# AgatheSenellart/MultiVae

Measured on AMD Instinct MI355X. Metric: train samples/sec (ELBO step) MoPoE MnistSvhn K=10, higher is better.
Workload: dtype f32 (error-corrected 2xfp16 / 3xbf16 products, fp32 accumulate); 1 GPU; MoPoE MnistSvhn (mnist MLP + svhn conv), K=10, per-device batch 512, latent_dim 20, Adam lr 1e-3, fwd+ELBO+bwd+optimizer; global_batch=512, K=10, parallelism=dp1, launch=hipGraph replay (fwd + bwd) + Adam

## Files before the change

include/mvk.h:

```cpp
#ifndef MVK_H
#define MVK_H

#include <stdint.h>

#ifdef __cplusplus
extern "C" {
#endif

#define MVK_OK 0
#define MVK_EINVAL (-1)
#define MVK_ELAUNCH (-2)

#define MVK_MAX_MODALITIES 8
#define MVK_MVAE_MAX_SUBSETS 32
#define MVK_IWAE_MAX_EXPERTS 32

#define MVK_DIST_NORMAL 0
#define MVK_DIST_LAPLACE 1
#define MVK_DIST_BERNOULLI 2
#define MVK_DIST_CATEGORICAL 3

#define MVK_ACT_NONE 0
#define MVK_ACT_RELU 1
#define MVK_ACT_SIGMOID 2
// ... 96 lines not shown
  int32_t fill;
} mvk_seed_desc;
int mvk_loss_backward_seed(const mvk_seed_desc* jobs, int n, const float* gscale, void* stream);


int mvk_mmvae_std_fwd(const float* lv, int rows, int L, int family, float* std, void* stream);
int mvk_mmvae_std_bwd(const float* lv, const float* std, const float* dstd, int rows, int L, int family,
                      float* dlv, void* stream);

int mvk_mmvae_latent_fwd(const float* const* mu, const float* const* std, const float* const* noise,
                         const uint8_t* const* masks, const float* prior_mean, const float* prior_std, int M,
                         int K, int B, int L, int family, float* const* z, float* const* lpz,
                         float* const* lqz, float* const* lq_all, int shared_dims, float* const* lqw, void* stream);

int mvk_mmvae_objective_fwd(const float* const* rows, const float* const* lpz, const float* const* lqz,
                            const uint8_t* const* masks, int M, int K, int B, int dreg, float* const* lw_out,
                            float* const* w, float* const* rowcoef, float* loss, const float* const* lqw, float beta,
                            void* stream);

int mvk_mmvae_latent_bwd(const float* const* mu, const float* const* std, const float* const* noise,
                         const float* const* z, const uint8_t* const* masks, const float* prior_mean,
                         const float* prior_std, const float* const* w, const float* const* lq_all,
                         const float* const* lqz, const float* const* dz_dec, int M, int K, int B, int L,
                         int family, int dreg, const float* gscale, float* const* dmu, float* const* dstd,
                         float* dprior_std, int shared_dims, float beta,
                         void* stream);

int mvk_mmvaeplus_cross_latent_fwd(const float* z, const float* prior_std, const float* noise, int64_t rows, int D,
                                   int Ls, int family, float* zc, void* stream);
int mvk_mmvaeplus_cross_latent_bwd(const float* dzc, const float* noise, int64_t rows, int D, int Ls, int family,
                                   float* dz, float* dprior_std, void* stream);


int mvk_iwae_sample(const float* loc, const float* sd, const float* noise, int K, int B, int L, int family, float* z,
                    void* stream);

int mvk_iwae_logw(const float* z, const float* const* rows, int n_rows, const float* const* loc,
                  const float* const* sd, int E, const float* prior_loc, const float* prior_sd, int K, int B, int L,
                  int family, float* lw, void* stream);

int mvk_iwae_reduce(const float* const* lw, int n, int K, int B, float* ll, void* stream);


int mvk_linear_fwd(const float* X, const float* W, const float* b, float* Y, int M, int N, int K, int act,
                   float* ws, int64_t ws_floats, void* stream);
int mvk_linear_bwd_data(const float* dY, const float* W, float* dX, int M, int N, int K, const float* y_out,
                        int y_act, const float* prev_out, int prev_act, int accumulate, float* colsum_acc,
                        float* ws, int64_t ws_floats, void* stream);
int mvk_linear_bwd_weight(const float* dY, const float* X, float* dW, float* db, int M, int N, int K,
                          const float* y_out, int y_act, float* ws, int64_t ws_floats, void* stream);
int64_t mvk_splitk_workspace_floats(int rows, int cols, int reduce_len);
int mvk_act_bwd_colsum(const float* dY, const float* Y, int act, int M, int N, float* dPre, float* db, float* ws,
                       int64_t ws_floats, void* stream);
int mvk_colsum_acc(const float* dY, const float* y_out, int y_act, float* db, int M, int N, float* ws, int64_t ws_floats,
                   void* stream);
int mvk_nchw_channel_sum_acc(const float* dY, const float* y_out, int y_act, float* db, int n, int c, int hw,
                             float* ws, int64_t ws_floats, void* stream);
int mvk_act_bwd(float* dY, const float* Y, int64_t n, int act, void* stream);
int mvk_act_bwd_scaled(const float* g, float a, const float* Y, int act, float* out, int64_t n, void* stream);

int mvk_gemm(const float* A, const float* B, float* C, int M, int N, int K, int ta, int tb, const float* bias,
             int bias_mod, int act, int accumulate, const float* a_act_src, int a_act, const float* c_act_src,
             int c_act, float* ws, int64_t ws_floats, void* stream);

#define MVK_FMT_IN_BF3 1
#define MVK_FMT_TILED 2
int mvk_f32_to_bf3(const float* x, int64_t n, void* planes, void* stream);
int mvk_bf3_to_f32(const void* planes, int64_t n, float* x, void* stream);

int mvk_pack_conv4s2_weight(const float* Wref, int Cv, int Cu, float* Wdown, int ld_down, int col_off,
                            float* Wup, void* stream);
#define MVK_PACK_MAX 16
typedef struct mvk_pack_desc {
  const float* Wref;
  float* Wdown;
  float* Wup;
  int Cv, Cu, ld_down, col_off, kind;
  void* Fdown;
  void* Fup;
  float* amax;
} mvk_pack_desc;
int64_t mvk_imgconv_frag_bytes(int Cu, int Cv);
int mvk_pack_weights(const mvk_pack_desc* jobs, int n, void* stream);
int mvk_conv4s2_down(const float* U, const float* Wdown, const float* bias, float* V, int n, int h, int w,
                     int Cu, int Cv, int act, int u_nchw, const float* u_act_src, int u_act,
                     const float* v_act_src, int v_act, float* colsum_acc, float* ws, int64_t ws_floats, int fmt,
                     const void* wfrag, void* stream);
int mvk_conv4s2_up(const float* V, const float* Wup, const float* bias, float* U, int n, int h, int w, int Cu,
                   int Cv, int act, int u_nchw, const float* u_act_src, int u_act, float* colsum_acc, float* ws,
                   int64_t ws_floats, int fmt, const void* wfrag, void* stream);
int mvk_gemm_smallk_amax(const float* A, const float* B, float* C, int M, int N, int K, int tb, const float* bias, int bias_mod,
                         int act, float* y_amax, void* stream);
int mvk_conv4s2_small_up_bwd_pre_y(const float* dpre, const float* rowscale, const float* V, int v_act, const float* Wref,
                                   float* dV, float* dWref, float* db, float* db_v, float* ws, int64_t ws_floats, int n, int h,
                                   int w, int Cu, int Cv, float* dv_amax, void* stream);
int mvk_conv4s2_scaled_ok(int n, int h, int w, int Cu, int Cv);
int mvk_conv4s2_wgrad_scaled_ok(int n, int h, int w, int Cu, int Cv);
int mvk_conv4s2_wgrad_s(const float* U, const float* V, float* dWref, int n, int h, int w, int Cu, int Cv, const float* u_amax,
                        const float* v_amax, float* ws, int64_t ws_floats, void* stream);
int mvk_conv4s2_down_s(const float* U, const float* Wdown, const float* bias, float* V, int n, int h, int w, int Cu, int Cv,
                       int act, const float* v_act_src, int v_act, float* colsum_acc, const float* x_amax,
                       const float* w_amax, float* y_amax, float* ws, int64_t ws_floats, const void* wfrag, void* stream);
int mvk_conv4s2_up_s(const float* V, const float* Wup, const float* bias, float* U, int n, int h, int w, int Cu, int Cv,
                     int act, const float* u_act_src, int u_act, float* colsum_acc, const float* x_amax, const float* w_amax,
                     float* y_amax, float* ws, int64_t ws_floats, const void* wfrag, void* stream);
int mvk_conv4s2_wgrad(const float* U, const float* V, float* dWref, int n, int h, int w, int Cu, int Cv,
                      int u_nchw, const float* u_act_src, int u_act, float* ws, int64_t ws_floats, void* stream);
int mvk_conv4s2_wgrad_pair(const float* U0, const float* V0, float* dW0, int h0, int w0, int Cu0, int Cv0, const float* U1,
                           const float* V1, float* dW1, int h1, int w1, int Cu1, int Cv1, int n, float* ws, int64_t ws_floats,
                           void* stream);

int mvk_conv3x3(const float* X, const float* Wp, const float* bias, float* Y, int n, int H, int W, int Cin, int Cout,
                int act, const float* y_act_src, int y_src_act, float* colsum_acc, float* ws, int64_t ws_floats,
                void* stream);
int mvk_conv3x3_res(const float* X, const float* Wp, const float* bias, float* Y, int n, int H, int W, int Cin,
                    int Cout, int act, const float* y_act_src, int y_src_act, const float* res, float res_alpha,
                    float* ws, int64_t ws_floats, void* stream);
int mvk_conv3x3_wgrad(const float* X, const float* dY, float* dWref, int n, int H, int W, int Cin, int Cout,
                      float* ws, int64_t ws_floats, void* stream);
int mvk_conv3x3_fused_ok(int n, int H, int W, int Cin, int Cout);
int mvk_conv3x3_f(const float* X, const float* Wp, const float* bias, float* Y, int n, int H, int W, int Cin, int Cout,
                  int act, const float* y_act_src, int y_src_act, const float* res, float res_alpha, float* colsum_acc,
                  int x_act, float pre_scale, float* ws, int64_t ws_floats, void* stream);
int mvk_conv3x3_wgrad_f(const float* X, const float* dY, float* dWref, float* db, int n, int H, int W, int Cin, int Cout,
                        int x_act, float dy_scale, float* ws, int64_t ws_floats, void* stream);
int mvk_amax(const float* x, int64_t n, float* out, void* stream);
int mvk_conv3x3_y(const float* X, const float* Wp, const float* bias, float* Y, int n, int H, int W, int Cin, int Cout, int act,
                  const float* y_act_src, int y_src_act, float* colsum_acc, float* y_amax, float* ws, int64_t ws_floats,
                  void* stream);
int mvk_conv3x3_scaled_ok(int n, int H, int W, int Cin, int Cout);
int mvk_conv3x3_s(const float* X, const float* Wp, const float* bias, float* Y, int n, int H, int W, int Cin, int Cout,
                  int act, const float* y_act_src, int y_src_act, const float* res, float res_alpha, float* colsum_acc,
                  int x_act, float pre_scale, const float* x_amax, const float* w_amax, float* y_amax, float* ws,
                  int64_t ws_floats, void* stream);
int mvk_conv3x3_s2(const float* X, const float* Wp, const float* bias, float* Y, float* y_pre, int n, int H, int W, int Cin, int Cout,
                   int act, const float* res, float res_alpha, const float* x_amax, const float* w_amax, float* y_amax, float* ws,
                   int64_t ws_floats, void* stream);
int mvk_conv3x3_s_part(const float* X, int x_channels, int x_off, const float* Wp, const float* bias, float* Y, int n, int H, int W,
                       int Cin, int Cout, int act, const float* y_act_src, int y_src_act, const float* res, int res_pre, int x_act,
                       float pre_scale, const float* x_amax, const float* w_amax, float* y_amax, void* stream);
int mvk_conv3x3_wgrad_scaled_ok(int n, int H, int W, int Cin, int Cout);
int mvk_conv3x3_wgrad_s(const float* X, const float* dY, float* dWref, float* db, int n, int H, int W, int Cin, int Cout,
                        int x_act, float dy_scale, const float* x_amax, const float* dy_amax, float* ws, int64_t ws_floats,
                        void* stream);
int mvk_avgpool3s2_fwd(const float* x, float* y, int n, int H, int W, int C, void* stream);
int mvk_avgpool3s2_bwd(const float* dy, float* dx, int n, int H, int W, int C, void* stream);
int mvk_upsample2_fwd(const float* x, float* y, int n, int H, int W, int C, void* stream);
int mvk_upsample2_bwd(const float* dy, float* dx, int n, int H, int W, int C, void* stream);
int mvk_axpby(const float* x, float a, const float* y, float b, int64_t n, int act, float* out, void* stream);
int mvk_probe_mfma_bf16(float* out, int iters, int random_operands, void* stream);
int mvk_probe_stream_copy(float* dst, const float* src, int64_t n, void* stream);
int mvk_transpose_act(const float* x, float* y, int batch, int rows, int cols, int act, const float* msrc, int dact,
                      void* stream);

int mvk_device_rng(float* out, int64_t n, uint64_t* state, int uniform, float lo, float hi, void* stream);
int mvk_conv4s2_up_nchw_small(const float* V, const float* Wref, const float* bias, float* U, int n, int h,
                              int w, int Cu, int Cv, int act, void* stream);

int mvk_conv4s2_small_down_fwd(const float* U, const float* Wdown, const float* bias, float* V, int n, int h, int w,
                               int Cu, int Cv, int act, void* stream);
int mvk_conv4s2_small_down_fwd_wref(const float* U, const float* Wref, const float* bias, float* V, int n, int h, int w,
                                    int Cu, int Cv, int act, void* stream);
int mvk_conv4s2_small_up_supported(int h, int w, int Cu, int Cv);
int mvk_conv4s2_small_up_fwd(const float* V, const float* Wref, const float* bias, float* U, int n, int h, int w,
                             int Cu, int Cv, int act, void* stream);
int mvk_conv4s2_small_up_bwd(const float* dU, const float* Uout, int u_act, const float* V, int v_act,
                             const float* Wref, float* dV, float* dWref, float* db, float* db_v, float* ws,
                             int64_t ws_floats, int n, int h, int w, int Cu, int Cv, void* stream);
int mvk_conv4s2_small_up_nll_supported(int h, int w, int Cu, int Cv);
int mvk_conv4s2_small_up_fwd_nll(const float* V, const float* Wref, const float* bias, const float* X, int xrows, float scale,
                                 float* dpre, float* rows, int n, int h, int w, int Cu, int Cv, int act, void* stream);
int mvk_conv4s2_small_up_bwd_pre(const float* dpre, const float* rowscale, const float* V, int v_act, const float* Wref,
                                 float* dV, float* dWref, float* db, float* db_v, float* ws, int64_t ws_floats, int n, int h,
                                 int w, int Cu, int Cv, void* stream);
int mvk_conv4s2_small_up_fwd_nll_w(const float* V, const float* Wref, const float* bias, const float* X, int xrows, float scale,
                                   float grad_weight, float* dpre, float* rows, int n, int h, int w, int Cu, int Cv, int act,
                                   void* stream);
int mvk_conv4s2_small_up_fwd_s(const float* V, const float* Wref, const float* bias, float* U, int n, int h, int w, int Cu, int Cv,
                               int act, const float* v_amax, void* stream);
int mvk_conv4s2_small_up_fwd_nll_s(const float* V, const float* Wref, const float* bias, const float* X, int xrows, float scale,
                                   float grad_weight, float* dpre, float* rows, int n, int h, int w, int Cu, int Cv, int act,
                                   const float* v_amax, void* stream);
int mvk_conv4s2_small_up_fwd_nll_sy(const float* V, const float* Wref, const float* bias, const float* X, int xrows, float scale,
                                    float grad_weight, float* dpre, float* rows, int n, int h, int w, int Cu, int Cv, int act,
                                    const float* v_amax, float* dpre_amax, void* stream);
int mvk_conv4s2_small_up_bwd_pre_s(const float* dpre, const float* rowscale, const float* V, int v_act, const float* Wref,
                                   float* dV, float* dWref, float* db, float* db_v, float* ws, int64_t ws_floats, int n, int h,
                                   int w, int Cu, int Cv, const float* dpre_amax, const float* v_amax, float* dv_amax,
// ... 178 lines not shown
```

multivae_amd/_lib.py:

```python
import ctypes as C
import os

import torch

_HERE = os.path.dirname(os.path.abspath(__file__))


_ALWAYS_READ = {"MVK_TUNE", "MVK_LIB_PATH", "MVK_DEFER_MB", "MVK_SYNC_DEBUG", "MVK_TRAINER_ALLOW_CPU", "MVK_CPU_THREADS",
                "MVK_BENCH_SAME_GPU", "MVK_FORCE_DIST", "MVK_DIST_BACKEND", "MVK_ADAM_ZERO", "MVK_RCCL", "MVK_BENCH_CHILD", "MVK_OVERLAP", "MVK_GRAPH_ADAM"}


def _warn_ignored_switches():
    if os.environ.get("MVK_TUNE") == "1":
        return
    ignored = sorted(k for k in os.environ if k.startswith("MVK_") and k not in _ALWAYS_READ)
    if ignored:
        import warnings

        warnings.warn(f"{', '.join(ignored)} set without MVK_TUNE=1: experiment switches are ignored unless MVK_TUNE=1 "
                      "(this process runs the shipped configuration)", RuntimeWarning, stacklevel=3)


_warn_ignored_switches()


def tune(name, default):
    return os.environ.get(name, default) if os.environ.get("MVK_TUNE") == "1" else default


LIB_PATH = os.environ.get("MVK_LIB_PATH") or os.path.join(_HERE, "libmvk.so")

MVK_OK = 0
DIST = {"normal": 0, "laplace": 1, "bernoulli": 2, "categorical": 3}
ACT = {None: 0, "none": 0, "relu": 1, "sigmoid": 2, "leaky_relu_0.2": 3}
FAMILY = {"normal": 0, "laplace_with_softmax": 1, "normal_with_softplus": 2}
MAX_MODALITIES = 8

_p = C.c_void_p
_i = C.c_int
_f = C.c_float
_d = C.c_double
_i64 = C.c_int64


class ReconDesc(C.Structure):
    _fields_ = [("recon", _p), ("x", _p), ("mask", _p), ("rows", _p), ("drecon", _p), ("rowcoef", _p),
                ("D", _i64), ("dist", C.c_int32), ("scale", _f), ("rescale", _f), ("coef", _f),
                ("n_classes", C.c_int32)]


class PackDesc(C.Structure):
    _fields_ = [("Wref", _p), ("Wdown", _p), ("Wup", _p), ("Cv", C.c_int32), ("Cu", C.c_int32),
                ("ld_down", C.c_int32), ("col_off", C.c_int32), ("kind", C.c_int32), ("Fdown", _p), ("Fup", _p),
                ("amax", _p)]


class CopyDesc(C.Structure):
    _fields_ = [("dst", _p), ("src", _p), ("bytes", _i64)]


class SeedDesc(C.Structure):
    _fields_ = [("buf", _p), ("n", _i64), ("coef", _f), ("fill", C.c_int32)]


class TermDesc(C.Structure):
    _fields_ = [("v", _p), ("mask", _p), ("n", _i64), ("period", _i64), ("coef", _f), ("lossw", _f), ("gfill", _p)]


PROTOTYPES = {
    "mvk_version": [],
    "mvk_mopoe_posterior_fwd": [_p, _p, _i, _p, _i, _p, _p, _p, _i, _i, _i, _p, _p, _p, _p, _p, _p, _p],
    "mvk_mopoe_posterior_bwd": [_p, _p, _i, _p, _i, _p, _p, _p, _p, _i, _i, _i, _p, _p, _p, _p],
    "mvk_mvtcae_posterior_fwd": [_p, _p, _p, _i, _p, _i, _i, _i, _p, _p, _p, _p, _p, _p],
    "mvk_mvtcae_posterior_bwd": [_p, _p, _p, _i, _p, _p, _i, _i, _i, _p, _p, _p, _p, _p],
    "mvk_jmvae_posterior_fwd": [_p, _p, _p, _p, _i, _p, _i, _i, _i, _p, _p, _p, _p],
    "mvk_jmvae_posterior_bwd": [_p, _p, _p, _p, _i, _p, _p, _i, _i, _i, _p, _p, _p, _p, _p, _p, _p],
    "mvk_recon_nll_fwd": [C.POINTER(ReconDesc), _i, _i, _i, _p],
    "mvk_recon_nll_bwd": [C.POINTER(ReconDesc), _i, _i, _i, _p],
    "mvk_reduce_terms": [C.POINTER(TermDesc), _i, _f, _p, _p, _p],
    "mvk_reduce_terms_ws": [C.POINTER(TermDesc), _i, _f, _p, _p, _p, _i64, _p],
    "mvk_scale_by_device_scalar": [_p, _i64, _p, _p],
    "mvk_linear_fwd": [_p, _p, _p, _p, _i, _i, _i, _i, _p, _i64, _p],
    "mvk_linear_bwd_data": [_p, _p, _p, _i, _i, _i, _p, _i, _p, _i, _i, _p, _p, _i64, _p],
    "mvk_linear_bwd_weight": [_p, _p, _p, _p, _i, _i, _i, _p, _i, _p, _i64, _p],
    "mvk_act_bwd_colsum": [_p, _p, _i, _i, _i, _p, _p, _p, _i64, _p],
    "mvk_colsum_acc": [_p, _p, _i, _p, _i, _i, _p, _i64, _p],
    "mvk_nchw_channel_sum_acc": [_p, _p, _i, _p, _i, _i, _i, _p, _i64, _p],
    "mvk_act_bwd": [_p, _p, _i64, _i, _p],
    "mvk_act_bwd_scaled": [_p, _f, _p, _i, _p, _i64, _p],
    "mvk_gemm": [_p, _p, _p, _i, _i, _i, _i, _i, _p, _i, _i, _i, _p, _i, _p, _i, _p, _i64, _p],
    "mvk_pack_conv4s2_weight": [_p, _i, _i, _p, _i, _i, _p, _p],
    "mvk_conv4s2_down": [_p, _p, _p, _p, _i, _i, _i, _i, _i, _i, _i, _p, _i, _p, _i, _p, _p, _i64, _i, _p, _p],
    "mvk_conv4s2_up": [_p, _p, _p, _p, _i, _i, _i, _i, _i, _i, _i, _p, _i, _p, _p, _i64, _i, _p, _p],
    "mvk_pack_weights": [C.POINTER(PackDesc), _i, _p],
    "mvk_loss_backward_seed": [C.POINTER(SeedDesc), _i, _p, _p],
    "mvk_f32_to_bf3": [_p, _i64, _p, _p],
    "mvk_bf3_to_f32": [_p, _i64, _p, _p],
    "mvk_conv4s2_small_up_fwd_nll": [_p, _p, _p, _p, _i, _f, _p, _p, _i, _i, _i, _i, _i, _i, _p],
    "mvk_conv4s2_small_up_fwd_nll_w": [_p, _p, _p, _p, _i, _f, _f, _p, _p, _i, _i, _i, _i, _i, _i, _p],
    "mvk_conv4s2_small_up_fwd_nll_s": [_p, _p, _p, _p, _i, _f, _f, _p, _p, _i, _i, _i, _i, _i, _i, _p, _p],
    "mvk_conv4s2_small_up_fwd_s": [_p, _p, _p, _p, _i, _i, _i, _i, _i, _i, _p, _p],
    "mvk_conv4s2_small_up_fwd_nll_sy": [_p, _p, _p, _p, _i, _f, _f, _p, _p, _i, _i, _i, _i, _i, _i, _p, _p, _p],
    "mvk_conv4s2_small_up_bwd_pre_s": [_p, _p, _p, _i, _p, _p, _p, _p, _p, _p, _i64, _i, _i, _i, _i, _i, _p, _p, _p, _p],
    "mvk_conv4s2_small_up_bwd_pre": [_p, _p, _p, _i, _p, _p, _p, _p, _p, _p, _i64, _i, _i, _i, _i, _i, _p],
    "mvk_conv3x3": [_p, _p, _p, _p, _i, _i, _i, _i, _i, _i, _p, _i, _p, _p, _i64, _p],
    "mvk_conv3x3_y": [_p, _p, _p, _p, _i, _i, _i, _i, _i, _i, _p, _i, _p, _p, _p, _i64, _p],
    "mvk_conv3x3_res": [_p, _p, _p, _p, _i, _i, _i, _i, _i, _i, _p, _i, _p, _f, _p, _i64, _p],
    "mvk_conv3x3_wgrad": [_p, _p, _p, _i, _i, _i, _i, _i, _p, _i64, _p],
    "mvk_conv3x3_f": [_p, _p, _p, _p, _i, _i, _i, _i, _i, _i, _p, _i, _p, _f, _p, _i, _f, _p, _i64, _p],
    "mvk_conv3x3_wgrad_f": [_p, _p, _p, _p, _i, _i, _i, _i, _i, _i, _f, _p, _i64, _p],
    "mvk_conv3x3_s": [_p, _p, _p, _p, _i, _i, _i, _i, _i, _i, _p, _i, _p, _f, _p, _i, _f, _p, _p, _p, _p, _i64, _p],
    "mvk_conv3x3_s2": [_p, _p, _p, _p, _p, _i, _i, _i, _i, _i, _i, _p, _f, _p, _p, _p, _p, _i64, _p],
    "mvk_conv3x3_s_part": [_p, _i, _i, _p, _p, _p, _i, _i, _i, _i, _i, _i, _p, _i, _p, _i, _i, _f, _p, _p, _p, _p],
    "mvk_amax": [_p, _i64, _p, _p],
    "mvk_conv4s2_wgrad_s": [_p, _p, _p, _i, _i, _i, _i, _i, _p, _p, _p, _i64, _p],
    "mvk_gemm_smallk_amax": [_p, _p, _p, _i, _i, _i, _i, _p, _i, _i, _p, _p],
    "mvk_conv4s2_small_up_bwd_pre_y": [_p, _p, _p, _i, _p, _p, _p, _p, _p, _p, _i64, _i, _i, _i, _i, _i, _p, _p],
    "mvk_conv4s2_down_s": [_p, _p, _p, _p, _i, _i, _i, _i, _i, _i, _p, _i, _p, _p, _p, _p, _p, _i64, _p, _p],
    "mvk_conv4s2_up_s": [_p, _p, _p, _p, _i, _i, _i, _i, _i, _i, _p, _i, _p, _p, _p, _p, _p, _i64, _p, _p],
    "mvk_conv3x3_wgrad_s": [_p, _p, _p, _p, _i, _i, _i, _i, _i, _i, _f, _p, _p, _p, _i64, _p],
    "mvk_avgpool3s2_fwd": [_p, _p, _i, _i, _i, _i, _p],
    "mvk_avgpool3s2_bwd": [_p, _p, _i, _i, _i, _i, _p],
    "mvk_upsample2_fwd": [_p, _p, _i, _i, _i, _i, _p],
    "mvk_upsample2_bwd": [_p, _p, _i, _i, _i, _i, _p],
    "mvk_axpby": [_p, _f, _p, _f, _i64, _i, _p, _p],
    "mvk_transpose_act": [_p, _p, _i, _i, _i, _i, _p, _i, _p],
    "mvk_probe_mfma_bf16": [_p, _i, _i, _p],
    "mvk_probe_stream_copy": [_p, _p, _i64, _p],
    "mvk_device_rng": [_p, _i64, _p, _i, _f, _f, _p],
    "mvk_conv4s2_wgrad": [_p, _p, _p, _i, _i, _i, _i, _i, _i, _p, _i, _p, _i64, _p],
    "mvk_conv4s2_wgrad_pair": [_p, _p, _p, _i, _i, _i, _i, _p, _p, _p, _i, _i, _i, _i, _i, _p, _i64, _p],
    "mvk_conv4s2_up_nchw_small": [_p, _p, _p, _p, _i, _i, _i, _i, _i, _i, _p],
    "mvk_conv4s2_small_up_fwd": [_p, _p, _p, _p, _i, _i, _i, _i, _i, _i, _p],
    "mvk_conv4s2_small_down_fwd": [_p, _p, _p, _p, _i, _i, _i, _i, _i, _i, _p],
    "mvk_conv4s2_small_down_fwd_wref": [_p, _p, _p, _p, _i, _i, _i, _i, _i, _i, _p],
    "mvk_conv4s2_small_up_bwd": [_p, _p, _i, _p, _i, _p, _p, _p, _p, _p, _p, _i64, _i, _i, _i, _i, _i, _p],
    "mvk_pack_unflatten_weight": [_p, _i, _i, _p, _p],
    "mvk_unflatten_wgrad": [_p, _p, _p, _i, _i, _i, _p, _i64, _p],
    "mvk_flatten_wgrad": [_p, _p, _p, _i, _i, _i, _p, _i64, _p],
    "mvk_nchw_to_nhwc": [_p, _p, _i, _i, _i, _i, _p],
    "mvk_nhwc_to_nchw": [_p, _p, _i, _i, _i, _i, _p],
    "mvk_adam_step": [_p, _p, _p, _p, _i64, _d, _d, _d, _d, _d, _i, _d, _p],
    "mvk_heads_fwd": [_p, _p, _p, _p, _p, _p, _p, _i, _i, _i, _i64, _i64, _p],
    "mvk_heads_bwd": [_p, _i, _p, _p, _p, _p, _i64, _i64, _i, _p, _p, _p, _p, _p, _p, _i, _i, _i, _p, _i64, _p],
    "mvk_defer_begin": [_p, _i64, _p, _i64],
    "mvk_defer_flush": [_p],
    "mvk_defer_end": [_p],
    "mvk_adam_step_amsgrad": [_p, _p, _p, _p, _p, _i64, _d, _d, _d, _d, _d, _i, _d, _p],
    "mvk_adam_step_fused": [_p, _p, _p, _p, _p, _i64, _d, _d, _d, _d, _d, _i, _d, _i, _p],
    "mvk_copy_batch": [C.POINTER(CopyDesc), _i, _p],
    "mvk_adam_prepare": [_p, _p, _p],
    "mvk_adam_step_pub": [_p, _p, _p, _p, _p, _i64, _d, _d, _d, _d, _d, _i, _d, _i, _p, _p],
    "mvk_adam_identity": [_p, _p],
    "mvk_adam_step_dev": [_p, _p, _p, _p, _p, _i64, _p, _i, _p],
    "mvk_mmvae_std_fwd": [_p, _i, _i, _i, _p, _p],
    "mvk_mmvae_std_bwd": [_p, _p, _p, _i, _i, _i, _p, _p],
    "mvk_mmvae_latent_fwd": [_p, _p, _p, _p, _p, _p, _i, _i, _i, _i, _i, _p, _p, _p, _p, _i, _p, _p],
    "mvk_mmvae_objective_fwd": [_p, _p, _p, _p, _i, _i, _i, _i, _p, _p, _p, _p, _p, _f, _p],
    "mvk_mmvae_latent_bwd": [_p, _p, _p, _p, _p, _p, _p, _p, _p, _p, _p, _i, _i, _i, _i, _i, _i, _p, _p, _p, _p, _i, _f, _p],
    "mvk_mmvaeplus_cross_latent_fwd": [_p, _p, _p, _i64, _i, _i, _i, _p, _p],
    "mvk_mmvaeplus_cross_latent_bwd": [_p, _p, _i64, _i, _i, _i, _p, _p, _p],
    "mvk_mvae_posterior_fwd": [_p, _p, _p, _i, _p, _i, _p, _i, _i, _p, _p, _p, _p, _p],
    "mvk_mvae_posterior_bwd": [_p, _p, _p, _i, _p, _i, _p, _p, _i, _i, _p, _p, _p, _p],
    "mvk_gauss_sample_kl_fwd": [_p, _p, _p, _i, _i, _i, _p, _p, _p],
    "mvk_gauss_sample_kl_bwd": [_p, _p, _p, _p, _p, _i, _i, _i, _p, _p, _p],
    "mvk_cond_latent_fwd": [_p, _p, _p, _p, _p, _p, _p, _i, _i, _i, _i, _p, _p, _p],
    "mvk_cond_latent_bwd": [_p, _p, _p, _p, _p, _p, _p, _i, _i, _i, _i, _p, _p, _p, _p, _p],
    "mvk_iwae_sample": [_p, _p, _p, _i, _i, _i, _i, _p, _p],
    "mvk_iwae_logw": [_p, _p, _i, _p, _p, _i, _p, _p, _i, _i, _i, _i, _p, _p],
    "mvk_iwae_reduce": [_p, _i, _i, _i, _p, _p],
    "mvk_poe_fwd": [_p, _p, _i, _i64, _f, _i, _p, _p, _p],
    "mvk_poe_bwd": [_p, _p, _i, _i64, _f, _i, _p, _p, _p, _p, _p],
    "mvk_kl_gauss_fwd": [_p, _i64, _p, _i64, _p, _i64, _p, _i64, _i64, _i, _p, _p],
    "mvk_kl_gauss_bwd": [_p, _i64, _p, _i64, _p, _i64, _p, _i64, _i64, _i, _p, _p, _p, _p, _p, _p],
    "mvk_logprob_fwd": [_p, _p, _i64, _i64, _i, _f, _i, _f, _p, _p],
    "mvk_logprob_bwd": [_p, _p, _i64, _i64, _i, _f, _i, _f, _p, _p, _p],
    "mvk_comm_unique_id": [_p],
    "mvk_comm_init": [C.POINTER(C.c_void_p), _i, _i, _p],
    "mvk_comm_destroy": [_p],
    "mvk_allreduce_avg": [_p, _i64, _i, _p, _p],
    "mvk_comm_size": [_p, C.POINTER(C.c_int), C.POINTER(C.c_int)],
    "mvk_allreduce_avg_ranges": [_p, C.POINTER(C.c_int64), C.POINTER(C.c_int64), _i, _i64, _p, _p],
    "mvk_event_create": [C.POINTER(C.c_void_p)],
    "mvk_event_destroy": [_p],
    "mvk_event_record": [_p, _i, _p],
    "mvk_stream_wait_event": [_p, _p],
    "mvk_dense16_pack": [_p, _i, _i, _p, _p, _p, _p, _p, _p, _p],
    "mvk_dense16_first": [_p, _p, _p, _p, _p, _p, _p, _i, _i, _i, _i, _p],
    "mvk_dense16_fwd_nll": [_p, _p, _p, _p, _p, _p, _p, _p, _i, _p, _f, _f, _p, _p, _p, _p, _p, _i, _i, _i, _p],
    "mvk_dense16_bwd_data": [_p, _p, _p, _p, _p, _p, _p, _p, _p, _p, _i64, _i, _i, _i, _p],
    "mvk_dense16_wgrad": [_p, _p, _p, _p, _p, _p, _p, _i, _p, _p, _p, _i64, _i, _i, _i, _p],
    "mvk_dense16_unsplit": [_p, _p, _p, _p, _f, _i, _i, _i, _p, _p],
    "mvk_nexus_aggregate_fwd": [_p, _p, _p, _p, _f, _i, _i, _i, _p, _p, _p],
    "mvk_nexus_aggregate_bwd": [_p, _p, _i, _i, _i, _p, _p],
    "mvk_nexus_top_nll_fwd": [_p, _p, _p, _p, _p, _p, _i, _i, _p, _p, _p, _p, _p],
    "mvk_nexus_top_nll_bwd": [_p, _p, _p, _p, _p, _p, _i, _i, _p, _p, _p, _p, _p, _p],
    "mvk_gmm_scratch_bytes": [_i, _i, C.POINTER(C.c_int64)],
    "mvk_gmm_estep": [_p, _i64, _i, _i, _p, _p, _p, _p, _i, _p, _p, _p, _p, _p, _p, _p],
    "mvk_gmm_mstep": [_p, _p, _i64, _i, _i, _d, _i, _p, _p, _p, _p, _p, _p, _p, _p],
    "mvk_gmm_em_step": [_p, _i64, _i, _i, _d, _d, _p, _p, _p, _p, _p, _p, _p, _p, _p, _p],
    "mvk_gmm_sample": [_p, _p, _p, _p, _i64, _i, _i, _p, _p],
    "mvk_ssim_tile": [],
# ... 50 lines not shown
    lib.mvk_conv3x3_fused_ok.restype = C.c_int
    lib.mvk_conv3x3_scaled_ok.argtypes = [_i, _i, _i, _i, _i]
    lib.mvk_conv3x3_scaled_ok.restype = C.c_int
    lib.mvk_conv3x3_wgrad_scaled_ok.argtypes = [_i, _i, _i, _i, _i]
    lib.mvk_conv3x3_wgrad_scaled_ok.restype = C.c_int
    lib.mvk_conv4s2_scaled_ok.argtypes = [_i, _i, _i, _i, _i]
    lib.mvk_conv4s2_scaled_ok.restype = C.c_int
    lib.mvk_conv4s2_wgrad_scaled_ok.argtypes = [_i, _i, _i, _i, _i]
    lib.mvk_conv4s2_wgrad_scaled_ok.restype = C.c_int
    lib.mvk_defer_wanted.argtypes = []
    lib.mvk_defer_wanted.restype = C.c_int64
    lib.mvk_defer_pending.argtypes = []
    lib.mvk_defer_pending.restype = C.c_int
    lib.mvk_prof_enable.argtypes = [_p, _i, _p, _p]
    lib.mvk_prof_enable.restype = C.c_int
    lib.mvk_prof_calibrate.argtypes = [_p, _i, _p]
    lib.mvk_prof_calibrate.restype = C.c_int
    lib.mvk_prof_count.argtypes = []
    lib.mvk_prof_count.restype = C.c_int
    lib.mvk_prof_clock_khz.argtypes = []
    lib.mvk_prof_clock_khz.restype = C.c_int
    lib.mvk_imgconv_frag_bytes.argtypes = [_i, _i]
    lib.mvk_imgconv_frag_bytes.restype = C.c_int64
    lib.mvk_comm_id_bytes.argtypes = []
    lib.mvk_comm_id_bytes.restype = C.c_int
    lib.mvk_comm_available.argtypes = []
    lib.mvk_comm_available.restype = C.c_int
    lib.mvk_dense16_ok.argtypes = [_i, _i, _i]
    lib.mvk_dense16_ok.restype = C.c_int
    lib.mvk_dense16_fwd_nll_rows.argtypes = [_i]
    lib.mvk_dense16_fwd_nll_rows.restype = C.c_int
    lib.mvk_dense16_colsum_rows.argtypes = [_i]
    lib.mvk_dense16_colsum_rows.restype = C.c_int
    lib.mvk_splitk_workspace_floats.argtypes = [_i, _i, _i]
    lib.mvk_splitk_workspace_floats.restype = C.c_int64
    _lib = lib
    return lib


def stream_ptr():
    return C.c_void_p(torch.cuda.current_stream().cuda_stream)


def ptr(t):
    if t is None:
        return None
    return C.c_void_p(t.data_ptr())


def ptr_array(tensors):
    arr = (C.c_void_p * len(tensors))()
    for i, t in enumerate(tensors):
        arr[i] = None if t is None else t.data_ptr()
    return arr


def check(rc, what):
    if rc != MVK_OK:
        raise MvkError(f"{what} failed with code {rc}")


_SYNC_DEBUG = os.environ.get("MVK_SYNC_DEBUG", "")


GEMM_FLOPS = {
    "mvk_linear_fwd": lambda a: 2.0 * a[4] * a[5] * a[6],
    "mvk_linear_bwd_data": lambda a: 2.0 * a[3] * a[4] * a[5],
    "mvk_linear_bwd_weight": lambda a: 2.0 * a[4] * a[5] * a[6],
    "mvk_gemm": lambda a: 2.0 * a[3] * a[4] * a[5],
    "mvk_conv4s2_down": lambda a: 2.0 * a[4] * a[5] * a[6] * 16 * a[7] * a[8],
    "mvk_conv4s2_up": lambda a: 2.0 * a[4] * a[5] * a[6] * 16 * a[7] * a[8],
    "mvk_conv4s2_wgrad": lambda a: 2.0 * a[3] * a[4] * a[5] * 16 * a[6] * a[7],
    "mvk_conv4s2_wgrad_pair": lambda a: 2.0 * a[14] * 16 * (a[3] * a[4] * a[5] * a[6] + a[10] * a[11] * a[12] * a[13]),
    "mvk_conv3x3": lambda a: 2.0 * a[4] * a[5] * a[6] * 9 * a[7] * a[8],
    "mvk_conv3x3_y": lambda a: 2.0 * a[4] * a[5] * a[6] * 9 * a[7] * a[8],
    "mvk_conv3x3_res": lambda a: 2.0 * a[4] * a[5] * a[6] * 9 * a[7] * a[8],
    "mvk_conv3x3_wgrad": lambda a: 2.0 * a[3] * a[4] * a[5] * 9 * a[6] * a[7],
    "mvk_conv3x3_f": lambda a: 2.0 * a[4] * a[5] * a[6] * 9 * a[7] * a[8],
    "mvk_conv3x3_wgrad_f": lambda a: 2.0 * a[4] * a[5] * a[6] * 9 * a[7] * a[8],
    "mvk_conv3x3_s": lambda a: 2.0 * a[4] * a[5] * a[6] * 9 * a[7] * a[8],
    "mvk_conv4s2_down_s": lambda a: 2.0 * a[4] * a[5] * a[6] * 16 * a[7] * a[8],
    "mvk_conv4s2_wgrad_s": lambda a: 2.0 * a[3] * a[4] * a[5] * 16 * a[6] * a[7],
    "mvk_conv4s2_up_s": lambda a: 2.0 * a[4] * a[5] * a[6] * 16 * a[7] * a[8],
    "mvk_conv3x3_wgrad_s": lambda a: 2.0 * a[4] * a[5] * a[6] * 9 * a[7] * a[8],
    "mvk_conv3x3_s2": lambda a: 2.0 * a[5] * a[6] * a[7] * 9 * a[8] * a[9],
    "mvk_conv3x3_s_part": lambda a: 2.0 * a[6] * a[7] * a[8] * 9 * a[9] * a[10],
    "mvk_conv4s2_up_nchw_small": lambda a: 2.0 * a[4] * a[5] * a[6] * 16 * a[7] * a[8],
    "mvk_conv4s2_small_up_fwd": lambda a: 2.0 * a[4] * a[5] * a[6] * 16 * a[7] * a[8],
    "mvk_conv4s2_small_down_fwd": lambda a: 2.0 * a[4] * a[5] * a[6] * 16 * a[7] * a[8],
    "mvk_conv4s2_small_down_fwd_wref": lambda a: 2.0 * a[4] * a[5] * a[6] * 16 * a[7] * a[8],
    "mvk_conv4s2_small_up_bwd": lambda a: 2.0 * 2.0 * a[12] * a[13] * a[14] * 16 * a[15] * a[16],
    "mvk_conv4s2_small_up_fwd_nll": lambda a: 2.0 * a[8] * a[9] * a[10] * 16 * a[11] * a[12],
    "mvk_conv4s2_small_up_fwd_nll_w": lambda a: 2.0 * a[9] * a[10] * a[11] * 16 * a[12] * a[13],
    "mvk_conv4s2_small_up_fwd_nll_s": lambda a: 2.0 * a[9] * a[10] * a[11] * 16 * a[12] * a[13],
    "mvk_conv4s2_small_up_bwd_pre": lambda a: 2.0 * 2.0 * a[11] * a[12] * a[13] * 16 * a[14] * a[15],
    "mvk_conv4s2_small_up_bwd_pre_y": lambda a: 2.0 * 2.0 * a[11] * a[12] * a[13] * 16 * a[14] * a[15],
    "mvk_conv4s2_small_up_fwd_nll_sy": lambda a: 2.0 * a[9] * a[10] * a[11] * 16 * a[12] * a[13],
    "mvk_conv4s2_small_up_bwd_pre_s": lambda a: 2.0 * 2.0 * a[11] * a[12] * a[13] * 16 * a[14] * a[15],
    "mvk_gemm_smallk_amax": lambda a: 2.0 * a[3] * a[4] * a[5],
    "mvk_unflatten_wgrad": lambda a: 2.0 * a[3] * a[4] * 16 * a[5],
    "mvk_flatten_wgrad": lambda a: 2.0 * a[3] * 16 * a[4] * a[5],
    "mvk_heads_fwd": lambda a: 2.0 * (2 if a[4] and a[4].value else 1) * a[7] * a[8] * a[9],
    "mvk_heads_bwd": lambda a: 4.0 * a[15] * a[16] * a[17] * (2 if a[3] else 1),
    "mvk_dense16_first": lambda a: 2.0 * a[7] * a[8] * a[9],
    "mvk_dense16_fwd_nll": lambda a: 2.0 * a[17] * a[18] * a[19],
    "mvk_dense16_bwd_data": lambda a: 2.0 * a[11] * a[12] * a[13],
    "mvk_dense16_wgrad": lambda a: 2.0 * a[12] * a[13] * a[14],
}
COUNT_FLOPS = None


_HIP = None


def new_stream(device):
    global _HIP
    if _HIP is None:
        cand = os.path.join(os.path.dirname(torch.__file__), "lib", "libamdhip64.so")
        _HIP = C.CDLL(cand if os.path.exists(cand) else "libamdhip64.so")
        _HIP.hipStreamCreateWithFlags.argtypes = [C.POINTER(C.c_void_p), C.c_uint]
        _HIP.hipStreamCreateWithFlags.restype = C.c_int
    h = C.c_void_p()
    with torch.cuda.device(device):
        rc = _HIP.hipStreamCreateWithFlags(C.byref(h), 1)
    if rc != 0 or not h.value:
        raise MvkError(f"hipStreamCreateWithFlags failed ({rc})")
    return torch.cuda.ExternalStream(h.value, device=device)


def call(name, *args):
    lib = load()
    check(getattr(lib, name)(*args), name)
    if COUNT_FLOPS is not None and name in GEMM_FLOPS:
        COUNT_FLOPS[0] += GEMM_FLOPS[name](args)
    if _SYNC_DEBUG and (_SYNC_DEBUG == "1" or name in _SYNC_DEBUG.split(",")):
        torch.cuda.synchronize()


def require_gpu_tensor(t, name="tensor"):
    if not t.is_cuda:
        raise MvkError(f"{name} must live on the GPU: multivae_amd has no CPU compute path")
    if t.dtype != torch.float32:
        raise MvkError(f"{name} must be float32, got {t.dtype}")
```

multivae_amd/csrc/igemm.hip:

```cpp
#include "igemm_bf.hpp"
#include <mutex>
#include <vector>

namespace mvk {
namespace {
struct DeferState {
  std::mutex mu;
  bool active = false;
  float* arena = nullptr;
  long long cap = 0, used = 0;
  long long wanted = 0;
  const char* g0 = nullptr;
  const char* g1 = nullptr;
  std::vector<DeferItem> items;
  std::vector<hipStream_t> streams;
  std::vector<hipEvent_t> events;
};
DeferState g_defer;

void defer_note_stream(hipStream_t s) {
  for (hipStream_t t : g_defer.streams)
    if (t == s) return;
  g_defer.streams.push_back(s);
}
// ... 569 lines not shown
  const int M = taps * Cu;
  if (deferred) return defer_push(e, M, Cv, nz, (long long)M * Cv);
  hipLaunchKernelGGL(splitk_reduce_kernel, dim3((M * Cv + 31) / 32), dim3(256), 0, s, e, M, Cv, nz);
  MVK_CHECK_LAUNCH();
  return MVK_OK;
}

__global__ void act_bwd_plain_kernel(float* __restrict__ dY, const float* __restrict__ Y, long long n, int act) {
  const long long stride = (long long)gridDim.x * blockDim.x;
  for (long long i = (long long)blockIdx.x * blockDim.x + threadIdx.x; i < n; i += stride)
    dY[i] *= mvk_act_grad_from_out(Y[i], act);
}

__global__ __launch_bounds__(256) void act_bwd_colsum_kernel(const float* __restrict__ dY, const float* __restrict__ Y,
                                                             int act, int M, int N, int rows_per_block,
                                                             float* __restrict__ dPre, float* __restrict__ part) {
  const int nq = N >> 2;
  const int r0 = blockIdx.x * rows_per_block;
  int r1 = r0 + rows_per_block;
  if (r1 > M) r1 = M;
  for (int q = threadIdx.x; q < nq; q += 256) {
    float4 acc = make_float4(0.f, 0.f, 0.f, 0.f);
#pragma unroll 4
    for (int r = r0; r < r1; ++r) {
      const long long o = (long long)r * N + 4 * q;
      float4 v = *reinterpret_cast<const float4*>(dY + o);
      const float4 y = *reinterpret_cast<const float4*>(Y + o);
      v.x *= mvk_act_grad_from_out(y.x, act);
      v.y *= mvk_act_grad_from_out(y.y, act);
      v.z *= mvk_act_grad_from_out(y.z, act);
      v.w *= mvk_act_grad_from_out(y.w, act);
      *reinterpret_cast<float4*>(dPre + o) = v;
      acc.x += v.x;
      acc.y += v.y;
      acc.z += v.z;
      acc.w += v.w;
    }
    *reinterpret_cast<float4*>(part + (long long)blockIdx.x * N + 4 * q) = acc;
  }
}

static int launch_with_colsum(GemmDesc& d, int zdim, float* db, float* ws, int64_t ws_floats, const float* out,
                              long long out_rows, hipStream_t s) {
  if (!db) return launch_igemm(d, zdim, s);
  const long long max_rows = (long long)((d.M + 63) / 64) * zdim;
  float* dpart = epilogue_vec_ok(d.e, d.N) ? defer_scratch(db, max_rows * d.N, s) : nullptr;
  float* cws = dpart ? dpart : ws;
  const bool fuse = cws && mvk_aligned16(cws) && epilogue_vec_ok(d.e, d.N) && (dpart || max_rows * d.N <= ws_floats);
  LaunchInfo info{};
  d.e.colsum_part = fuse ? cws : nullptr;
  int rc = launch_igemm(d, zdim, s, &info);
  d.e.colsum_part = nullptr;
  if (rc != MVK_OK) return rc;
  if (fuse && info.bm > 0) {
    const int rows = ((d.M + info.bm - 1) / info.bm) * zdim;
    return dpart ? defer_push_plain(db, dpart, d.N, rows, d.N, s) : colsum_finish(cws, rows, d.N, db, s);
  }
  return colsum(out, nullptr, 0, (int)out_rows, d.N, db, ws, ws_floats, s);
}

}

using namespace mvk;

namespace mvk {
int conv3_smallcin(const float* X, const float* Wp, const float* bias, float* Y, int n, int H, int W, int Cin, int Cout, int act,
                   const float* mask_src, int mask_act, hipStream_t s, float* y_amax = nullptr);
int conv3_smallcout(const float* X, const float* Wp, const float* bias, float* Y, int n, int H, int W, int Cin, int Cout, int act,
                    const float* mask_src, int mask_act, hipStream_t s);
int conv3_small_wgrad(const float* X, const float* dY, float* slab, long long slab_floats, int n, int H, int W, int Cin, int Cout,
                      int* nz, hipStream_t s);
int conv3_small_wgrad_slabs(const float* X, const float* dY, int n, int H, int W, int Cin, int Cout);
int heads_launch(const float* X, const float* W0, const float* b0, float* Y0, const float* W1, const float* b1, float* Y1,
                 int M, int N, int K, long long w_sk, long long w_sn, int act, hipStream_t s, float* ws = nullptr,
                 long long ws_floats = 0);
int heads_bwd_launch(const float* X, int x_act, const float* dY0, const float* dY1, const float* W0, const float* W1,
                     long long w_sk, long long w_sn, int flat_c, float* dX, float* wslab0, float* wslab1, float* bslab0,
                     float* bslab1, float* pslab, int M, int N, int K, int* nz, hipStream_t s);
int smallk_fwd(const float* X, const float* W, long long w_sk, long long w_sn, const float* bias, int bias_mod, int act,
               float* Y, int M, int N, int K, hipStream_t s, const float* mask_src = nullptr, int mask_act = 0,
               int accumulate = 0, float* y_amax = nullptr);
int imgconv_up(const float* V, const float* Wup, const void* wfrag, const float* bias, float* U, int n, int h, int w, int Cu,
               int Cv, int act, const float* u_act_src, int u_act, float* colsum_part, int* part_rows, const float* x_amax,
               const float* w_amax, float* y_amax, hipStream_t s);
int imgconv_down(const float* U, const float* Wdown, const void* wfrag, const float* bias, float* V, int n, int h, int w,
                 int Cu, int Cv, int act, const float* v_act_src, int v_act, float* colsum_part, int* part_rows,
                 const float* x_amax, const float* w_amax, float* y_amax, hipStream_t s);
int imgconv_wgrad(const float* U, const float* V, float* slab, long long slab_floats, int n, int h, int w, int Cu, int Cv,
                  int* nz, const float* u_amax, const float* v_amax, hipStream_t s);
int c3rs_conv(const float* X, const float* Wp, const float* bias, float* Y, int n, int H, int W, int Cin, int Cout, int act,
              const float* act_src, int src_act, const float* res, float res_alpha, float* colsum_part, int* part_rows,
              int x_act, float pre_scale, const float* x_amax, const float* w_amax, float* y_amax, hipStream_t s,
              float* y_pre = nullptr, int x_channels = 0, int w_channels = 0, int res_pre = 0);
bool c3rs_shape_ok(int n, int H, int W, int Cin, int Cout, int np);
bool c3rs_wgrad_ok(int n, int H, int W, int Cin, int Cout);
int c3rs_wgrad(const float* X, const float* dY, float* slab, long long slab_floats, float* dbpart, int x_act, float dy_scale,
               int n, int H, int W, int Cin, int Cout, int* nz, const float* x_amax, const float* y_amax, hipStream_t s);
int convref_reduce(const float* slab, int nz, int Cu, int Cv, int taps, float* dWref, hipStream_t s, bool deferred);
static bool c3rs_wgrad_covers(int n, int H, int W, int Cin, int Cout);
static bool c3rs_covers(int n, int H, int W, int Cin, int Cout, int np = 3) {
  static int min_tiles = -1;
  if (min_tiles < 0) {
    const char* e = mvk_tune("MVK_C3RS");
    min_tiles = e ? atoi(e) : 200;
    if (min_tiles == 0) min_tiles = 1 << 30;
  }
  if (g_dbg_flags & 0x400) return false;
  if (!c3rs_shape_ok(n, H, W, Cin, Cout, np)) return false;
  const long long tiles = ((long long)n * (H + 1) * (W + 1) + 31) / 32;
  return (g_dbg_flags & 0x800) ? true : tiles >= min_tiles;
}
static bool c3rs_wgrad_covers(int n, int H, int W, int Cin, int Cout) {
  if ((g_dbg_flags & 0x400) || !c3rs_wgrad_ok(n, H, W, Cin, Cout)) return false;
  if (g_dbg_flags & 0x800) return true;
  return c3rs_covers(n, H, W, 64, 64);
}
static int imgconv_min_images() {
  static int v = -1;
  if (v < 0) {
    const char* e = mvk_tune("MVK_IMGCONV");
    v = e ? atoi(e) : 256;
    if (v == 0) v = 1 << 30;
  }
  if (g_dbg_flags & 0x100) return 1 << 30;
  if (g_dbg_flags & 0x200) return 1;
  return v;
}
static bool imgconv_act_ok(int a) { return a == MVK_ACT_NONE || a == MVK_ACT_RELU; }
}

extern "C" {

static int launch_auto(GemmDesc& d, float* ws, int64_t ws_floats, hipStream_t s) {
  long long tiles = (long long)((d.M + 127) / 128) * ((d.N + 63) / 64);
  if (d.e.atomic || (ws && tiles < 128 && d.K >= 256)) return launch_splitk(d, ws, ws_floats, 512, s);
  return launch_igemm(d, 1, s);
}

int mvk_linear_fwd(const float* X, const float* W, const float* b, float* Y, int M, int N, int K, int act,
                   float* ws, int64_t ws_floats, void* stream) {
  if (M == 0) return MVK_OK;
  if (!X || !W || !Y || M < 0 || N <= 0 || K <= 0) return MVK_EINVAL;
  if (K <= 32) {
    const int rc = smallk_fwd(X, W, 1, K, b, N, act, Y, M, N, K, mvk_stream(stream));
    if (rc != 1) return rc;
  }
  static const int fewrows = mvk_tune("MVK_FEWROWS") ? atoi(mvk_tune("MVK_FEWROWS")) : 1024;
  if (M <= fewrows && K >= 64 && (long long)N * K <= (1 << 21)) {
    const int rc = heads_launch(X, W, b, Y, nullptr, nullptr, nullptr, M, N, K, 1, K, act, mvk_stream(stream), ws, ws_floats);
    if (rc != 1) return rc;
  }
  GemmDesc d{};
  plain_a(d.a, X, K, 1, M, K);
  plain_b(d.b, W, 1, K, K, N);
  rowmajor_epi(d.e, Y, N);
  d.e.bias = b;
  d.e.bias_mod = N;
  d.e.act = act;
  d.M = M;
  d.N = N;
  d.K = K;
  return launch_auto(d, ws, ws_floats, mvk_stream(stream));
}

int mvk_linear_bwd_data(const float* dY, const float* W, float* dX, int M, int N, int K, const float* y_out,
                        int y_act, const float* prev_out, int prev_act, int accumulate, float* colsum_acc, float* ws,
                        int64_t ws_floats, void* stream) {
  if (M == 0) return MVK_OK;
  if (!dY || !W || !dX || M < 0 || N <= 0 || K <= 0 || (colsum_acc && accumulate)) return MVK_EINVAL;
  GemmDesc d{};
// ... 49 lines not shown
  if (!fused) {
    if (dPre != dY && hipMemcpyAsync(dPre, dY, sizeof(float) * (size_t)M * N, hipMemcpyDeviceToDevice, s) != hipSuccess)
      return MVK_ELAUNCH;
    const long long n = (long long)M * N;
    hipLaunchKernelGGL(act_bwd_plain_kernel, dim3((unsigned)((n + 255) / 256 > 65535 ? 65535 : (n + 255) / 256)), dim3(256),
                       0, s, dPre, Y, n, act);
    MVK_CHECK_LAUNCH();
    return db ? colsum(dPre, nullptr, 0, M, N, db, ws, ws_floats, s) : MVK_OK;
  }
  float* dpart = db ? defer_scratch(db, (long long)blocks * N, s) : nullptr;
  hipLaunchKernelGGL(act_bwd_colsum_kernel, dim3(blocks), dim3(256), 0, s, dY, Y, act, M, N, rpb, dPre, dpart ? dpart : ws);
  MVK_CHECK_LAUNCH();
  if (dpart) return defer_push_plain(db, dpart, N, blocks, N, s);
  return db ? colsum_finish(ws, blocks, N, db, s) : MVK_OK;
}

int mvk_colsum_acc(const float* dY, const float* y_out, int y_act, float* db, int M, int N, float* ws, int64_t ws_floats,
                   void* stream) {
  if (!dY || !db) return MVK_EINVAL;
  return colsum(dY, y_out, y_act, M, N, db, ws, ws_floats, mvk_stream(stream));
}

int mvk_nchw_channel_sum_acc(const float* dY, const float* y_out, int y_act, float* db, int n, int c, int hw,
                             float* ws, int64_t ws_floats, void* stream) {
  if (!dY || !db || n < 0 || c <= 0 || hw <= 0) return MVK_EINVAL;
  if (n == 0) return MVK_OK;
  int ipb = 16;
  const int gy = (n + ipb - 1) / ipb;
  float* dpart = defer_scratch(db, (long long)gy * c, mvk_stream(stream));
  float* part = dpart ? dpart : ((ws && (long long)gy * c <= ws_floats) ? ws : nullptr);
  hipLaunchKernelGGL(nchw_channel_sum_kernel, dim3(c, gy), dim3(256), 0, mvk_stream(stream), dY, y_out, y_act, n, c, hw,
                     ipb, db, part);
  MVK_CHECK_LAUNCH();
  if (dpart) return defer_push_plain(db, dpart, c, gy, c, mvk_stream(stream));
  return part ? colsum_finish_any(part, gy, c, db, mvk_stream(stream)) : MVK_OK;
}

int mvk_gemm(const float* A, const float* B, float* C, int M, int N, int K, int ta, int tb, const float* bias,
             int bias_mod, int act, int accumulate, const float* a_act_src, int a_act, const float* c_act_src,
             int c_act, float* ws, int64_t ws_floats, void* stream) {
  if (!A || !B || !C || M < 0 || N <= 0 || K <= 0) return MVK_EINVAL;
  if (K <= 32 && !ta && !a_act_src && M > 0 && !accumulate && !c_act_src) {
    const int rc = smallk_fwd(A, B, tb ? 1 : N, tb ? K : 1, bias, bias_mod, act, C, M, N, K, mvk_stream(stream), c_act_src,
                              c_act, accumulate);
    if (rc != 1) return rc;
  }
  GemmDesc d{};
  if (ta)
    plain_a(d.a, A, 1, M, M, K);
  else
    plain_a(d.a, A, K, 1, M, K);
  d.a.act_src = a_act_src;
  d.a.act = a_act;
  if (tb)
    plain_b(d.b, B, 1, K, K, N);
  else
    plain_b(d.b, B, N, 1, K, N);
  rowmajor_epi(d.e, C, N);
  d.e.bias = bias;
  d.e.bias_mod = bias_mod > 0 ? bias_mod : 1;
  d.e.act = act;
  d.e.act_src = c_act_src;
  d.e.src_act = c_act;
  d.e.atomic = accumulate;
  d.M = M;
  d.N = N;
  d.K = K;
  return launch_auto(d, ws, ws_floats, mvk_stream(stream));
}

int mvk_gemm_smallk_amax(const float* A, const float* B, float* C, int M, int N, int K, int tb, const float* bias, int bias_mod,
                         int act, float* y_amax, void* stream) {
  if (!A || !B || !C || !y_amax || M < 0 || N <= 0 || K <= 0 || K > 32) return MVK_EINVAL;
  if (M == 0) return MVK_OK;
  const int rc = smallk_fwd(A, B, tb ? 1 : N, tb ? K : 1, bias, bias_mod, act, C, M, N, K, mvk_stream(stream), nullptr, 0, 0, y_amax);
  return rc == 1 ? MVK_EINVAL : rc;
}

static bool imgconv_pair(int h, int w, int Cu, int Cv) { return h == w && ((h == 8 && Cu == 32 && Cv == 64) || (h == 4 && Cu == 64 && Cv == 128)); }

static int conv4s2_down_impl(const float* U, const float* Wdown, const float* bias, float* V, int n, int h, int w, int Cu,
                             int Cv, int act, int u_nchw, const float* u_act_src, int u_act, const float* v_act_src,
                             int v_act, float* colsum_acc, float* ws, int64_t ws_floats, int fmt, const void* wfrag,
                             const float* x_amax, const float* w_amax, float* y_amax, void* stream) {
  if (n == 0) return MVK_OK;
  if (!U || !Wdown || !V || n < 0 || h <= 0 || w <= 0 || Cu <= 0 || Cv <= 0 || (!x_amax != !w_amax)) return MVK_EINVAL;
  const bool wants_rs = x_amax || y_amax;
  if ((fmt & ~MVK_FMT_IN_BF3) || ((fmt & MVK_FMT_IN_BF3) && (u_nchw || u_act_src))) return MVK_EINVAL;
  if (u_nchw && !u_act_src && !v_act_src && !colsum_acc) {
    if (mvk_conv4s2_small_up_supported(h, w, Cu, Cv))
      return mvk_conv4s2_small_down_fwd(U, Wdown, bias, V, n, h, w, Cu, Cv, act, stream);
    if (smallcin_supported(Cu, Cv)) return smallcin_fwd(U, Wdown, bias, V, n, h, w, Cu, Cv, act, mvk_stream(stream));
  }
  if (!u_nchw && !u_act_src && fmt == 0 && n >= imgconv_min_images() && imgconv_act_ok(act) &&
      imgconv_act_ok(v_act) && (!colsum_acc || (ws && ws_floats >= 256 * (int64_t)Cv)) && mvk_aligned16(U)) {
    int rows = 0;
    float* dpart = colsum_acc ? defer_scratch(colsum_acc, 256 * (long long)Cv, mvk_stream(stream)) : nullptr;
    float* cpart = dpart ? dpart : ws;
    const int rc = imgconv_down(U, Wdown, wfrag, bias, V, n, h, w, Cu, Cv, act, v_act_src, v_act, colsum_acc ? cpart : nullptr,
                                &rows, x_amax, w_amax, y_amax, mvk_stream(stream));
    if (rc == MVK_OK && dpart) return defer_push_plain(colsum_acc, dpart, Cv, rows, Cv, mvk_stream(stream));
    if (rc == MVK_OK && colsum_acc) return colsum_finish(ws, rows, Cv, colsum_acc, mvk_stream(stream));
    if (rc != 1) return rc;
  }
  if (wants_rs) return MVK_EINVAL;
  GemmDesc d{};
  d.a = AOperand{};
  d.a.p = U;
  d.a.kind = u_nchw ? A_DOWN_NCHW : A_DOWN;
  d.a.trans = 0;
  d.a.C = Cu;
  d.a.H = 2 * h;
  d.a.W = 2 * w;
  d.a.OH = h;
  d.a.OW = w;
  d.a.contig_k = u_nchw ? 0 : 1;
  d.a.vec4 = (!u_nchw) && (Cu % 4 == 0) && mvk_aligned16(U) && (!u_act_src || mvk_aligned16(u_act_src));
  d.a.act_src = u_act_src;
  d.a.act = u_act;
  d.a.bf3 = (fmt & MVK_FMT_IN_BF3) ? 1 : 0;
  d.a.plane_bytes = (long long)n * 4 * h * w * Cu * 2;
  plain_b(d.b, Wdown, Cv, 1, 16 * Cu, Cv);
  rowmajor_epi(d.e, V, Cv);
  d.e.bias = bias;
  d.e.bias_mod = Cv;
  d.e.act = act;
  d.e.act_src = v_act_src;
  d.e.src_act = v_act;
  d.M = n * h * w;
  d.N = Cv;
  d.K = 16 * Cu;
  return launch_with_colsum(d, 1, colsum_acc, ws, ws_floats, V, (long long)n * h * w, mvk_stream(stream));
}

int mvk_conv4s2_down(const float* U, const float* Wdown, const float* bias, float* V, int n, int h, int w, int Cu,
                     int Cv, int act, int u_nchw, const float* u_act_src, int u_act, const float* v_act_src,
                     int v_act, float* colsum_acc, float* ws, int64_t ws_floats, int fmt, const void* wfrag, void* stream) {
  return conv4s2_down_impl(U, Wdown, bias, V, n, h, w, Cu, Cv, act, u_nchw, u_act_src, u_act, v_act_src, v_act, colsum_acc, ws,
                           ws_floats, fmt, wfrag, nullptr, nullptr, nullptr, stream);
}

int mvk_conv4s2_scaled_ok(int n, int h, int w, int Cu, int Cv) {
  return n >= imgconv_min_images() && imgconv_pair(h, w, Cu, Cv) && (h != 4 || n % 2 == 0) ? 1 : 0;
}

int mvk_conv4s2_down_s(const float* U, const float* Wdown, const float* bias, float* V, int n, int h, int w, int Cu, int Cv,
                       int act, const float* v_act_src, int v_act, float* colsum_acc, const float* x_amax, const float* w_amax,
                       float* y_amax, float* ws, int64_t ws_floats, const void* wfrag, void* stream) {
  if (n == 0) return MVK_OK;
  if (!mvk_conv4s2_scaled_ok(n, h, w, Cu, Cv) || (!x_amax && !y_amax)) return MVK_EINVAL;
  return conv4s2_down_impl(U, Wdown, bias, V, n, h, w, Cu, Cv, act, 0, nullptr, MVK_ACT_NONE, v_act_src, v_act, colsum_acc, ws,
                           ws_floats, 0, wfrag, x_amax, w_amax, y_amax, stream);
}

static int conv4s2_up_impl(const float* V, const float* Wup, const float* bias, float* U, int n, int h, int w, int Cu,
                           int Cv, int act, int u_nchw, const float* u_act_src, int u_act, float* colsum_acc, float* ws,
                           int64_t ws_floats, int fmt, const void* wfrag, const float* x_amax, const float* w_amax,
                           float* y_amax, void* stream) {
  if (n == 0) return MVK_OK;
  if (!V || !Wup || !U || n < 0 || h <= 0 || w <= 0 || Cu <= 0 || Cv <= 0 || (colsum_acc && u_nchw) || (!x_amax != !w_amax))
    return MVK_EINVAL;
  const bool wants_rs = x_amax || y_amax;
  if (fmt & ~(MVK_FMT_IN_BF3 | MVK_FMT_TILED)) return MVK_EINVAL;
  if (!u_nchw && fmt == 0 && n >= imgconv_min_images() && imgconv_act_ok(act) && imgconv_act_ok(u_act) &&
      (!colsum_acc || (ws && ws_floats >= 256 * (int64_t)Cu)) && mvk_aligned16(V)) {
    int rows = 0;
    float* dpart = colsum_acc ? defer_scratch(colsum_acc, 256 * (long long)Cu, mvk_stream(stream)) : nullptr;
    float* cpart = dpart ? dpart : ws;
    const int rc = imgconv_up(V, Wup, wfrag, bias, U, n, h, w, Cu, Cv, act, u_act_src, u_act, colsum_acc ? cpart : nullptr,
                              &rows, x_amax, w_amax, y_amax, mvk_stream(stream));
    if (rc == MVK_OK && dpart) return defer_push_plain(colsum_acc, dpart, Cu, rows, Cu, mvk_stream(stream));
    if (rc == MVK_OK && colsum_acc) return colsum_finish(ws, rows, Cu, colsum_acc, mvk_stream(stream));
    if (rc != 1) return rc;
  }
  if (wants_rs) return MVK_EINVAL;
  GemmDesc d{};
  d.a = AOperand{};
  d.a.p = V;
  d.a.kind = A_UP;
  d.a.trans = 0;
  d.a.C = Cv;
  d.a.H = h;
  d.a.W = w;
  d.a.OH = h;
  d.a.OW = w;
  d.a.contig_k = 1;
  d.a.vec4 = (Cv % 4 == 0) && mvk_aligned16(V);
  d.a.bf3 = (fmt & MVK_FMT_IN_BF3) ? 1 : 0;
  d.a.plane_bytes = (long long)n * h * w * Cv * 2;
  plain_b(d.b, Wup, Cu, 1, 4 * Cv, Cu);
  d.b.z_stride = (long long)4 * Cv * Cu;
  d.e = Epilogue{};
  d.e.out = U;
  d.e.kind = u_nchw ? E_UP_NCHW : E_UP;
  d.e.ld = Cu;
  d.e.bias = bias;
  d.e.bias_mod = Cu;
  d.e.act = act;
  d.e.act_src = u_act_src;
  d.e.src_act = u_act;
  d.e.Cu = Cu;
  d.e.OH = h;
  d.e.OW = w;
  d.M = n * h * w;
  d.N = Cu;
  d.K = 4 * Cv;
  d.zmode = Z_PARITY;
  return launch_with_colsum(d, 4, colsum_acc, ws, ws_floats, U, (long long)n * 4 * h * w, mvk_stream(stream));
}

int mvk_conv4s2_up(const float* V, const float* Wup, const float* bias, float* U, int n, int h, int w, int Cu,
                   int Cv, int act, int u_nchw, const float* u_act_src, int u_act, float* colsum_acc, float* ws,
                   int64_t ws_floats, int fmt, const void* wfrag, void* stream) {
  return conv4s2_up_impl(V, Wup, bias, U, n, h, w, Cu, Cv, act, u_nchw, u_act_src, u_act, colsum_acc, ws, ws_floats, fmt, wfrag,
                         nullptr, nullptr, nullptr, stream);
}

int mvk_conv4s2_up_s(const float* V, const float* Wup, const float* bias, float* U, int n, int h, int w, int Cu, int Cv, int act,
                     const float* u_act_src, int u_act, float* colsum_acc, const float* x_amax, const float* w_amax,
                     float* y_amax, float* ws, int64_t ws_floats, const void* wfrag, void* stream) {
  if (n == 0) return MVK_OK;
  if (!mvk_conv4s2_scaled_ok(n, h, w, Cu, Cv) || (!x_amax && !y_amax)) return MVK_EINVAL;
  return conv4s2_up_impl(V, Wup, bias, U, n, h, w, Cu, Cv, act, 0, u_act_src, u_act, colsum_acc, ws, ws_floats, 0, wfrag, x_amax,
                         w_amax, y_amax, stream);
}

static int conv3x3_any(const float* X, const float* Wp, const float* bias, float* Y, int n, int H, int W, int Cin, int Cout,
                       int act, const float* y_act_src, int y_src_act, float* colsum_acc, const float* res, float res_alpha,
                       float* ws, int64_t ws_floats, void* stream, int x_act = MVK_ACT_NONE, float pre_scale = 1.f,
                       const float* x_amax = nullptr, const float* w_amax = nullptr, float* y_amax = nullptr,
                       float* y_pre = nullptr) {
  const bool img_y = y_amax && !x_amax && !w_amax && Cin <= 4 && !res && x_act == MVK_ACT_NONE && pre_scale == 1.f;
  const bool fused = !img_y && (x_act != MVK_ACT_NONE || pre_scale != 1.f || x_amax || w_amax || y_amax || y_pre);
  if (y_pre && !(res && x_amax && w_amax && !y_act_src && !colsum_acc)) return MVK_EINVAL;
  const int np = x_amax && w_amax ? 2 : 3;
  if (!X || !Wp || !Y || n < 0 || H <= 0 || W <= 0 || Cin <= 0 || Cout <= 0 || (!x_amax != !w_amax)) return MVK_EINVAL;
  if (fused && !(n > 0 && ws && ws_floats >= 256ll * Cout && !(res && colsum_acc) && mvk_aligned16(X) &&
                 (!colsum_acc || y_act_src) && c3rs_covers(n, H, W, Cin, Cout, np)))
    return MVK_EINVAL;
  if (n > 0 && Cin <= 4 && !res) {
    const int rc = conv3_smallcin(X, Wp, bias, Y, n, H, W, Cin, Cout, act, y_act_src, y_src_act, mvk_stream(stream), y_amax);
    if (rc == MVK_OK && colsum_acc)
      return colsum(Y, nullptr, 0, n * H * W, Cout, colsum_acc, ws, ws_floats, mvk_stream(stream));
    if (rc != 1) return rc;
  }
  if (img_y) return MVK_EINVAL;
  if (n > 0 && Cout <= 4 && !res) {
    const int rc = conv3_smallcout(X, Wp, bias, Y, n, H, W, Cin, Cout, act, y_act_src, y_src_act, mvk_stream(stream));
    if (rc == MVK_OK && colsum_acc)
      return colsum(Y, nullptr, 0, n * H * W, Cout, colsum_acc, ws, ws_floats, mvk_stream(stream));
    if (rc != 1) return rc;
  }
  if (n > 0 && ws && ws_floats >= 256ll * Cout && !(res && colsum_acc) && mvk_aligned16(X) && act != MVK_ACT_SIGMOID &&
      !(y_act_src && y_src_act == MVK_ACT_SIGMOID) && (!colsum_acc || y_act_src) && c3rs_covers(n, H, W, Cin, Cout, np)) {
    int rows = 0;
    float* dpart = colsum_acc ? defer_scratch(colsum_acc, 256ll * Cout, mvk_stream(stream)) : nullptr;
    const int rc = c3rs_conv(X, Wp, bias, Y, n, H, W, Cin, Cout, act, y_act_src, y_src_act, res, res_alpha,
                             colsum_acc ? (dpart ? dpart : ws) : nullptr, &rows, x_act, pre_scale, x_amax, w_amax, y_amax,
                             mvk_stream(stream), y_pre);
    if (rc == MVK_OK && dpart) return defer_push_plain(colsum_acc, dpart, Cout, rows, Cout, mvk_stream(stream));
    if (rc == MVK_OK && colsum_acc) return colsum_finish(ws, rows, Cout, colsum_acc, mvk_stream(stream));
    if (rc != 1) return rc;
    if (dpart) return MVK_EINVAL;
  }
  if (fused) return MVK_EINVAL;
  GemmDesc d{};
  d.a = AOperand{};
  d.a.p = X;
  d.a.kind = A_DOWN;
  d.a.tw = 3;
  d.a.mul = 1;
  d.a.trans = 0;
  d.a.C = Cin;
  d.a.H = H;
  d.a.W = W;
  d.a.OH = H;
  d.a.OW = W;
  d.a.contig_k = 1;
  d.a.vec4 = (Cin % 4 == 0) && mvk_aligned16(X);
  plain_b(d.b, Wp, Cout, 1, 9 * Cin, Cout);
  rowmajor_epi(d.e, Y, Cout);
  d.e.bias = bias;
  d.e.bias_mod = Cout;
  d.e.act = act;
  d.e.act_src = y_act_src;
  d.e.src_act = y_src_act;
  d.e.res = res;
  d.e.res_alpha = res_alpha;
  d.M = n * H * W;
  d.N = Cout;
  d.K = 9 * Cin;
  if (res && colsum_acc && !epilogue_vec_ok(d.e, d.N)) return MVK_EINVAL;
  return launch_with_colsum(d, 1, colsum_acc, ws, ws_floats, Y, (long long)n * H * W, mvk_stream(stream));
}

int mvk_conv3x3(const float* X, const float* Wp, const float* bias, float* Y, int n, int H, int W, int Cin, int Cout,
                int act, const float* y_act_src, int y_src_act, float* colsum_acc, float* ws, int64_t ws_floats,
                void* stream) {
  return conv3x3_any(X, Wp, bias, Y, n, H, W, Cin, Cout, act, y_act_src, y_src_act, colsum_acc, nullptr, 0.f, ws, ws_floats,
                     stream);
}

int mvk_conv3x3_res(const float* X, const float* Wp, const float* bias, float* Y, int n, int H, int W, int Cin, int Cout,
                    int act, const float* y_act_src, int y_src_act, const float* res, float res_alpha, float* ws,
                    int64_t ws_floats, void* stream) {
  if (!res) return MVK_EINVAL;
  return conv3x3_any(X, Wp, bias, Y, n, H, W, Cin, Cout, act, y_act_src, y_src_act, nullptr, res, res_alpha, ws, ws_floats,
                     stream);
}
// ... 363 lines not shown
```

multivae_amd/csrc/imgconv.hip:

```cpp
#include <cstdlib>
#include <type_traits>

#include "bf3.hpp"


namespace mvk {

constexpr int ic_sched(int hs) { return hs == 8 ? 5 : 4; }
constexpr int IC_SCHED2 = 2;

#ifdef MVK_ICPROF
__device__ unsigned long long* g_ic_dbg = nullptr;
#define IC_CLK() __builtin_readcyclecounter()
#endif

enum { IC_UP = 0, IC_DOWN = 1 };

struct ImgConvArgs {
  const float* A;
  const float* Wp;
  const void* wfrag;
  const float* bias;
  float* out;
  const float* act_src;
  float* colsum_part;
  int n;
  int act, src_act;
  mvk_prof_slot* prof;
  const float* x_amax;
  const float* w_amax;
  float* y_amax;
};

template <int KIND, int HS, int CIN, int COUT, int NP = 3>
struct ICfg {
  static constexpr int PIX = HS * HS;
  static constexpr int APIX = KIND == IC_UP ? PIX : 4 * PIX;
  static constexpr int AW = KIND == IC_UP ? HS : 2 * HS;
  static constexpr int CHUNKS = CIN / 16;
  static constexpr int NTAPS = 16 / CHUNKS;
  static constexpr int TAPS_ALL = KIND == IC_UP ? 4 : 16;
  static constexpr int KSPLIT = TAPS_ALL / NTAPS;
  static constexpr int NCT = COUT / 32;
  static constexpr int ROLES = (KIND == IC_UP ? 4 : 1) * NCT * KSPLIT;
  static constexpr int WG_TYPES = ROLES / 4;
  static constexpr int SU = PIX >= 32 ? 1 : 32 / PIX;
  static constexpr int TPU = PIX >= 32 ? PIX / 32 : 1;
  static constexpr int AROWS = SU * APIX;
  static constexpr int S = CIN * 2 + 16;
  static constexpr bool XPERM = KIND == IC_DOWN && HS == 8;
  static constexpr int LPAD = KIND == IC_DOWN ? 64 : 0;
  static constexpr int IPAD = (KIND == IC_DOWN && HS == 4) ? 16 : 0;
  static constexpr int LINEB = AW * S + LPAD;
  static constexpr int IMGB = AW * LINEB + IPAD;
  static constexpr int ZOFF = SU * IMGB;
  static constexpr int PLANE = SU * IMGB + S;
  __host__ __device__ static constexpr int pix_off(int img, int y, int x) {
    return img * IMGB + y * LINEB + (XPERM ? (x & 1) * (AW / 2) + (x >> 1) : x) * S;
  }
  static constexpr int BUF = NP * PLANE;
  static constexpr int NF4 = AROWS * CIN / 4 / 256;
  static constexpr int OWN = 16 / KSPLIT;
  static constexpr int XWAVE = (KSPLIT - 1) * OWN * 64 * 4;
  static constexpr int XBUF = KSPLIT > 1 ? 4 * XWAVE : 0;
  static constexpr int LDS_BYTES = 2 * BUF + 2 * XBUF + 4 * 32 * 4;
  static_assert(CIN % 16 == 0 && 16 % CHUNKS == 0 && TAPS_ALL % NTAPS == 0, "k split");
  static_assert(ROLES % 4 == 0 && COUT % 32 == 0, "roles");
  static_assert((AROWS * CIN / 4) % 256 == 0, "stage unit must split evenly over 256 threads");
  static_assert(LDS_BYTES <= 160 * 1024, "LDS");
};

__device__ __forceinline__ bf16x8 ic_pack8(const unsigned (&d)[4]) {
  u32x4 v = {d[0], d[1], d[2], d[3]};
  return __builtin_bit_cast(bf16x8, v);
}

template <int KIND, int HS, int CIN, int COUT, bool HAS_SRC, bool PIPE, int NP = 3>
__global__ __launch_bounds__(256) __attribute__((amdgpu_waves_per_eu(1, 1))) void imgconv_kernel(const ImgConvArgs g) {
  using T = ICfg<KIND, HS, CIN, COUT, NP>;
  static_assert(NP == 3 || PIPE, "the scaled-fp16 form exists for the two-tile-latency loop only");
  using frag = std::conditional_t<NP == 3, bf16x8, f16x8>;
  const float sx = NP == 2 ? f16_scale_of(*g.x_amax) : 1.f, sw = NP == 2 ? f16_scale_of(*g.w_amax) : 1.f;
  const float inv_s = NP == 2 ? f16_inv_scale(sx) * f16_inv_scale(sw) : 1.f;
  extern __shared__ __attribute__((aligned(16))) char lds[];
  mvk_prof_begin(g.prof);
#ifdef MVK_ICPROF
  const unsigned long long ic_t0 = IC_CLK();
  unsigned long long ic_bar = 0, ic_k = 0, ic_pre = 0, ic_post = 0, ic_tend = 0;
#endif
  const int tid = threadIdx.x, lane = tid & 63, wave = tid >> 6;
  const int col = lane & 31, kg = lane >> 5;
  int wgtype = blockIdx.x % T::WG_TYPES;
  int worker = blockIdx.x / T::WG_TYPES;
  const int workers = gridDim.x / T::WG_TYPES;
  if (T::WG_TYPES > 1 && gridDim.x % (8 * T::WG_TYPES) == 0) {
    const int xcd = blockIdx.x & 7, slot = blockIdx.x >> 3;
    wgtype = slot % T::WG_TYPES;
    worker = xcd * (gridDim.x / (8 * T::WG_TYPES)) + slot / T::WG_TYPES;
  }

  int cls = 0, ct = 0, ks = 0;
  if (KIND == IC_UP) {
    const int role = wgtype * 4 + wave;
    cls = role / (T::KSPLIT * T::NCT);
    ks = (role / T::NCT) % T::KSPLIT;
    ct = role % T::NCT;
  } else if (T::WG_TYPES == 1) {
    ks = wave / T::NCT;
    ct = wave % T::NCT;
  } else {
    ct = wgtype;
    ks = wave;
  }
  const int py = cls >> 1, px = cls & 1;
  const int ncol = ct * 32 + col;

  frag Bw[T::NTAPS][T::CHUNKS][NP];
  if (NP == 3 && g.wfrag) {
    const bf16x8* f = reinterpret_cast<const bf16x8*>(g.wfrag) + (long long)(wgtype * 4 + wave) * 16 * 3 * 64 + lane;
#pragma unroll
    for (int q = 0; q < T::NTAPS; ++q)
#pragma unroll
      for (int c = 0; c < T::CHUNKS; ++c)
#pragma unroll
        for (int pc = 0; pc < 3; ++pc) Bw[q][c][pc < NP ? pc : 0] = __builtin_bit_cast(frag, f[((q * T::CHUNKS + c) * 3 + pc) * 64]);
  } else
#pragma unroll
  for (int q = 0; q < T::NTAPS; ++q) {
    const int tap = ks * T::NTAPS + q;
    const long long rowbase = KIND == IC_UP ? (long long)(cls * 4 + tap) * CIN : (long long)tap * CIN;
#pragma unroll
    for (int c = 0; c < T::CHUNKS; ++c) {
      float v[8];
#pragma unroll
      for (int e = 0; e < 8; ++e) v[e] = g.Wp[(rowbase + c * 16 + kg * 8 + e) * COUT + ncol];
      unsigned p[3][4];
#pragma unroll
      for (int e = 0; e < 4; ++e) {
        if constexpr (NP == 3) bf3_split(v[2 * e], v[2 * e + 1], p[0][e], p[1][e], p[2][e]);
        else f16_split(v[2 * e] * sw, v[2 * e + 1] * sw, p[0][e], p[1][e]);
      }
#pragma unroll
      for (int pc = 0; pc < NP; ++pc) Bw[q][c][pc] = __builtin_bit_cast(frag, u32x4{p[pc][0], p[pc][1], p[pc][2], p[pc][3]});
    }
  }

#pragma unroll
  for (int q = 0; q < T::NTAPS; ++q)
#pragma unroll
    for (int c = 0; c < T::CHUNKS; ++c)
#pragma unroll
      for (int pc = 0; pc < NP; ++pc) {
        frag t = Bw[q][c][pc];
        asm volatile("" : "=a"(Bw[q][c][pc]) : "0"(t));
      }

  char* const xbase = lds + 2 * T::BUF;
  float* const csred = reinterpret_cast<float*>(lds + 2 * T::BUF + 2 * T::XBUF);
  for (int i = tid; i < 2 * NP * (T::S / 4); i += 256) {
    const int pl = i / (T::S / 4), w = i % (T::S / 4);
    *reinterpret_cast<unsigned*>(lds + (pl / NP) * T::BUF + (pl % NP) * T::PLANE + T::ZOFF + w * 4) = 0u;
  }
  int aoff[T::TPU][T::NTAPS];
#pragma unroll
  for (int tt = 0; tt < T::TPU; ++tt) {
    const int gr = tt * 32 + col;
    const int img = gr / T::PIX, p = gr % T::PIX, i = p / HS, j = p % HS;
#pragma unroll
    for (int q = 0; q < T::NTAPS; ++q) {
      const int tap = ks * T::NTAPS + q;
      int y, x;
      if (KIND == IC_UP) {
        y = i + py - (tap >> 1);
        x = j + px - (tap & 1);
      } else {
        y = 2 * i - 1 + (tap >> 2);
        x = 2 * j - 1 + (tap & 3);
      }
      const bool ok = y >= 0 && y < T::AW && x >= 0 && x < T::AW;
      aoff[tt][q] = (ok ? T::pix_off(img, y, x) : T::ZOFF) + kg * 16;
    }
  }
  int soff[T::NF4];
#pragma unroll
  for (int u = 0; u < T::NF4; ++u) {
    const int f = tid + u * 256;
    const int r = f / (CIN / 4), img = r / T::APIX, p = r % T::APIX;
    soff[u] = T::pix_off(img, p / T::AW, p % T::AW) + (f % (CIN / 4)) * 8;
  }
  auto out_off = [&](int tt, int r, int kgv) -> int {
    const int R = (r & 3) + 8 * (r >> 2) + 4 * kgv;
    const int gr = tt * 32 + R;
    const int img = gr / T::PIX, p = gr % T::PIX, i = p / HS, j = p % HS;
    if (KIND == IC_UP) return ((img * 2 * HS + 2 * i) * 2 * HS + 2 * j) * COUT;
    return (img * T::PIX + p) * COUT;
  };
  const int obase = out_off(0, ks * T::OWN, kg) + (KIND == IC_UP ? (py * 2 * HS + px) * COUT : 0) + ncol;
  constexpr long long OUT_UNIT = (long long)T::SU * (KIND == IC_UP ? 4 * T::PIX : T::PIX) * COUT;
  constexpr long long IN_UNIT = (long long)T::AROWS * CIN;

  const float bias = g.bias ? g.bias[ncol] : 0.f;
  const float act_lo = g.act == MVK_ACT_RELU ? 0.f : -__builtin_inff();
  const float src_lo = g.src_act == MVK_ACT_RELU ? 0.f : -__builtin_inff();
  float csum = 0.f, amax_l = 0.f;

  const long long units = g.n / T::SU;
  const long long u0 = __builtin_amdgcn_readfirstlane((int)(units * worker / workers));
  const long long u1 = __builtin_amdgcn_readfirstlane((int)(units * (worker + 1) / workers));

  f32x4 raw[T::NF4];
  auto unit_src = [&](long long u) {
    const long long uc = u < u1 ? u : u1 - 1;
    return reinterpret_cast<const f32x4*>(g.A + uc * IN_UNIT) + tid;
  };
  auto write_f4 = [&](char* buf, int k) {
    if constexpr (NP == 3) {
      unsigned a0, a1, a2, b0, b1, b2;
      bf3_split(raw[k][0], raw[k][1], a0, a1, a2);
      bf3_split(raw[k][2], raw[k][3], b0, b1, b2);
      *reinterpret_cast<u32x2*>(buf + soff[k]) = u32x2{a0, b0};
      *reinterpret_cast<u32x2*>(buf + T::PLANE + soff[k]) = u32x2{a1, b1};
      *reinterpret_cast<u32x2*>(buf + 2 * T::PLANE + soff[k]) = u32x2{a2, b2};
    } else {
      unsigned a0, a1, b0, b1;
      f16_split_su(raw[k][0], raw[k][1], sx, a0, a1);
      f16_split_su(raw[k][2], raw[k][3], sx, b0, b1);
      *reinterpret_cast<u32x2*>(buf + soff[k]) = u32x2{a0, b0};
      *reinterpret_cast<u32x2*>(buf + T::PLANE + soff[k]) = u32x2{a1, b1};
    }
  };

  if (u0 < u1) {
    const f32x4* s0 = unit_src(u0);
#pragma unroll
    for (int k = 0; k < T::NF4; ++k) raw[k] = s0[k * 256];
#pragma unroll
    for (int k = 0; k < T::NF4; ++k) write_f4(lds, k);
    const f32x4* s1 = unit_src(u0 + 1);
// ... 367 lines not shown
        ic_tend = IC_CLK();
        ic_bar += ic_tend - ic_b0;
#else
        if (tt == T::TPU - 1) __syncthreads();
#endif
        read_pair(a_cur, next_buf, ntt, 0);
      }
#pragma unroll
      for (int o = 0; o < T::OWN; ++o) msk_prev[o] = msk_cur[o];
      first = false;
#ifdef MVK_ICPROF
      ic_post += IC_CLK() - ic_tend;
#endif
    }
  }
  if (u0 < u1) {
    float* const outp_last = g.out + (u1 - 1) * OUT_UNIT;
#pragma unroll
    for (int o = 0; o < T::OWN; ++o) epilogue_row(outp_last, T::TPU - 1, o, 1.f);
  }

  }
  if (g.y_amax) {
    amax_publish(amax_l, g.y_amax, csred);
    __syncthreads();
  }
  if (g.colsum_part) {
    csum += __shfl_xor(csum, 32, 64);
    if (kg == 0) csred[wave * 32 + col] = csum;
    __syncthreads();
    if (KIND == IC_DOWN && T::WG_TYPES > 1) {
      if (tid < 32) {
        float s = 0.f;
        for (int w = 0; w < 4; ++w) s += csred[w * 32 + tid];
        g.colsum_part[(long long)worker * COUT + wgtype * 32 + tid] = s;
      }
    } else if (tid < COUT) {
      const int c_t = tid / 32, c_l = tid % 32;
      float s = 0.f;
      for (int w = 0; w < 4; ++w) {
        const int wct = KIND == IC_UP ? (wgtype * 4 + w) % T::NCT : w % T::NCT;
        if (wct == c_t) s += csred[w * 32 + c_l];
      }
      g.colsum_part[(long long)(worker * T::WG_TYPES + wgtype) * COUT + tid] = s;
    }
  }
#ifdef MVK_ICPROF
  if (g_ic_dbg && lane == 0) {
    unsigned long long* o = g_ic_dbg + (blockIdx.x * 4 + wave) * 4;
    o[0] = IC_CLK() - ic_t0;
    o[1] = ic_bar;
    o[2] = ic_k;
    o[3] = (ic_pre << 32) | (ic_post & 0xffffffffull);
  }
#endif
  mvk_prof_end(g.prof);
}

template <int KIND, int HS, int CIN, int COUT>
static int imgconv_launch_f16(const ImgConvArgs& a, int* part_rows, hipStream_t s) {
  using T = ICfg<KIND, HS, CIN, COUT, 2>;
  static bool attr_done = false;
  auto kern = a.act_src ? imgconv_kernel<KIND, HS, CIN, COUT, true, true, 2> : imgconv_kernel<KIND, HS, CIN, COUT, false, true, 2>;
  if (!attr_done) {
    const void* all[2] = {reinterpret_cast<const void*>(imgconv_kernel<KIND, HS, CIN, COUT, true, true, 2>),
                          reinterpret_cast<const void*>(imgconv_kernel<KIND, HS, CIN, COUT, false, true, 2>)};
    for (const void* f : all)
      if (hipFuncSetAttribute(f, hipFuncAttributeMaxDynamicSharedMemorySize, T::LDS_BYTES) != hipSuccess) return MVK_ELAUNCH;
    attr_done = true;
  }
  const int grid = 256;
  if (part_rows) *part_rows = (KIND == IC_DOWN && T::WG_TYPES > 1) ? grid / T::WG_TYPES : grid;
  ImgConvArgs ap = a;
  ap.prof = prof_next(KIND == IC_UP ? 2 : 3, 2.0 * a.n * HS * HS * 16.0 * CIN * COUT);
  hipLaunchKernelGGL(kern, dim3(grid), dim3(256), T::LDS_BYTES, s, ap);
  MVK_CHECK_LAUNCH();
  prof_fold(ap.prof, s);
  return MVK_OK;
}

template <int KIND, int HS, int CIN, int COUT>
static int imgconv_launch(const ImgConvArgs& a, int* part_rows, hipStream_t s) {
  using T = ICfg<KIND, HS, CIN, COUT>;
  if (a.x_amax && a.w_amax) return imgconv_launch_f16<KIND, HS, CIN, COUT>(a, part_rows, s);
  static bool attr_done = false;
  static const bool pipe = !(mvk_tune("MVK_IMGCONV_PIPE") && atoi(mvk_tune("MVK_IMGCONV_PIPE")) == 0);
  auto kern = a.act_src ? (pipe ? imgconv_kernel<KIND, HS, CIN, COUT, true, true> : imgconv_kernel<KIND, HS, CIN, COUT, true, false>)
                        : (pipe ? imgconv_kernel<KIND, HS, CIN, COUT, false, true> : imgconv_kernel<KIND, HS, CIN, COUT, false, false>);
  if (!attr_done) {
    const void* all[4] = {reinterpret_cast<const void*>(imgconv_kernel<KIND, HS, CIN, COUT, true, true>),
                          reinterpret_cast<const void*>(imgconv_kernel<KIND, HS, CIN, COUT, true, false>),
                          reinterpret_cast<const void*>(imgconv_kernel<KIND, HS, CIN, COUT, false, true>),
                          reinterpret_cast<const void*>(imgconv_kernel<KIND, HS, CIN, COUT, false, false>)};
    for (const void* f : all)
      if (hipFuncSetAttribute(f, hipFuncAttributeMaxDynamicSharedMemorySize, T::LDS_BYTES) != hipSuccess) return MVK_ELAUNCH;
    attr_done = true;
  }
  const int grid = 256;
  if (part_rows) *part_rows = (KIND == IC_DOWN && T::WG_TYPES > 1) ? grid / T::WG_TYPES : grid;
  ImgConvArgs ap = a;
  ap.prof = prof_next(KIND == IC_UP ? 2 : 3, 2.0 * a.n * HS * HS * 16.0 * CIN * COUT);
  hipLaunchKernelGGL(kern, dim3(grid), dim3(256), T::LDS_BYTES, s, ap);
  MVK_CHECK_LAUNCH();
  prof_fold(ap.prof, s);
  return MVK_OK;
}

template <int HS, int CU, int CV, int NP = 3>
struct WCfg {
  static constexpr int PIX = HS * HS, AW = 2 * HS;
  static constexpr bool SPLIT_KH = (CU * CV > 32 * 64);
  static constexpr int WG_TYPES = SPLIT_KH ? 4 : 1;
  static constexpr int NKW = SPLIT_KH ? 1 : 4;
  static constexpr int MT = SPLIT_KH ? CU / 32 : 4;
  static constexpr int NT = CV / 32;
  static constexpr int SU = PIX >= 32 ? 1 : 2;
  static constexpr int KS = SU * PIX / 16;
  static constexpr int UROWS_IMG = SPLIT_KH ? HS * AW : 4 * PIX;
  static constexpr int UROWS = SU * UROWS_IMG, VROWS = SU * PIX;
  static constexpr int PAD = SPLIT_KH ? 32 : 0;
  static constexpr int SUB = CU * 2 + PAD, SVB = CV * 2 + PAD;
  static constexpr int PLANE_U = (UROWS + 1) * SUB, PLANE_V = VROWS * SVB;
  static constexpr int OFF_V = NP * PLANE_U;
  static constexpr int BUF = NP * PLANE_U + 3 * PLANE_V;
  static constexpr int NFU = UROWS * CU / 4 / 256, NFV = VROWS * CV / 4 / 256;
  static constexpr int NF = NFU + NFV;
  static constexpr int LDS_BYTES = 2 * BUF;
  static_assert(MT * NT == 8, "8 accumulator tiles per wave");
  static_assert(SPLIT_KH || CU == 32, "the 4 taps of a kernel row are the 4 row tiles");
  static_assert(UROWS * CU / 4 % 256 == 0 && VROWS * CV / 4 % 256 == 0 && NF % KS == 0, "staging split");
  static_assert(LDS_BYTES <= 160 * 1024, "LDS");
};

typedef __bf16 bf16x4 __attribute__((ext_vector_type(4)));

typedef _Float16 ic_f16x4 __attribute__((ext_vector_type(4)));
template <typename F>
__device__ __forceinline__ F ic_tr_pair(const char* p0, const char* p1) {
  if constexpr (std::is_same<F, bf16x8>::value) {
    typedef __attribute__((address_space(3))) bf16x4* lp;
    const bf16x4 lo = __builtin_amdgcn_ds_read_tr16_b64_v4bf16((lp)(p0));
    const bf16x4 hi = __builtin_amdgcn_ds_read_tr16_b64_v4bf16((lp)(p1));
    return __builtin_shufflevector(lo, hi, 0, 1, 2, 3, 4, 5, 6, 7);
  } else {
    typedef __fp16 h4 __attribute__((__vector_size__(4 * sizeof(__fp16))));
    typedef __attribute__((address_space(3))) h4* lp;
    const ic_f16x4 lo = __builtin_bit_cast(ic_f16x4, __builtin_amdgcn_ds_read_tr16_b64_v4f16((lp)(p0)));
    const ic_f16x4 hi = __builtin_bit_cast(ic_f16x4, __builtin_amdgcn_ds_read_tr16_b64_v4f16((lp)(p1)));
    return __builtin_shufflevector(lo, hi, 0, 1, 2, 3, 4, 5, 6, 7);
  }
}

struct ImgWgradArgs {
  const float* U;
  const float* V;
  float* slab;
  int n;
  mvk_prof_slot* prof;
  const float* u_amax;
  const float* v_amax;
};

template <int HS, int CU, int CV, int NP = 3>
__global__ __launch_bounds__(256) __attribute__((amdgpu_waves_per_eu(1, 1))) void imgwgrad_kernel(const ImgWgradArgs g) {
  using T = WCfg<HS, CU, CV, NP>;
  using frag = std::conditional_t<NP == 3, bf16x8, f16x8>;
  constexpr int NPU = NP, NPV = 3;
// ... 164 lines not shown
      }
      {
        constexpr int IW_SCHED = 4;
#pragma unroll
        for (int m = 0; m < 2 * NP * T::MT * T::NT; ++m) {
          __builtin_amdgcn_sched_group_barrier(0x008, 1, 0);
          __builtin_amdgcn_sched_group_barrier(0x496, IW_SCHED * (NP == 3 ? 1 : 2), 0);
        }
      }
      if (s + 1 < T::KS) {
#pragma unroll
        for (int pc = 0; pc < 3; ++pc) {
          if (pc < NPU) {
#pragma unroll
            for (int a = 0; a < T::MT; ++a) Af[a][pc] = An[a][pc];
          }
#pragma unroll
          for (int b = 0; b < T::NT; ++b) Bf[b][pc] = Bn[b][pc];
        }
      }
    }
    __syncthreads();
    read_frags(Af, Bf, nbuf, 0);
  }

  float* const slab = g.slab + (long long)worker * 16 * CU * CV;
  const int col = lane & 31, kg = lane >> 5;
  const float oa = NP == 2 ? f16_inv_scale(su) : 1.f, ob = NP == 2 ? f16_inv_scale(sv) * (1.f / 2048.f) : 1.f;
#pragma unroll
  for (int a = 0; a < T::MT; ++a) {
    const int kw = T::SPLIT_KH ? wave : a, cut = T::SPLIT_KH ? a : 0;
    const int tap = kh * 4 + kw;
#pragma unroll
    for (int b = 0; b < T::NT; ++b)
#pragma unroll
      for (int r = 0; r < 16; ++r) {
        const int cu = cut * 32 + (r & 3) + 8 * (r >> 2) + 4 * kg;
        slab[(long long)(tap * CU + cu) * CV + b * 32 + col] = NP == 2 ? acc[a][b][r] * oa * ob : acc[a][b][r];
      }
  }
  mvk_prof_end(g.prof);
}

template <int HS, int CU, int CV, int NP>
static int imgwgrad_launch_np(const ImgWgradArgs& a, int* nz, hipStream_t s);
template <int HS, int CU, int CV>
static int imgwgrad_launch(const ImgWgradArgs& a, int* nz, hipStream_t s) {
  return a.u_amax && a.v_amax ? imgwgrad_launch_np<HS, CU, CV, 2>(a, nz, s) : imgwgrad_launch_np<HS, CU, CV, 3>(a, nz, s);
}
template <int HS, int CU, int CV, int NP>
static int imgwgrad_launch_np(const ImgWgradArgs& a, int* nz, hipStream_t s) {
  using T = WCfg<HS, CU, CV, NP>;
  static bool attr_done = false;
  auto kern = imgwgrad_kernel<HS, CU, CV, NP>;
  if (!attr_done) {
    if (hipFuncSetAttribute(reinterpret_cast<const void*>(kern), hipFuncAttributeMaxDynamicSharedMemorySize,
                            T::LDS_BYTES) != hipSuccess)
      return MVK_ELAUNCH;
    attr_done = true;
  }
  static const int grid_env = mvk_tune("MVK_IMGWGRAD_GRID") ? atoi(mvk_tune("MVK_IMGWGRAD_GRID")) : 256;
  const int grid = (grid_env >= T::WG_TYPES && grid_env <= 256) ? grid_env / T::WG_TYPES * T::WG_TYPES : 256;
  *nz = grid / T::WG_TYPES;
  ImgWgradArgs ap = a;
  ap.prof = prof_next(4, 2.0 * a.n * HS * HS * 16.0 * CU * CV);
  hipLaunchKernelGGL(kern, dim3(grid), dim3(256), T::LDS_BYTES, s, ap);
  MVK_CHECK_LAUNCH();
  prof_fold(ap.prof, s);
  return MVK_OK;
}

int imgconv_wgrad(const float* U, const float* V, float* slab, long long slab_floats, int n, int h, int w, int Cu, int Cv,
                  int* nz, const float* u_amax, const float* v_amax, hipStream_t s) {
  if (h != w) return 1;
  ImgWgradArgs a{U, V, slab, n, nullptr, u_amax, v_amax};
  if (h == 8 && Cu == 32 && Cv == 64 && slab_floats >= 256ll * 16 * Cu * Cv) return imgwgrad_launch<8, 32, 64>(a, nz, s);
  if (h == 4 && Cu == 64 && Cv == 128 && n % 2 == 0 && slab_floats >= 64ll * 16 * Cu * Cv)
    return imgwgrad_launch<4, 64, 128>(a, nz, s);
  return 1;
}

int imgconv_up(const float* V, const float* Wup, const void* wfrag, const float* bias, float* U, int n, int h, int w, int Cu,
               int Cv, int act, const float* u_act_src, int u_act, float* colsum_part, int* part_rows, const float* x_amax,
               const float* w_amax, float* y_amax, hipStream_t s) {
  if (h != w) return 1;
  ImgConvArgs a{V, Wup, wfrag, bias, U, u_act_src, colsum_part, n, act, u_act, nullptr, x_amax, w_amax, y_amax};
  if (h == 8 && Cv == 64 && Cu == 32) return imgconv_launch<IC_UP, 8, 64, 32>(a, part_rows, s);
  if (h == 4 && Cv == 128 && Cu == 64 && n % 2 == 0) return imgconv_launch<IC_UP, 4, 128, 64>(a, part_rows, s);
  return 1;
}

int imgconv_down(const float* U, const float* Wdown, const void* wfrag, const float* bias, float* V, int n, int h, int w,
                 int Cu, int Cv, int act, const float* v_act_src, int v_act, float* colsum_part, int* part_rows,
                 const float* x_amax, const float* w_amax, float* y_amax, hipStream_t s) {
  if (h != w) return 1;
  ImgConvArgs a{U, Wdown, wfrag, bias, V, v_act_src, colsum_part, n, act, v_act, nullptr, x_amax, w_amax, y_amax};
  if (h == 8 && Cu == 32 && Cv == 64) return imgconv_launch<IC_DOWN, 8, 32, 64>(a, part_rows, s);
  if (h == 4 && Cu == 64 && Cv == 128 && n % 2 == 0) return imgconv_launch<IC_DOWN, 4, 64, 128>(a, part_rows, s);
  return 1;
}

}

#ifdef MVK_ICPROF
extern "C" int mvk_imgconv_debug_buffer(unsigned long long* p) {
  return hipMemcpyToSymbol(HIP_SYMBOL(mvk::g_ic_dbg), &p, sizeof(p)) == hipSuccess ? 0 : -2;
}
#endif
```

multivae_amd/csrc/misc.hip:

```cpp
#include "bf3.hpp"

namespace {

__global__ void pack_conv4s2_kernel(const float* __restrict__ Wref, int Cv, int Cu, float* __restrict__ Wdown,
                                    int ldd, int coff, float* __restrict__ Wup) {
  int idx = blockIdx.x * blockDim.x + threadIdx.x;
  int total = Cv * Cu * 16;
  if (idx >= total) return;
  int tap = idx & 15;
  int cu = (idx >> 4) % Cu;
  int cv = (idx >> 4) / Cu;
  float v = Wref[idx];
  int kh = tap >> 2, kw = tap & 3;
  if (Wdown) Wdown[(long long)(tap * Cu + cu) * ldd + coff + cv] = v;
  if (Wup) {
    int ph = 1 - (kh & 1), a = kh >> 1;
    int pw = 1 - (kw & 1), b = kw >> 1;
    Wup[((long long)(ph * 2 + pw) * 4 * Cv + (a * 2 + b) * Cv + cv) * Cu + cu] = v;
  }
}

struct PackJobs {
  mvk_pack_desc j[MVK_PACK_MAX];
};
__device__ __forceinline__ void pack_amax(const mvk_pack_desc& d, int total, float* red) {
  constexpr int NB = 32;
  if (!d.amax || blockIdx.x >= NB) return;
  float m[8] = {0.f, 0.f, 0.f, 0.f, 0.f, 0.f, 0.f, 0.f};
  const int stride = NB * 256;
  for (int i = blockIdx.x * 256 + threadIdx.x; i < total; i += 8 * stride) {
#pragma unroll
    for (int j = 0; j < 8; ++j) {
      const int k = i + j * stride;
      m[j] = fmaxf(m[j], k < total ? fabsf(d.Wref[k]) : 0.f);
    }
  }
  const float mm = fmaxf(fmaxf(fmaxf(m[0], m[1]), fmaxf(m[2], m[3])), fmaxf(fmaxf(m[4], m[5]), fmaxf(m[6], m[7])));
  mvk::amax_publish(mm, d.amax, red);
}

__global__ __launch_bounds__(256) void pack_multi_kernel(const PackJobs jobs) {
  __shared__ float amax_red[4];
  const mvk_pack_desc& d = jobs.j[blockIdx.y];
  if (d.kind == 2) {
    const int total9 = d.Cv * d.Cu * 9;
    for (int idx = blockIdx.x * 256 + threadIdx.x; idx < total9; idx += gridDim.x * 256) {
      const int tap = idx % 9;
      const int cu = (idx / 9) % d.Cu;
      const int cv = (idx / 9) / d.Cu;
      const float v = d.Wref[idx];
      if (d.Wdown) d.Wdown[(long long)(tap * d.Cu + cu) * d.ld_down + d.col_off + cv] = v;
      if (d.Wup) d.Wup[(long long)((8 - tap) * d.Cv + cv) * d.Cu + cu] = v;
    }
    pack_amax(d, total9, amax_red);
    return;
  }
  const int total = d.Cv * d.Cu * 16;
  if (d.kind == 0 && d.Cu % 8 == 0 && d.Cv % 8 == 0 && d.ld_down % 4 == 0 && d.col_off % 4 == 0 &&
      mvk_dev_aligned16(d.Wref) && (!d.Wdown || mvk_dev_aligned16(d.Wdown)) && (!d.Wup || mvk_dev_aligned16(d.Wup))) {
    __shared__ __attribute__((aligned(16))) float T[8][8][16];
    const int tcu = d.Cu / 8, ntiles = (d.Cv / 8) * tcu, t = threadIdx.x;
    typedef float pf4 __attribute__((ext_vector_type(4)));
    typedef unsigned pu4 __attribute__((ext_vector_type(4)));
    float wmax = 0.f;
    for (int tile = blockIdx.x; tile < ntiles; tile += gridDim.x) {
      const int cv0 = (tile / tcu) * 8, cu0 = (tile % tcu) * 8;
      __syncthreads();
#pragma unroll
      for (int r = 0; r < 4; ++r) {
        const int e = t + 256 * r, cvl = e >> 7, rem = e & 127;
        const float v = d.Wref[((long long)(cv0 + cvl) * d.Cu + cu0) * 16 + rem];
        (&T[0][0][0])[e] = v;
        wmax = fmaxf(wmax, fabsf(v));
      }
      __syncthreads();
      const int pair = t >> 1, half = t & 1, tap = pair >> 3, l8 = pair & 7;
      const int kh = tap >> 2, kw = tap & 3, ph = 1 - (kh & 1), a = kh >> 1, pw = 1 - (kw & 1), b = kw >> 1;
      if (d.Wdown) {
        const pf4 v = {T[4 * half][l8][tap], T[4 * half + 1][l8][tap], T[4 * half + 2][l8][tap], T[4 * half + 3][l8][tap]};
        *reinterpret_cast<pf4*>(d.Wdown + (long long)(tap * d.Cu + cu0 + l8) * d.ld_down + d.col_off + cv0 + 4 * half) = v;
      }
      if (d.Wup) {
        const pf4 v = {T[l8][4 * half][tap], T[l8][4 * half + 1][tap], T[l8][4 * half + 2][tap], T[l8][4 * half + 3][tap]};
        *reinterpret_cast<pf4*>(d.Wup + ((long long)(ph * 2 + pw) * 4 * d.Cv + (a * 2 + b) * d.Cv + cv0 + l8) * d.Cu + cu0 + 4 * half) = v;
      }
      if (t < 128 && d.Fdown) {
        const int tp = t >> 3, cvl = t & 7, cv = cv0 + cvl;
        const int chunks = d.Cu / 16, ntaps = 16 / chunks, ksplit = 16 / ntaps, nct = d.Cv / 32;
        const int ks = tp / ntaps, q = tp % ntaps, ct = cv / 32;
        const int role = nct * ksplit <= 4 ? ks * nct + ct : ct * 4 + ks;
        const int kk = q * chunks + cu0 / 16, lane = ((cu0 % 16) / 8) * 32 + cv % 32;
        pu4 pc[3];
#pragma unroll
        for (int j = 0; j < 4; ++j) {
          unsigned p0, p1, p2;
          mvk::bf3_split(T[cvl][2 * j][tp], T[cvl][2 * j + 1][tp], p0, p1, p2);
          pc[0][j] = p0;
          pc[1][j] = p1;
          pc[2][j] = p2;
        }
        pu4* f = static_cast<pu4*>(d.Fdown);
#pragma unroll
        for (int p = 0; p < 3; ++p) f[(((long long)role * 16 + kk) * 3 + p) * 64 + lane] = pc[p];
      }
      if (t >= 128 && d.Fup) {
        const int i = t - 128, tp = i >> 3, cul = i & 7, cu = cu0 + cul;
        const int kh2 = tp >> 2, kw2 = tp & 3, ph2 = 1 - (kh2 & 1), a2 = kh2 >> 1, pw2 = 1 - (kw2 & 1), b2 = kw2 >> 1;
        const int chunks = d.Cv / 16, ntaps = 16 / chunks, ksplit = 4 / ntaps, nct = d.Cu / 32;
        const int t4 = a2 * 2 + b2, ks = t4 / ntaps, q = t4 % ntaps, ct = cu / 32;
        const int role = (ph2 * 2 + pw2) * (ksplit * nct) + ks * nct + ct;
        const int kk = q * chunks + cv0 / 16, lane = ((cv0 % 16) / 8) * 32 + cu % 32;
        pu4 pc[3];
#pragma unroll
        for (int j = 0; j < 4; ++j) {
          unsigned p0, p1, p2;
          mvk::bf3_split(T[2 * j][cul][tp], T[2 * j + 1][cul][tp], p0, p1, p2);
          pc[0][j] = p0;
          pc[1][j] = p1;
          pc[2][j] = p2;
        }
        pu4* f = static_cast<pu4*>(d.Fup);
#pragma unroll
        for (int p = 0; p < 3; ++p) f[(((long long)role * 16 + kk) * 3 + p) * 64 + lane] = pc[p];
      }
    }
    if (d.amax && blockIdx.x < ntiles) mvk::amax_publish(wmax, d.amax, amax_red);
    return;
  }
  for (int idx = blockIdx.x * 256 + threadIdx.x; idx < total; idx += gridDim.x * 256) {
    const int tap = idx & 15;
    const int cu = (idx >> 4) % d.Cu;
    const int cv = (idx >> 4) / d.Cu;
    const float v = d.Wref[idx];
    if (d.kind == 1) {
      d.Wup[(long long)cv * 16 * d.Cu + tap * d.Cu + cu] = v;
      continue;
    }
    const int kh = tap >> 2, kw = tap & 3;
    if (d.Wdown) d.Wdown[(long long)(tap * d.Cu + cu) * d.ld_down + d.col_off + cv] = v;
    const int ph = 1 - (kh & 1), a = kh >> 1;
    const int pw = 1 - (kw & 1), b = kw >> 1;
    if (d.Wup) d.Wup[((long long)(ph * 2 + pw) * 4 * d.Cv + (a * 2 + b) * d.Cv + cv) * d.Cu + cu] = v;
    if (d.Fdown || d.Fup) {
      unsigned p0, p1, p2;
      mvk::bf3_split(v, 0.f, p0, p1, p2);
      const unsigned short pc[3] = {(unsigned short)p0, (unsigned short)p1, (unsigned short)p2};
      if (d.Fdown) {
        const int chunks = d.Cu / 16, ntaps = 16 / chunks, ksplit = 16 / ntaps, nct = d.Cv / 32;
        const int ks = tap / ntaps, q = tap % ntaps, ct = cv / 32;
        const int role = nct * ksplit <= 4 ? ks * nct + ct : ct * 4 + ks;
        const int kk = q * chunks + cu / 16, lane = ((cu % 16) / 8) * 32 + cv % 32;
        unsigned short* f = static_cast<unsigned short*>(d.Fdown);
#pragma unroll
        for (int p = 0; p < 3; ++p) f[((((long long)role * 16 + kk) * 3 + p) * 64 + lane) * 8 + cu % 8] = pc[p];
      }
      if (d.Fup) {
        const int chunks = d.Cv / 16, ntaps = 16 / chunks, ksplit = 4 / ntaps, nct = d.Cu / 32;
        const int t4 = a * 2 + b, ks = t4 / ntaps, q = t4 % ntaps, ct = cu / 32;
        const int role = (ph * 2 + pw) * (ksplit * nct) + ks * nct + ct;
        const int kk = q * chunks + cv / 16, lane = ((cv % 16) / 8) * 32 + cu % 32;
        unsigned short* f = static_cast<unsigned short*>(d.Fup);
#pragma unroll
        for (int p = 0; p < 3; ++p) f[((((long long)role * 16 + kk) * 3 + p) * 64 + lane) * 8 + cv % 8] = pc[p];
      }
    }
  }
  pack_amax(d, total, amax_red);
}

__global__ void pack_unflatten_kernel(const float* __restrict__ Wref, int Cin, int Cout, float* __restrict__ Wp) {
  int idx = blockIdx.x * blockDim.x + threadIdx.x;
  int total = Cin * Cout * 16;
  if (idx >= total) return;
  int tap = idx & 15;
  int co = (idx >> 4) % Cout;
  int ci = (idx >> 4) / Cout;
  Wp[(long long)ci * 16 * Cout + tap * Cout + co] = Wref[idx];
}

__global__ void nchw_to_nhwc_kernel(const float* __restrict__ src, float* __restrict__ dst, long long total, int c,
                                    int hw) {
  long long idx = (long long)blockIdx.x * blockDim.x + threadIdx.x;
  if (idx >= total) return;
  int ch = idx % c;
  long long t = idx / c;
  int p = t % hw;
  long long n = t / hw;
  dst[idx] = src[(n * c + ch) * hw + p];
}
__global__ void nhwc_to_nchw_kernel(const float* __restrict__ src, float* __restrict__ dst, long long total, int c,
                                    int hw) {
  long long idx = (long long)blockIdx.x * blockDim.x + threadIdx.x;
  if (idx >= total) return;
  int p = idx % hw;
  long long t = idx / hw;
  int ch = t % c;
  long long n = t / c;
  dst[idx] = src[(n * hw + p) * c + ch];
}

__global__ void act_bwd_kernel(float* __restrict__ dY, const float* __restrict__ Y, long long n, int act) {
  long long i = (long long)blockIdx.x * blockDim.x + threadIdx.x;
  long long stride = (long long)gridDim.x * blockDim.x;
  for (; i < n; i += stride) dY[i] *= mvk_act_grad_from_out(Y[i], act);
}

// ... 304 lines not shown
__global__ __launch_bounds__(64) void prof_fold_kernel(mvk_prof_slot* s) {
  const unsigned long long now = (unsigned long long)wall_clock64();
  const int l = threadIdx.x & (MVK_PROF_ENTRIES - 1);
  unsigned long long t0 = s->w[8 + 8 * l], t1 = s->w[8 + 8 * MVK_PROF_ENTRIES + 8 * l];
#pragma unroll
  for (int off = MVK_PROF_ENTRIES / 2; off > 0; off >>= 1) {
    const unsigned long long a = __shfl_xor(t0, off, 64), b = __shfl_xor(t1, off, 64);
    t0 = a < t0 ? a : t0;
    t1 = b > t1 ? b : t1;
  }
  if (threadIdx.x == 0 && t1 > t0) {
    s->w[0] += t1 - t0;
    s->w[1] += 1;
    s->w[2] += now - t0;
  }
  if (threadIdx.x < MVK_PROF_ENTRIES) {
    s->w[8 + 8 * l] = ~0ull;
    s->w[8 + 8 * MVK_PROF_ENTRIES + 8 * l] = 0ull;
  }
}
__global__ __launch_bounds__(64) void prof_stamp_kernel(unsigned long long* out) {
  const unsigned long long t = (unsigned long long)wall_clock64();
  if (threadIdx.x == 0) {
    out[0] = t;
    out[1] = (unsigned long long)wall_clock64();
  }
}
namespace mvk {
mvk_prof_slot* prof_next(int kind, double work) {
  if (!g_prof_slots || g_prof_used >= g_prof_n) return nullptr;
  const int i = g_prof_used++;
  if (g_prof_kinds) g_prof_kinds[i] = kind;
  if (g_prof_work) g_prof_work[i] = work;
  return g_prof_slots + i;
}
void prof_fold(mvk_prof_slot* slot, hipStream_t s) {
  if (slot) hipLaunchKernelGGL(prof_fold_kernel, dim3(1), dim3(64), 0, s, slot);
}
}

extern "C" {

int mvk_version(void) { return 100; }

int mvk_prof_enable(void* device_slots, int nslots, int32_t* host_kinds, double* host_work) {
  g_prof_slots = static_cast<mvk_prof_slot*>(device_slots);
  g_prof_n = device_slots ? nslots : 0;
  g_prof_used = 0;
  g_prof_kinds = host_kinds;
  g_prof_work = host_work;
  return MVK_OK;
}
int mvk_prof_count(void) { return g_prof_used; }
int mvk_prof_calibrate(void* device_ticks, int n, void* stream) {
  if (!device_ticks || n < 2) return MVK_EINVAL;
  unsigned long long* out = static_cast<unsigned long long*>(device_ticks);
  for (int i = 0; i < n; ++i) hipLaunchKernelGGL(prof_stamp_kernel, dim3(1), dim3(64), 0, mvk_stream(stream), out + 2 * i);
  MVK_CHECK_LAUNCH();
  return MVK_OK;
}
int mvk_prof_clock_khz(void) {
  int dev = 0, khz = 0;
  if (hipGetDevice(&dev) != hipSuccess) return 0;
  if (hipDeviceGetAttribute(&khz, hipDeviceAttributeWallClockRate, dev) != hipSuccess) return 0;
  return khz;
}

int mvk_pack_conv4s2_weight(const float* Wref, int Cv, int Cu, float* Wdown, int ld_down, int col_off,
                            float* Wup, void* stream) {
  if (!Wref || Cv <= 0 || Cu <= 0 || (!Wdown && !Wup)) return MVK_EINVAL;
  int total = Cv * Cu * 16;
  hipLaunchKernelGGL(pack_conv4s2_kernel, dim3((total + 255) / 256), dim3(256), 0, mvk_stream(stream), Wref, Cv, Cu,
                     Wdown, ld_down > 0 ? ld_down : Cv, col_off, Wup);
  MVK_CHECK_LAUNCH();
  return MVK_OK;
}

int64_t mvk_imgconv_frag_bytes(int Cu, int Cv) {
  if ((Cu == 32 && Cv == 64) || (Cu == 64 && Cv == 128)) return (int64_t)16 * Cu * Cv * 3 * 2;
  return 0;
}

int mvk_pack_weights(const mvk_pack_desc* jobs, int n, void* stream) {
  if (!jobs || n <= 0 || n > MVK_PACK_MAX) return MVK_EINVAL;
  PackJobs pj{};
  int maxtot = 0;
  for (int i = 0; i < n; ++i) {
    const mvk_pack_desc& d = jobs[i];
    if (!d.Wref || d.Cv <= 0 || d.Cu <= 0 || d.kind < 0 || d.kind > 2 || (!d.Wdown && !d.Wup && !d.Fdown && !d.Fup) ||
        (d.kind == 1 && !d.Wup))
      return MVK_EINVAL;
    if ((d.Fdown || d.Fup) && (d.kind != 0 || mvk_imgconv_frag_bytes(d.Cu, d.Cv) == 0)) return MVK_EINVAL;
    pj.j[i] = d;
    if (pj.j[i].ld_down <= 0) pj.j[i].ld_down = d.Cv;
    const int tot = d.Cv * d.Cu * 16;
    if (tot > maxtot) maxtot = tot;
  }
  int gx = (maxtot + 255) / 256;
  if (gx > 256) gx = 256;
  hipLaunchKernelGGL(pack_multi_kernel, dim3(gx, n), dim3(256), 0, mvk_stream(stream), pj);
  MVK_CHECK_LAUNCH();
  return MVK_OK;
}

int mvk_pack_unflatten_weight(const float* Wref, int Cin, int Cout, float* Wp, void* stream) {
  if (!Wref || !Wp || Cin <= 0 || Cout <= 0) return MVK_EINVAL;
  int total = Cin * Cout * 16;
  hipLaunchKernelGGL(pack_unflatten_kernel, dim3((total + 255) / 256), dim3(256), 0, mvk_stream(stream), Wref, Cin,
                     Cout, Wp);
  MVK_CHECK_LAUNCH();
  return MVK_OK;
}

int mvk_nchw_to_nhwc(const float* src, float* dst, int n, int c, int h, int w, void* stream) {
  if (!src || !dst) return MVK_EINVAL;
  long long total = (long long)n * c * h * w;
  if (total == 0) return MVK_OK;
  hipLaunchKernelGGL(nchw_to_nhwc_kernel, dim3((unsigned)((total + 255) / 256)), dim3(256), 0, mvk_stream(stream), src,
                     dst, total, c, h * w);
  MVK_CHECK_LAUNCH();
  return MVK_OK;
}

int mvk_nhwc_to_nchw(const float* src, float* dst, int n, int c, int h, int w, void* stream) {
  if (!src || !dst) return MVK_EINVAL;
  long long total = (long long)n * c * h * w;
  if (total == 0) return MVK_OK;
  hipLaunchKernelGGL(nhwc_to_nchw_kernel, dim3((unsigned)((total + 255) / 256)), dim3(256), 0, mvk_stream(stream), src,
                     dst, total, c, h * w);
  MVK_CHECK_LAUNCH();
  return MVK_OK;
}

int mvk_act_bwd(float* dY, const float* Y, int64_t n, int act, void* stream) {
  if (!dY || !Y) return MVK_EINVAL;
  if (n == 0) return MVK_OK;
  if (n % 4 == 0 && mvk_aligned16(dY) && mvk_aligned16(Y))
    hipLaunchKernelGGL(act_bwd4_kernel, dim3((unsigned)((n / 4 + 255) / 256)), dim3(256), 0, mvk_stream(stream),
                       reinterpret_cast<float4*>(dY), reinterpret_cast<const float4*>(Y), (long long)(n / 4), act);
  else
    hipLaunchKernelGGL(act_bwd_kernel, dim3(grid_for(n, 256)), dim3(256), 0, mvk_stream(stream), dY, Y, (long long)n, act);
  MVK_CHECK_LAUNCH();
  return MVK_OK;
}

int mvk_act_bwd_scaled(const float* g, float a, const float* Y, int act, float* out, int64_t n, void* stream) {
  if (!g || !Y || !out || n < 0) return MVK_EINVAL;
  if (n == 0) return MVK_OK;
  hipLaunchKernelGGL(act_bwd_scaled_kernel, dim3((unsigned)((n / 4 + 256) / 256)), dim3(256), 0, mvk_stream(stream), g, a, Y,
                     (long long)n, act, out);
  MVK_CHECK_LAUNCH();
  return MVK_OK;
}

int mvk_scale_by_device_scalar(float* buf, int64_t n, const float* gscale, void* stream) {
  if (!buf || !gscale) return MVK_EINVAL;
  if (n == 0) return MVK_OK;
  hipLaunchKernelGGL(scale_kernel, dim3(grid_for(n, 256)), dim3(256), 0, mvk_stream(stream), buf, (long long)n, gscale);
  MVK_CHECK_LAUNCH();
  return MVK_OK;
}

int mvk_loss_backward_seed(const mvk_seed_desc* jobs, int n, const float* gscale, void* stream) {
  if (!jobs || !gscale || n <= 0 || n > MVK_SEED_MAX) return MVK_EINVAL;
  SeedJobs sj{};
  long long maxn = 0;
  for (int i = 0; i < n; ++i) {
    if (!jobs[i].buf || jobs[i].n < 0) return MVK_EINVAL;
    sj.j[i] = jobs[i];
    if (jobs[i].n > maxn) maxn = jobs[i].n;
  }
  if (maxn == 0) return MVK_OK;
  long long gx = (maxn + 255) / 256;
  if (gx > 4096) gx = 4096;
  hipLaunchKernelGGL(loss_seed_kernel, dim3((unsigned)gx, n), dim3(256), 0, mvk_stream(stream), sj, gscale);
// ... 724 lines not shown
```

multivae_amd/kernels.py:

```python
import ctypes as C
import math

import torch
from torch.autograd import Function
from torch.autograd.function import once_differentiable

from . import _lib, schedule
from ._lib import ACT, DIST, FAMILY, PackDesc, ReconDesc, SeedDesc, TermDesc, call, ptr, ptr_array, stream_ptr

RELU, SIGMOID, NONE = ACT["relu"], ACT["sigmoid"], ACT["none"]

PROFILE = {}
DIRECT_GRAD = True
deferred_reductions = schedule.deferred_reductions
_ws = schedule._ws

_RNG = {}
_UNIT_SEEDS = {}
_CONST_GRADS = {}


def _c(t):
    _lib.require_gpu_tensor(t)
    return t if t.is_contiguous() else t.contiguous()
# ... 70 lines not shown
def linear_bwd_weight(dy, x2, w, b, y_out=None, y_act=NONE):
    M, N = dy.shape
    K = x2.shape[1]
    dw, rw = _grad_target(w)
    db, rb = _grad_target(b) if b is not None else (None, None)
    ws = _ws(dy)
    call("mvk_linear_bwd_weight", ptr(dy), ptr(x2), ptr(dw), ptr(db), M, N, K, ptr(y_out), y_act, ptr(ws),
         ws.numel(), stream_ptr())
    return rw, rb


def gemm(a, b, M, N, K, ta=False, tb=False, bias=None, bias_mod=0, act=NONE, out=None, accumulate=False,
         a_act_src=None, a_act=NONE, c_act_src=None, c_act=NONE):
    c = out if out is not None else _new((M, N), a)
    ws = _ws(a)
    call("mvk_gemm", ptr(a), ptr(b), ptr(c), M, N, K, int(ta), int(tb), ptr(bias), bias_mod, act,
         1 if accumulate else 0, ptr(a_act_src), a_act, ptr(c_act_src), c_act, ptr(ws), ws.numel(), stream_ptr())
    return c


def heads_fwd(h2, w_mu, b_mu, w_lv, b_lv, N, w_sk, w_sn):
    M, K = h2.shape
    if N > 32 or K % 4 != 0:
        return None
    mu, lv = _new((M, N), h2), _new((M, N), h2)
    call("mvk_heads_fwd", ptr(h2), ptr(w_mu), ptr(b_mu), ptr(mu), ptr(w_lv), ptr(b_lv), ptr(lv), M, N, K, w_sk, w_sn,
         stream_ptr())
    return mu, lv


HEADS_BWD = _lib.tune("MVK_HEADS_BWD", "1") != "0"
_HEADS_BWD_MLP_MODE = _lib.tune("MVK_HEADS_BWD_MLP", "auto")


def heads_bwd_mlp(device):
    if _HEADS_BWD_MLP_MODE in ("0", "1"):
        return _HEADS_BWD_MLP_MODE == "1"
    return not schedule.has_big_late_leaves(device)


def heads_bwd(x, x_act, dys, ws_, bs, w_sk, w_sn, flat_c=0, want_dx=True, prev_bias=None, dw_params=None):
    M, K = x.shape
    N = dys[0].shape[1]
    if not HEADS_BWD or N > 32 or K % 16 != 0 or len(dys) > 2 or M < 1 or (M + 127) // 128 > 64:
        return None
    dw_params = ws_ if dw_params is None else dw_params
    tw, rw = zip(*[_grad_target(p) for p in dw_params])
    tb, rb = zip(*[_grad_target(b) if b is not None else (None, None) for b in bs])
    tp, rp = _grad_target(prev_bias) if prev_bias is not None else (None, None)
    dx = _new((M, K), x) if want_dx else None
    two = len(dys) == 2
    ws = _ws(x)
    rgs = (M + 127) // 128
    if (len(dys) * (N * K + N) + K) * rgs + 64 > ws.numel():
        return None
    call("mvk_heads_bwd", ptr(x), x_act, ptr(dys[0]), ptr(dys[1]) if two else None, ptr(ws_[0]), ptr(ws_[1]) if two else None,
         w_sk, w_sn, flat_c, ptr(dx), ptr(tw[0]), ptr(tw[1]) if two else None, ptr(tb[0]), ptr(tb[1]) if two else None,
         ptr(tp), M, N, K, ptr(ws), ws.numel(), stream_ptr())
    return dx, list(rw), list(rb), rp


def colsum(dy2, b, y_out=None, y_act=NONE):
    M, N = dy2.shape
    db, rb = _grad_target(b)
    ws = _ws(dy2)
    call("mvk_colsum_acc", ptr(dy2), ptr(y_out), y_act, ptr(db), M, N, ptr(ws), ws.numel(), stream_ptr())
    return rb


def pack_conv(wref, want_down=True, want_up=True):
    (wd, wu), = pack_weights([(wref, want_down, want_up)])
    return wd, wu


def _frag(like, Cu, Cv):
    nb = _lib.load().mvk_imgconv_frag_bytes(Cu, Cv)
    return torch.empty(nb, dtype=torch.uint8, device=like.device) if nb else None


def wfrag(w):
    return getattr(w, "mvk_frag", None)


PACK_MAX = 16
_PACK_SCOPE = None


class pack_scope:

    def __init__(self, model):
        self.model, self.own = model, False

    def __enter__(self):
        global _PACK_SCOPE
        if _PACK_SCOPE is None:
            _PACK_SCOPE = {"model": self.model, "cache": {}, "done": False}
            self.own = True
            dev = next((p.device for p in self.model.parameters()), None)
            if (C3_F16 or IMG_F16) and dev is not None and dev.type == "cuda":
                _PACK_SCOPE["amax"], _PACK_SCOPE["amax_pos"] = torch.zeros(512, dtype=torch.float32, device=dev), 0
        return self

    def __exit__(self, *exc):
        global _PACK_SCOPE
        if self.own:
            _PACK_SCOPE = None
        return False


def _job_key(job):
    return (job[0].data_ptr(), tuple(job[0].shape)) + tuple(job[1:])


def pack_weights(jobs):
    sc = _PACK_SCOPE
    keys = [_job_key(j) for j in jobs]
    rot = schedule.rotation(jobs[0][0].device)
    if rot is not None and rot.cache:
        hit = [k in rot.cache for k in keys]
        if any(hit):
            rot.wait()
            if all(hit):
                return [rot.cache[k] for k in keys]
            rest = iter(pack_weights([j for j, h in zip(jobs, hit) if not h]))
            return [rot.cache[k] if h else next(rest) for k, h in zip(keys, hit)]
    if sc is None:
        return _pack_launch(jobs)
    cache = sc["cache"]
    if all(k in cache for k in keys):
        return [cache[k] for k in keys]
    todo, tkeys = list(jobs), list(keys)
    if not sc["done"]:
        sc["done"] = True
        for mod in sc["model"].modules():
            announce = getattr(mod, "pack_jobs", None)
            if announce is None:
                continue
            for j in announce():
                k = _job_key(j)
                if rot is not None and k in rot.cache:
                    continue
                if k not in tkeys and k not in cache and j[0].device == jobs[0][0].device and len(todo) < PACK_MAX:
                    todo.append(j)
                    tkeys.append(k)
    outs = []
    for i0 in range(0, len(todo), PACK_MAX):
        outs += _pack_launch(todo[i0:i0 + PACK_MAX])
    for k, o in zip(tkeys, outs):
        cache[k] = o
    return outs[:len(jobs)]


def _pack_launch(jobs, am=None):
    descs = (PackDesc * len(jobs))()
    outs = []
    if am is None and ((C3_F16 and any(job[1] == "c3" for job in jobs))
                       or (IMG_F16 and any(job[1] not in ("c3", "unflatten") for job in jobs))):
        am = _amax_slots(jobs[0][0], len(jobs), create=True)
    for i, job in enumerate(jobs):
        wref = job[0]
        Cv, Cu = wref.shape[0], wref.shape[1]
        d = descs[i]
        d.Wref, d.Cv, d.Cu, d.ld_down, d.col_off = wref.data_ptr(), Cv, Cu, Cv, 0
        if job[1] == "unflatten":
            wp = _new((Cv, 16 * Cu), wref)
            d.kind, d.Wdown, d.Wup = 1, None, wp.data_ptr()
            outs.append(wp)
        elif job[1] == "c3":
            wf = _new((9 * Cu, Cv), wref) if job[2] else None
            wb = _new((9 * Cv, Cu), wref) if job[3] else None
            d.kind = 2
            d.Wdown = wf.data_ptr() if wf is not None else None
            d.Wup = wb.data_ptr() if wb is not None else None
            if am is not None:
                d.amax = am[i:i + 1].data_ptr()
                for t in (wf, wb):
                    if t is not None:
                        t.mvk_amax = am[i:i + 1]
            outs.append((wf, wb))
        else:
            wd = _new((16 * Cu, Cv), wref) if job[1] else None
            wu = _new((4, 4 * Cv, Cu), wref) if job[2] else None
            d.kind = 0
            d.Wdown = wd.data_ptr() if wd is not None else None
            d.Wup = wu.data_ptr() if wu is not None else None
            if wd is not None:
                wd.mvk_frag = _frag(wref, Cu, Cv)
                d.Fdown = wd.mvk_frag.data_ptr() if wd.mvk_frag is not None else None
            if wu is not None:
                wu.mvk_frag = _frag(wref, Cu, Cv)
                d.Fup = wu.mvk_frag.data_ptr() if wu.mvk_frag is not None else None
            if am is not None:
                d.amax = am[i:i + 1].data_ptr()
                for t in (wd, wu):
                    if t is not None:
                        t.mvk_amax = am[i:i + 1]
            outs.append((wd, wu))
    call("mvk_pack_weights", descs, len(jobs), stream_ptr())
    return outs


def conv4s2_scaled_ok(n, h, w, Cu, Cv):
    return bool(_lib.load().mvk_conv4s2_scaled_ok(n, h, w, Cu, Cv))


def conv_down(U, wdown, bias, n, h, w, Cu, Cv, act=NONE, u_nchw=False, u_act_src=None, u_act=NONE,
              v_act_src=None, v_act=NONE, out_bias=None, in_bf3=False, frag=None, amax=None, out=None):
    V = out if out is not None else torch.empty((n, h, w, Cv), dtype=torch.float32, device=U.device)
    ws = _ws(V)
    tb, rb = _bias_target(out_bias)
    if amax is not None:
        if u_nchw or u_act_src is not None or in_bf3:
            raise _lib.MvkError("conv_down: the amax form takes NHWC fp32 input without a fused input activation")
        call("mvk_conv4s2_down_s", ptr(U), ptr(wdown), ptr(bias), ptr(V), n, h, w, Cu, Cv, act, ptr(v_act_src), v_act, ptr(tb),
             ptr(amax[0]), ptr(amax[1]), ptr(amax[2]), ptr(ws), ws.numel(), ptr(frag if frag is not None else wfrag(wdown)),
             stream_ptr())
        return V if out_bias is None else (V, rb)
    call("mvk_conv4s2_down", ptr(U), ptr(wdown), ptr(bias), ptr(V), n, h, w, Cu, Cv, act, int(u_nchw),
         ptr(u_act_src), u_act, ptr(v_act_src), v_act, ptr(tb), ptr(ws), ws.numel(), FMT_IN_BF3 if in_bf3 else 0,
         ptr(frag if frag is not None else wfrag(wdown)), stream_ptr())
    return V if out_bias is None else (V, rb)


def conv_up(V, wup, bias, n, h, w, Cu, Cv, act=NONE, u_nchw=False, u_act_src=None, u_act=NONE, out_bias=None,
            in_bf3=False, frag=None, amax=None, out=None):
    U = out if out is not None else torch.empty((n, Cu, 2 * h, 2 * w) if u_nchw else (n, 2 * h, 2 * w, Cu), dtype=torch.float32,
                                                device=V.device)
    ws = _ws(U)
    tb, rb = _bias_target(out_bias)
    if amax is not None:
        if u_nchw or in_bf3:
            raise _lib.MvkError("conv_up: the amax form writes NHWC and reads fp32")
        call("mvk_conv4s2_up_s", ptr(V), ptr(wup), ptr(bias), ptr(U), n, h, w, Cu, Cv, act, ptr(u_act_src), u_act, ptr(tb),
             ptr(amax[0]), ptr(amax[1]), ptr(amax[2]), ptr(ws), ws.numel(), ptr(frag if frag is not None else wfrag(wup)),
             stream_ptr())
        return U if out_bias is None else (U, rb)
    call("mvk_conv4s2_up", ptr(V), ptr(wup), ptr(bias), ptr(U), n, h, w, Cu, Cv, act, int(u_nchw),
         ptr(u_act_src), u_act, ptr(tb), ptr(ws), ws.numel(), FMT_IN_BF3 if in_bf3 else 0,
         ptr(frag if frag is not None else wfrag(wup)), stream_ptr())
    return U if out_bias is None else (U, rb)


LEAKY = ACT["leaky_relu_0.2"]


C3_Y_AMAX = _lib.tune("MVK_C3_Y_AMAX", "1") != "0"


def conv3x3(X, wpack, bias, n, H, W, Cin, Cout, act=NONE, y_act_src=None, y_src_act=NONE, out_bias=None, res=None,
            res_alpha=1.0, y_amax=None):
    Y = _new((n, H, W, Cout), X)
    ws = _ws(X)
    if res is not None:
        if out_bias is not None:
            raise _lib.MvkError("conv3x3: a residual and a fused bias gradient are exclusive")
        call("mvk_conv3x3_res", ptr(X), ptr(wpack), ptr(bias), ptr(Y), n, H, W, Cin, Cout, act, ptr(y_act_src), y_src_act,
             ptr(res), float(res_alpha), ptr(ws), ws.numel(), stream_ptr())
        return Y
    tb, rb = _bias_target(out_bias)
    if y_amax is not None:
        call("mvk_conv3x3_y", ptr(X), ptr(wpack), ptr(bias), ptr(Y), n, H, W, Cin, Cout, act, ptr(y_act_src), y_src_act,
             ptr(tb), ptr(y_amax), ptr(ws), ws.numel(), stream_ptr())
        return Y if out_bias is None else (Y, rb)
    call("mvk_conv3x3", ptr(X), ptr(wpack), ptr(bias), ptr(Y), n, H, W, Cin, Cout, act, ptr(y_act_src), y_src_act,
         ptr(tb), ptr(ws), ws.numel(), stream_ptr())
    return Y if out_bias is None else (Y, rb)


def conv3x3_wgrad(X, dY, wparam, n, H, W, Cin, Cout):
    dw, rw = _grad_target(wparam)
    ws = _ws(X)
    call("mvk_conv3x3_wgrad", ptr(X), ptr(dY), ptr(dw), n, H, W, Cin, Cout, ptr(ws), ws.numel(), stream_ptr())
    return rw


def conv3x3_fused_ok(n, H, W, Cin, Cout):
    return bool(_lib.load().mvk_conv3x3_fused_ok(n, H, W, Cin, Cout))


def conv3x3_f(X, wpack, bias, n, H, W, Cin, Cout, act=NONE, y_act_src=None, y_src_act=NONE, res=None, res_alpha=1.0,
              out_bias=None, x_act=NONE, pre_scale=1.0):
    Y = _new((n, H, W, Cout), X)
    ws = _ws(X)
    tb, rb = _bias_target(out_bias)
    call("mvk_conv3x3_f", ptr(X), ptr(wpack), ptr(bias), ptr(Y), n, H, W, Cin, Cout, act, ptr(y_act_src), y_src_act, ptr(res),
         float(res_alpha), ptr(tb), x_act, float(pre_scale), ptr(ws), ws.numel(), stream_ptr())
    return Y if out_bias is None else (Y, rb)


C3_F16 = _lib.tune("MVK_C3_F16", "1") != "0"
IMG_F16 = _lib.tune("MVK_IMG_F16", "1") != "0"
IMG_F16_MIN_ROWS = 1024


def _amax_slots(like, n, create=False):
    sc = _PACK_SCOPE
    if sc is not None:
        ar = sc.get("amax")
        if ar is not None and ar.device == like.device and sc["amax_pos"] + n <= ar.numel():
            sc["amax_pos"] += n
            return ar[sc["amax_pos"] - n:sc["amax_pos"]]
    return torch.zeros(n, dtype=torch.float32, device=like.device)


class AmaxPool:

    def __init__(self, like, slots):
        self.t = _amax_slots(like, slots)
        self.i = 0

    def take(self):
        if self.i >= self.t.numel():
            self.t, self.i = torch.zeros_like(self.t), 0
        self.i += 1
        return self.t[self.i - 1:self.i]
# ... 542 lines not shown
        h2 = conv_down(h1, wd1, b1, B, H // 4, W // 4, chans[1], chans[2], RELU)
        h3 = conv_down(h2, wd2, b2, B, H // 8, W // 8, chans[2], chans[3], RELU)
        if (H // 8, W // 8) != (4, 4):
            raise _lib.MvkError("Encoder_VAE_SVHN expects 32x32 inputs (4x4 feature map before the heads)")
        Kf = 16 * chans[3]
        h3f = h3.view(B, Kf)
        heads = heads_fwd(h3f, wdc1, bc1, wdc2, bc2, L, L, 1)
        if heads is not None:
            mu, lv = heads
        else:
            mu = gemm(h3f, wdc1, B, L, Kf, bias=bc1, bias_mod=L)
            lv = gemm(h3f, wdc2, B, L, Kf, bias=bc2, bias_mod=L)
        ctx.save_for_backward(x, h1, h2, h3, wu1, wu2, wdc1, wdc2, w0, b0, w1, b1, w2, b2, wc1, bc1, wc2, bc2)
        _tap("svhn_encoder", w0, h1, h2, h3)
        ctx.frags = (wfrag(wu1), wfrag(wu2))
        ctx.dims = (B, H, W, chans, L)
        return mu, lv

    @staticmethod
    @once_differentiable
    def backward(ctx, dmu, dlv):
        x, h1, h2, h3, wu1, wu2, wdc1, wdc2, w0, b0, w1, b1, w2, b2, wc1, bc1, wc2, bc2 = ctx.saved_tensors
        B, H, W, ch, L = ctx.dims
        dmu, dlv = _c(dmu).view(B, L), _c(dlv).view(B, L)
        Kf = 16 * ch[3]
        h3f = h3.view(B, Kf)
        schedule.defer_flush_sibling(x.device, node_params=(w0, b0, w1, b1, w2, b2, wc1, bc1, wc2, bc2))
        fused = heads_bwd(h3f, RELU, [dmu, dlv], [wdc1, wdc2], [bc1, bc2], L, 1, flat_c=ch[3], prev_bias=b2,
                          dw_params=[wc1, wc2]) if (H // 8, W // 8) == (4, 4) else None
        if fused is not None:
            dh3, (dwc1, dwc2), (dbc1, dbc2), db2 = fused
        else:
            tw1, dwc1 = _grad_target(wc1)
            tw2, dwc2 = _grad_target(wc2)
            ws = _ws(x)
            call("mvk_flatten_wgrad", ptr(h3f), ptr(dmu), ptr(tw1), B, ch[3], L, ptr(ws), ws.numel(), stream_ptr())
            call("mvk_flatten_wgrad", ptr(h3f), ptr(dlv), ptr(tw2), B, ch[3], L, ptr(ws), ws.numel(), stream_ptr())
            dbc1, dbc2 = colsum(dmu, bc1), colsum(dlv, bc2)
            dh3 = gemm(dmu, wdc1, B, Kf, L, tb=True, c_act_src=h3f, c_act=RELU)
            gemm(dlv, wdc2, B, Kf, L, tb=True, c_act_src=h3f, c_act=RELU, out=dh3, accumulate=True)
        dh3 = dh3.view(B, H // 8, W // 8, ch[3])
        pair = (WGRAD_PAIR and schedule.scope(x.device) is not None and _is_direct(w1) and _is_direct(w2)
                and x.device.type == "cuda")
        if not pair:
            dw2 = conv_wgrad(h2, dh3, w2, B, H // 8, W // 8, ch[2], ch[3])
        if fused is None:
            db2 = colsum(dh3.view(-1, ch[3]), b2)
        dh2, db1 = conv_up(dh3, wu2, None, B, H // 8, W // 8, ch[2], ch[3], u_act_src=h2, u_act=RELU, out_bias=b1,
                           frag=ctx.frags[1])
        if not pair:
            dw1 = conv_wgrad(h1, dh2, w1, B, H // 4, W // 4, ch[1], ch[2])
        dh1, db0 = conv_up(dh2, wu1, None, B, H // 4, W // 4, ch[1], ch[2], u_act_src=h1, u_act=RELU, out_bias=b0,
                           frag=ctx.frags[0])
        if pair:
            ws = _ws(x)
            call("mvk_conv4s2_wgrad_pair", ptr(h2), ptr(dh3), ptr(_grad_target(w2)[0]), H // 8, W // 8, ch[2], ch[3],
                 ptr(h1), ptr(dh2), ptr(_grad_target(w1)[0]), H // 4, W // 4, ch[1], ch[2], B, ptr(ws), ws.numel(), stream_ptr())
            dw2 = dw1 = None
        dw0 = conv_wgrad(x, dh1, w0, B, H // 2, W // 2, ch[0], ch[1], u_nchw=True)
        dx = None
        if ctx.needs_input_grad[0]:
            raise _lib.MvkError("gradient w.r.t. the encoder input image is not implemented")
        return dx, dw0, db0, dw1, db1, dw2, db2, dwc1, dbc1, dwc2, dbc2


TAIL_F16 = _lib.tune("MVK_TAIL_F16", "1") != "0"
C3_SPLIT256 = _lib.tune("MVK_C3_SPLIT256", "1") != "0"
C3_DUAL = _lib.tune("MVK_C3_DUAL", "1") != "0"
TAIL_BWD_F16 = _lib.tune("MVK_TAIL_BWD_F16", "1") != "0"


class SVHNDecoderFn(Function):

    WAITS_FOR_LOSS = True

    @staticmethod
    def forward(ctx, z, w0, b0, w1, b1, w2, b2, w3, b3, nll_x=None, nll_scale=1.0, nll_weight=1.0):
        _check_nll_weight(nll_x, nll_weight)
        L = w0.shape[0]
        z2 = _c(z.reshape(-1, L))
        n = z2.shape[0]
        C1, C2, C3, C4 = w0.shape[1], w1.shape[1], w2.shape[1], w3.shape[1]
        wp0, (wd1, wu1), (wd2, wu2), (wd3, _) = pack_weights(
            [(w0, "unflatten"), (w1, True, True), (w2, True, True), (w3, True, False)])
        f16 = (IMG_F16 and n >= IMG_F16_MIN_ROWS and conv4s2_scaled_ok(n, 4, 4, C2, C1) and conv4s2_scaled_ok(n, 8, 8, C3, C2)
               and all(getattr(t, "mvk_amax", None) is not None for t in (wu1, wu2, wd1, wd2)))
        ctx.f16 = f16
        rot = schedule.rotation(z2.device)
        if rot is not None:
            rot.wait()
        if not (schedule.ROT_SVHN and rot is not None and f16 and nll_x is not None and schedule.LATE_LEAVES
                and schedule.scope(z2.device) is not None and all(_is_direct(t) for t in (w0, w1, w2))):
            rot = None
        ctx.rot, ctx.rot_mode = rot, schedule.ROT_SVHN
        if schedule.ROT_SVHN != 1:
            rot = None
        rkey = ("svhn_dec", w0.data_ptr(), n)
        if rot is not None:
            z2 = rot.buf(rkey + ("z",), z2.shape).copy_(z2)
        if f16:
            pool = AmaxPool(z2, 6) if rot is None else AmaxPool.__new__(AmaxPool)
            if rot is not None:
                pool.t, pool.i = rot.slots(6), 0
            a1, a2 = pool.take(), pool.take()
            a3 = pool.take() if (TAIL_F16 and nll_x is not None) else None
            ctx.a_dpre = pool.take() if (a3 is not None and TAIL_BWD_F16) else None
            ctx.a_g3 = a3
            ctx.bslots = (pool.take(), pool.take())
            g1 = _new((n, 16 * C1), z2) if rot is None else rot.buf(rkey + ("g1",), (n, 16 * C1))
            if L <= 32 and (16 * C1) % 4 == 0:
                call("mvk_gemm_smallk_amax", ptr(z2), ptr(wp0), ptr(g1), n, 16 * C1, L, 0, ptr(b0), C1, RELU, ptr(a1),
                     stream_ptr())
            else:
                gemm(z2, wp0, n, 16 * C1, L, bias=b0, bias_mod=C1, act=RELU, out=g1)
                amax_of(g1, a1)
            g2 = conv_up(g1, wu1, b1, n, 4, 4, C2, C1, RELU, amax=(a1, wu1.mvk_amax, a2),
                         out=None if rot is None else rot.buf(rkey + ("g2",), (n, 8, 8, C2)))
            g3 = conv_up(g2, wu2, b2, n, 8, 8, C3, C2, RELU, amax=(a2, wu2.mvk_amax, a3))
            ctx.wamax = (wd1.mvk_amax, wd2.mvk_amax)
            ctx.gamax = (a1, a2)
        else:
            a3 = None
            g1 = gemm(z2, wp0, n, 16 * C1, L, bias=b0, bias_mod=C1, act=RELU)
            g2 = conv_up(g1, wu1, b1, n, 4, 4, C2, C1, RELU)
            g3 = conv_up(g2, wu2, b2, n, 8, 8, C3, C2, RELU)
        out = _new((n, C4, 32, 32), z2)
        small = bool(_lib.load().mvk_conv4s2_small_up_supported(16, 16, C4, C3))
        ctx.fused = nll_x is not None
        if ctx.fused:
            rows = _new((n,), z2)
            ctx.nll_weight = float(nll_weight)
            if a3 is not None and ctx.a_dpre is not None:
                call("mvk_conv4s2_small_up_fwd_nll_sy", ptr(g3), ptr(w3), ptr(b3), ptr(nll_x), nll_x.shape[0], float(nll_scale),
                     float(nll_weight), ptr(out), ptr(rows), n, 16, 16, C4, C3, SIGMOID, ptr(a3), ptr(ctx.a_dpre), stream_ptr())
            elif a3 is not None:
                call("mvk_conv4s2_small_up_fwd_nll_s", ptr(g3), ptr(w3), ptr(b3), ptr(nll_x), nll_x.shape[0], float(nll_scale),
                     float(nll_weight), ptr(out), ptr(rows), n, 16, 16, C4, C3, SIGMOID, ptr(a3), stream_ptr())
            else:
                call("mvk_conv4s2_small_up_fwd_nll_w", ptr(g3), ptr(w3), ptr(b3), ptr(nll_x), nll_x.shape[0], float(nll_scale),
                     float(nll_weight), ptr(out), ptr(rows), n, 16, 16, C4, C3, SIGMOID, stream_ptr())
        elif small:
            call("mvk_conv4s2_small_up_fwd", ptr(g3), ptr(w3), ptr(b3), ptr(out), n, 16, 16, C4, C3, SIGMOID,
                 stream_ptr())
        else:
            call("mvk_conv4s2_up_nchw_small", ptr(g3), ptr(w3), ptr(b3), ptr(out), n, 16, 16, C4, C3, SIGMOID,
                 stream_ptr())
        ctx.small = small
        ctx.frags = (wfrag(wd1), wfrag(wd2))
        ctx.save_for_backward(z2, g1, g2, g3, out, wp0, wd1, wd2, wd3, w0, b0, w1, b1, w2, b2, w3, b3)
        _tap("svhn_decoder", w0, g1.view(n, 4, 4, C1), g2, g3)
        ctx.dims = (n, L, C1, C2, C3, C4)
        ctx.z_shape = z.shape
        if ctx.fused:
            return rows.view(*z.shape[:-1])
        return out.view(*z.shape[:-1], C4, 32, 32)

    @staticmethod
    @once_differentiable
    def backward(ctx, dout):
        z2, g1, g2, g3, out, wp0, wd1, wd2, wd3, w0, b0, w1, b1, w2, b2, w3, b3 = ctx.saved_tensors
        n, L, C1, C2, C3, C4 = ctx.dims
        if ctx.fused:
            c = const_grad(dout)
            if c is not None and c == ctx.nll_weight:
                drows = None
            else:
                schedule.wait_loss(dout.device)
                drows = _c(dout).reshape(-1)
                if ctx.nll_weight != 1.0:
                    drows = drows * (1.0 / ctx.nll_weight)
            tw3, dw3 = _grad_target(w3)
            tb3, db3 = _grad_target(b3)
            rot = ctx.rot if (ctx.rot is not None and ctx.rot_mode == 1 and schedule.rotation(z2.device) is ctx.rot) else None
            rkey = ("svhn_dec", w0.data_ptr(), n)
            dg3 = _new((n, 16, 16, C3), z2) if rot is None else rot.buf(rkey + ("dg3",), (n, 16, 16, C3))
            ws = _ws(z2)
            tb2, db2 = _grad_target(b2)
            if ctx.f16:
                a_dg3 = ctx.bslots[0]
                if ctx.a_dpre is not None:
                    call("mvk_conv4s2_small_up_bwd_pre_s", ptr(out), ptr(drows), ptr(g3), RELU, ptr(w3), ptr(dg3), ptr(tw3), ptr(tb3),
                         ptr(tb2), ptr(ws), ws.numel(), n, 16, 16, C4, C3, ptr(ctx.a_dpre), ptr(ctx.a_g3), ptr(a_dg3), stream_ptr())
                else:
                    call("mvk_conv4s2_small_up_bwd_pre_y", ptr(out), ptr(drows), ptr(g3), RELU, ptr(w3), ptr(dg3), ptr(tw3), ptr(tb3),
                         ptr(tb2), ptr(ws), ws.numel(), n, 16, 16, C4, C3, ptr(a_dg3), stream_ptr())
                schedule.tail_bwd_done(z2.device)
            else:
                call("mvk_conv4s2_small_up_bwd_pre", ptr(out), ptr(drows), ptr(g3), RELU, ptr(w3), ptr(dg3), ptr(tw3), ptr(tb3),
                     ptr(tb2), ptr(ws), ws.numel(), n, 16, 16, C4, C3, stream_ptr())
        else:
            dout = _c(dout).view(out.shape)
        if ctx.fused:
            pass
        elif ctx.small:
            tw3, dw3 = _grad_target(w3)
            tb3, db3 = _grad_target(b3)
            dg3 = _new((n, 16, 16, C3), z2)
            ws = _ws(z2)
            tb2, db2 = _grad_target(b2)
            call("mvk_conv4s2_small_up_bwd", ptr(dout), ptr(out), SIGMOID, ptr(g3), RELU, ptr(w3), ptr(dg3), ptr(tw3),
                 ptr(tb3), ptr(tb2), ptr(ws), ws.numel(), n, 16, 16, C4, C3, stream_ptr())
        else:
            dw3 = conv_wgrad(dout, g3, w3, n, 16, 16, C4, C3, u_nchw=True, u_act_src=out, u_act=SIGMOID)
            tb3, db3 = _grad_target(b3)
            ws = _ws(dout)
            call("mvk_nchw_channel_sum_acc", ptr(dout), ptr(out), SIGMOID, ptr(tb3), n, C4, 32 * 32, ptr(ws), ws.numel(),
                 stream_ptr())
            dg3 = conv_down(dout, wd3, None, n, 16, 16, C4, C3, NONE, u_nchw=True, u_act_src=out, u_act=SIGMOID,
                            v_act_src=g3, v_act=RELU)
        am2 = am1 = wam2 = wam1 = None
        if ctx.f16:
            if not ctx.fused:
                a_dg3 = None
            a_dg2 = ctx.bslots[1]
            am2 = (a_dg3, ctx.wamax[1] if a_dg3 is not None else None, a_dg2)
            am1 = (a_dg2, ctx.wamax[0], None)
            wam2, wam1 = (a_dg3, ctx.gamax[1]), (a_dg2, ctx.gamax[0])
        if ctx.f16 and wam1 is not None and schedule.LATE_LEAVES and schedule.scope(z2.device) is not None:
            schedule.big_late_leaves(z2.device)
        rot = ctx.rot if (ctx.fused and ctx.rot is not None and schedule.rotation(z2.device) is ctx.rot) else None
        rot0 = rot if (rot is not None and ctx.rot_mode == 2) else None
        if rot0 is not None:
            rot = None
        late = schedule.late_leaves(z2.device, dg3, g2, g1, z2)
        if not late.on:
            rot = rot0 = None
            dw2 = conv_wgrad(dg3, g2, w2, n, 8, 8, C3, C2, amax=wam2)
        if not ctx.small and not ctx.fused:
            db2 = colsum(dg3.view(-1, C3), b2)
        dg2, db1 = conv_down(dg3, wd2, None, n, 8, 8, C3, C2, NONE, v_act_src=g2, v_act=RELU, out_bias=b1,
                             frag=ctx.frags[1], amax=am2, out=None if rot is None else rot.buf(rkey + ("dg2",), (n, 8, 8, C2)))
        if not late.on:
            dw1 = conv_wgrad(dg2, g1, w1, n, 4, 4, C2, C1, amax=wam1)
        rany = rot if rot is not None else rot0
        dg1, db0 = conv_down(dg2, wd1, None, n, 4, 4, C2, C1, NONE, v_act_src=g1, v_act=RELU, out_bias=b0, frag=ctx.frags[0],
                             amax=am1, out=None if rany is None else rany.buf(("svhn_dec", w0.data_ptr(), n, "dg1"), (n, 4, 4, C1)))
        dg1f = dg1.view(n, 16 * C1)
        tw0, dw0 = _grad_target(w0)
        dz = None
        if rot is not None:
            if ctx.needs_input_grad[0]:
                dz = _svhn_dz(dg1f, wp0, n, L, C1).view(ctx.z_shape)

            def leaves():
                conv_wgrad(dg3, g2, w2, n, 8, 8, C3, C2, amax=wam2)
                conv_wgrad(dg2, g1, w1, n, 4, 4, C2, C1, amax=wam1)
                wsl = _ws(z2)
                call("mvk_unflatten_wgrad", ptr(z2), ptr(dg1f), ptr(_grad_target(w0)[0]), n, L, C1, ptr(wsl), wsl.numel(),
                     stream_ptr())

            def prepare(r):
                jobs = [(w0, "unflatten"), (w1, True, True), (w2, True, True), (w3, True, False)]
                for j, o in zip(jobs, _pack_launch(jobs, am=r.slots(len(jobs)))):
                    r.cache[_job_key(j)] = o

            rot.push(leaves, (w0, w1, w2), prepare)
            return dz, None, db0, None, db1, None, db2, dw3, db3, None, None, None
        if late.on:
            if ctx.needs_input_grad[0]:
                dz = _svhn_dz(dg1f, wp0, n, L, C1).view(ctx.z_shape)
            dg2.record_stream(schedule._side_stream(z2.device, 30))
            dg1.record_stream(schedule._side_stream(z2.device, 30))
            with late:
                dw2 = conv_wgrad(dg3, g2, w2, n, 8, 8, C3, C2, amax=wam2)
                dw1 = conv_wgrad(dg2, g1, w1, n, 4, 4, C2, C1, amax=wam1)
                if rot0 is not None:
                    zp = rot0.buf(("svhn_dec", w0.data_ptr(), n, "z"), z2.shape).copy_(z2)

                    def leaf0():
                        wsl = _ws(zp)
                        call("mvk_unflatten_wgrad", ptr(zp), ptr(dg1f), ptr(_grad_target(w0)[0]), n, L, C1, ptr(wsl), wsl.numel(),
                             stream_ptr())

                    def prepare0(r):
                        job = (w0, "unflatten")
                        r.cache[_job_key(job)] = _pack_launch([job])[0]

                    rot0.push(leaf0, (w0,), prepare0)
                else:
                    ws = _ws(z2)
                    call("mvk_unflatten_wgrad", ptr(z2), ptr(dg1f), ptr(tw0), n, L, C1, ptr(ws), ws.numel(), stream_ptr())
            if dw0 is not None or dw1 is not None or dw2 is not None:
                torch.cuda.current_stream(z2.device).wait_stream(schedule._side_stream(z2.device, 30))
            return dz, dw0, db0, dw1, db1, dw2, db2, dw3, db3, None, None, None
        ws = _ws(z2)
        call("mvk_unflatten_wgrad", ptr(z2), ptr(dg1f), ptr(tw0), n, L, C1, ptr(ws), ws.numel(), stream_ptr())
        if ctx.needs_input_grad[0]:
            dz = _svhn_dz(dg1f, wp0, n, L, C1).view(ctx.z_shape)
        return dz, dw0, db0, dw1, db1, dw2, db2, dw3, db3, None, None, None


def _svhn_dz(dg1f, wp0, n, L, C1):
    return gemm(dg1f, wp0, n, L, 16 * C1, tb=True)


def svhn_fused_tail_ok(C4, C3):
    return bool(_lib.load().mvk_conv4s2_small_up_nll_supported(16, 16, C4, C3))


def _rs_conv(pool, X, xam, wpack, bias, n, H, W, Cin, Cout, **kw):
    w_am = getattr(wpack, "mvk_amax", None)
    if (pool is not None and w_am is not None and kw.get("act", NONE) != SIGMOID and kw.get("y_src_act", NONE) != SIGMOID
            and conv3x3_scaled_ok(n, H, W, Cin, Cout)):
        xam = xam if xam is not None else amax_of(X, pool.take())
        yam = pool.take()
        return conv3x3_s(X, wpack, bias, n, H, W, Cin, Cout, xam, w_am, yam, **kw), yam
    if (C3_SPLIT256 and pool is not None and w_am is not None and Cin == 256 and kw.get("res") is None
            and kw.get("act", NONE) != SIGMOID and kw.get("y_src_act", NONE) != SIGMOID and conv3x3_scaled_ok(n, H, W, 128, Cout)):
        xam = xam if xam is not None else amax_of(X, pool.take())
        yam = pool.take()
        kw2 = {k: v for k, v in kw.items() if k not in ("res", "res_alpha")}
        return conv3x3_s_split(X, wpack, bias, n, H, W, Cin, Cout, xam, w_am, yam, **kw2), yam
    if kw.get("x_act", NONE) != NONE or kw.get("pre_scale", 1.0) != 1.0:
        return conv3x3_f(X, wpack, bias, n, H, W, Cin, Cout, **kw), None
    kw.pop("x_act", None)
    kw.pop("pre_scale", None)
    if pool is not None and Cin <= 4 and Cout % 4 == 0 and kw.get("res") is None and C3_Y_AMAX:
        yam = pool.take()
        try:
# ... 1087 lines not shown
```

multivae_amd/models/nn/svhn.py:

```python
import math

import torch
from torch import nn

from ... import kernels
from ..base.base_utils import ModelOutput
from .base_architectures import BaseDecoder, BaseEncoder


class Encoder_VAE_SVHN(BaseEncoder):
    def __init__(self, args):
        BaseEncoder.__init__(self)
        self.input_dim = args.input_dim
        self.latent_dim = args.latent_dim
        self.n_channels = args.input_dim[0]
        self.fBase = 32
        self.enc = nn.Sequential(
            nn.Conv2d(self.n_channels, self.fBase, 4, 2, 1, bias=True), nn.ReLU(True),
            nn.Conv2d(self.fBase, self.fBase * 2, 4, 2, 1, bias=True), nn.ReLU(True),
            nn.Conv2d(self.fBase * 2, self.fBase * 4, 4, 2, 1, bias=True), nn.ReLU(True),
        )
        self.c1 = nn.Conv2d(self.fBase * 4, self.latent_dim, 4, 2, 0)
        self.c2 = nn.Conv2d(self.fBase * 4, self.latent_dim, 4, 2, 0)

    def pack_jobs(self):
        e = self.enc
        first = [] if (e[0].weight.shape[1] <= 4 and e[0].weight.shape[0] in (16, 32, 64)) else [(e[0].weight, True, False)]
        return first + [(e[2].weight, True, True), (e[4].weight, True, True),
                        (self.c1.weight, True, False), (self.c2.weight, True, False)]

    def forward(self, x: torch.Tensor):
        e = self.enc
        mu, lv = kernels.SVHNEncoderFn.apply(x, e[0].weight, e[0].bias, e[2].weight, e[2].bias, e[4].weight,
                                             e[4].bias, self.c1.weight, self.c1.bias, self.c2.weight, self.c2.bias)
        return ModelOutput(embedding=mu.squeeze(), log_covariance=lv.squeeze())


class Decoder_VAE_SVHN(BaseDecoder):
    rows_independent = True

    def __init__(self, args):
        BaseDecoder.__init__(self)
        self.latent_dim = args.latent_dim
        self.fBase = 32
        self.nb_channels = args.input_dim[0]
        self.dec = nn.Sequential(
            nn.ConvTranspose2d(self.latent_dim, self.fBase * 4, 4, 1, 0, bias=True), nn.ReLU(True),
            nn.ConvTranspose2d(self.fBase * 4, self.fBase * 2, 4, 2, 1, bias=True), nn.ReLU(True),
            nn.ConvTranspose2d(self.fBase * 2, self.fBase, 4, 2, 1, bias=True), nn.ReLU(True),
            nn.ConvTranspose2d(self.fBase, self.nb_channels, 4, 2, 1, bias=True), nn.Sigmoid(),
        )

    def pack_jobs(self):
        d = self.dec
        return [(d[0].weight, "unflatten"), (d[2].weight, True, True), (d[4].weight, True, True), (d[6].weight, True, False)]

    def late_leaf_params(self):
        d = self.dec
        return [d[0].weight, d[2].weight, d[4].weight]

    def forward(self, z: torch.Tensor):
        d = self.dec
        out = kernels.SVHNDecoderFn.apply(z, d[0].weight, d[0].bias, d[2].weight, d[2].bias, d[4].weight, d[4].bias,
                                          d[6].weight, d[6].bias)
        return ModelOutput(reconstruction=out)

    def reconstruction_nll(self, z: torch.Tensor, x: torch.Tensor, dist: str = "normal", scale: float = 1.0, row_weight=None):
        d = self.dec
        if dist != "normal" or x.dim() != 4 or z.shape[-1] != self.latent_dim or not torch.is_grad_enabled() \
                or not kernels.svhn_fused_tail_ok(d[6].weight.shape[1], d[6].weight.shape[0]):
            return None
        n = z.reshape(-1, z.shape[-1]).shape[0]
        if (tuple(x.shape[1:]) != (d[6].weight.shape[1], 32, 32) or not x.is_cuda or x.device != z.device
                or x.shape[0] == 0 or n % x.shape[0] != 0):
            return None
        if row_weight is not None and not (math.isfinite(float(row_weight)) and float(row_weight) != 0.0):
            return None
        x = x.float().contiguous()
        if x.data_ptr() % 16:
            x = x.clone()
        return kernels.SVHNDecoderFn.apply(z, d[0].weight, d[0].bias, d[2].weight, d[2].bias, d[4].weight, d[4].bias,
                                           d[6].weight, d[6].bias, x, float(scale),
                                           1.0 if row_weight is None else float(row_weight))
```

Baseline: 538,900 samples/s.

## Prepack per-column scaled fp16 weight fragments for SVHN decoder imgconv kernels

Adds a weight-pack path that emits fp16 fragments in MFMA register layout, each output column carrying its own inverse scale. The scaled fp16 imgconv up and down kernels load these fragments directly instead of converting fp32 weights with a global amax in every block. This removes per-block weight conversion and may improve precision through per-column scaling. In exchange it adds extra buffers, new entry points, and ties the pack step to the row count the decoder last saw.

```diff
diff --git a/include/mvk.h b/include/mvk.h
--- a/include/mvk.h
+++ b/include/mvk.h
@@ -202,6 +202,8 @@
 } mvk_pack_desc;
 int64_t mvk_imgconv_frag_bytes(int Cu, int Cv);
 int mvk_pack_weights(const mvk_pack_desc* jobs, int n, void* stream);
+int mvk_pack_weights_h(const mvk_pack_desc* jobs, int n, void* const* Hdown, void* const* Hup, float* const* inv_down,
+                       float* const* inv_up, void* stream);
 int mvk_conv4s2_down(const float* U, const float* Wdown, const float* bias, float* V, int n, int h, int w,
                      int Cu, int Cv, int act, int u_nchw, const float* u_act_src, int u_act,
                      const float* v_act_src, int v_act, float* colsum_acc, float* ws, int64_t ws_floats, int fmt,
@@ -224,6 +226,12 @@
 int mvk_conv4s2_up_s(const float* V, const float* Wup, const float* bias, float* U, int n, int h, int w, int Cu, int Cv,
                      int act, const float* u_act_src, int u_act, float* colsum_acc, const float* x_amax, const float* w_amax,
                      float* y_amax, float* ws, int64_t ws_floats, const void* wfrag, void* stream);
+int mvk_conv4s2_down_sf(const float* U, const float* Wdown, const float* bias, float* V, int n, int h, int w, int Cu, int Cv,
+                        int act, const float* v_act_src, int v_act, float* colsum_acc, const float* x_amax, const void* hfrag,
+                        const float* w_inv, float* y_amax, float* ws, int64_t ws_floats, void* stream);
+int mvk_conv4s2_up_sf(const float* V, const float* Wup, const float* bias, float* U, int n, int h, int w, int Cu, int Cv,
+                      int act, const float* u_act_src, int u_act, float* colsum_acc, const float* x_amax, const void* hfrag,
+                      const float* w_inv, float* y_amax, float* ws, int64_t ws_floats, void* stream);
 int mvk_conv4s2_wgrad(const float* U, const float* V, float* dWref, int n, int h, int w, int Cu, int Cv,
                       int u_nchw, const float* u_act_src, int u_act, float* ws, int64_t ws_floats, void* stream);
 int mvk_conv4s2_wgrad_pair(const float* U0, const float* V0, float* dW0, int h0, int w0, int Cu0, int Cv0, const float* U1,
diff --git a/multivae_amd/_lib.py b/multivae_amd/_lib.py
--- a/multivae_amd/_lib.py
+++ b/multivae_amd/_lib.py
@@ -93,6 +93,7 @@
     "mvk_conv4s2_down": [_p, _p, _p, _p, _i, _i, _i, _i, _i, _i, _i, _p, _i, _p, _i, _p, _p, _i64, _i, _p, _p],
     "mvk_conv4s2_up": [_p, _p, _p, _p, _i, _i, _i, _i, _i, _i, _i, _p, _i, _p, _p, _i64, _i, _p, _p],
     "mvk_pack_weights": [C.POINTER(PackDesc), _i, _p],
+    "mvk_pack_weights_h": [C.POINTER(PackDesc), _i, _p, _p, _p, _p, _p],
     "mvk_loss_backward_seed": [C.POINTER(SeedDesc), _i, _p, _p],
     "mvk_f32_to_bf3": [_p, _i64, _p, _p],
     "mvk_bf3_to_f32": [_p, _i64, _p, _p],
@@ -118,6 +119,8 @@
     "mvk_conv4s2_small_up_bwd_pre_y": [_p, _p, _p, _i, _p, _p, _p, _p, _p, _p, _i64, _i, _i, _i, _i, _i, _p, _p],
     "mvk_conv4s2_down_s": [_p, _p, _p, _p, _i, _i, _i, _i, _i, _i, _p, _i, _p, _p, _p, _p, _p, _i64, _p, _p],
     "mvk_conv4s2_up_s": [_p, _p, _p, _p, _i, _i, _i, _i, _i, _i, _p, _i, _p, _p, _p, _p, _p, _i64, _p, _p],
+    "mvk_conv4s2_down_sf": [_p, _p, _p, _p, _i, _i, _i, _i, _i, _i, _p, _i, _p, _p, _p, _p, _p, _p, _i64, _p],
+    "mvk_conv4s2_up_sf": [_p, _p, _p, _p, _i, _i, _i, _i, _i, _i, _p, _i, _p, _p, _p, _p, _p, _p, _i64, _p],
     "mvk_conv3x3_wgrad_s": [_p, _p, _p, _p, _i, _i, _i, _i, _i, _i, _f, _p, _p, _p, _i64, _p],
     "mvk_avgpool3s2_fwd": [_p, _p, _i, _i, _i, _i, _p],
     "mvk_avgpool3s2_bwd": [_p, _p, _i, _i, _i, _i, _p],
@@ -334,6 +337,8 @@
     "mvk_conv4s2_down_s": lambda a: 2.0 * a[4] * a[5] * a[6] * 16 * a[7] * a[8],
     "mvk_conv4s2_wgrad_s": lambda a: 2.0 * a[3] * a[4] * a[5] * 16 * a[6] * a[7],
     "mvk_conv4s2_up_s": lambda a: 2.0 * a[4] * a[5] * a[6] * 16 * a[7] * a[8],
+    "mvk_conv4s2_down_sf": lambda a: 2.0 * a[4] * a[5] * a[6] * 16 * a[7] * a[8],
+    "mvk_conv4s2_up_sf": lambda a: 2.0 * a[4] * a[5] * a[6] * 16 * a[7] * a[8],
     "mvk_conv3x3_wgrad_s": lambda a: 2.0 * a[4] * a[5] * a[6] * 9 * a[7] * a[8],
     "mvk_conv3x3_s2": lambda a: 2.0 * a[5] * a[6] * a[7] * 9 * a[8] * a[9],
     "mvk_conv3x3_s_part": lambda a: 2.0 * a[6] * a[7] * a[8] * 9 * a[9] * a[10],
diff --git a/multivae_amd/csrc/igemm.hip b/multivae_amd/csrc/igemm.hip
--- a/multivae_amd/csrc/igemm.hip
+++ b/multivae_amd/csrc/igemm.hip
@@ -675,10 +675,11 @@
                int accumulate = 0, float* y_amax = nullptr);
 int imgconv_up(const float* V, const float* Wup, const void* wfrag, const float* bias, float* U, int n, int h, int w, int Cu,
                int Cv, int act, const float* u_act_src, int u_act, float* colsum_part, int* part_rows, const float* x_amax,
-               const float* w_amax, float* y_amax, hipStream_t s);
+               const float* w_amax, float* y_amax, hipStream_t s, const void* hfrag = nullptr, const float* w_inv = nullptr);
 int imgconv_down(const float* U, const float* Wdown, const void* wfrag, const float* bias, float* V, int n, int h, int w,
                  int Cu, int Cv, int act, const float* v_act_src, int v_act, float* colsum_part, int* part_rows,
-                 const float* x_amax, const float* w_amax, float* y_amax, hipStream_t s);
+                 const float* x_amax, const float* w_amax, float* y_amax, hipStream_t s, const void* hfrag = nullptr,
+                 const float* w_inv = nullptr);
 int imgconv_wgrad(const float* U, const float* V, float* slab, long long slab_floats, int n, int h, int w, int Cu, int Cv,
                   int* nz, const float* u_amax, const float* v_amax, hipStream_t s);
 int c3rs_conv(const float* X, const float* Wp, const float* bias, float* Y, int n, int H, int W, int Cin, int Cout, int act,
@@ -894,9 +895,11 @@
 static int conv4s2_down_impl(const float* U, const float* Wdown, const float* bias, float* V, int n, int h, int w, int Cu,
                              int Cv, int act, int u_nchw, const float* u_act_src, int u_act, const float* v_act_src,
                              int v_act, float* colsum_acc, float* ws, int64_t ws_floats, int fmt, const void* wfrag,
-                             const float* x_amax, const float* w_amax, float* y_amax, void* stream) {
+                             const float* x_amax, const float* w_amax, float* y_amax, void* stream,
+                             const void* hfrag = nullptr, const float* w_inv = nullptr) {
   if (n == 0) return MVK_OK;
-  if (!U || !Wdown || !V || n < 0 || h <= 0 || w <= 0 || Cu <= 0 || Cv <= 0 || (!x_amax != !w_amax)) return MVK_EINVAL;
+  const bool w_scaled = w_amax || (hfrag && w_inv);
+  if (!U || !Wdown || !V || n < 0 || h <= 0 || w <= 0 || Cu <= 0 || Cv <= 0 || (!x_amax != !w_scaled)) return MVK_EINVAL;
   const bool wants_rs = x_amax || y_amax;
   if ((fmt & ~MVK_FMT_IN_BF3) || ((fmt & MVK_FMT_IN_BF3) && (u_nchw || u_act_src))) return MVK_EINVAL;
   if (u_nchw && !u_act_src && !v_act_src && !colsum_acc) {
@@ -910,7 +913,7 @@
     float* dpart = colsum_acc ? defer_scratch(colsum_acc, 256 * (long long)Cv, mvk_stream(stream)) : nullptr;
     float* cpart = dpart ? dpart : ws;
     const int rc = imgconv_down(U, Wdown, wfrag, bias, V, n, h, w, Cu, Cv, act, v_act_src, v_act, colsum_acc ? cpart : nullptr,
-                                &rows, x_amax, w_amax, y_amax, mvk_stream(stream));
+                                &rows, x_amax, w_amax, y_amax, mvk_stream(stream), hfrag, w_inv);
     if (rc == MVK_OK && dpart) return defer_push_plain(colsum_acc, dpart, Cv, rows, Cv, mvk_stream(stream));
     if (rc == MVK_OK && colsum_acc) return colsum_finish(ws, rows, Cv, colsum_acc, mvk_stream(stream));
     if (rc != 1) return rc;
@@ -968,9 +971,10 @@
 static int conv4s2_up_impl(const float* V, const float* Wup, const float* bias, float* U, int n, int h, int w, int Cu,
                            int Cv, int act, int u_nchw, const float* u_act_src, int u_act, float* colsum_acc, float* ws,
                            int64_t ws_floats, int fmt, const void* wfrag, const float* x_amax, const float* w_amax,
-                           float* y_amax, void* stream) {
+                           float* y_amax, void* stream, const void* hfrag = nullptr, const float* w_inv = nullptr) {
   if (n == 0) return MVK_OK;
-  if (!V || !Wup || !U || n < 0 || h <= 0 || w <= 0 || Cu <= 0 || Cv <= 0 || (colsum_acc && u_nchw) || (!x_amax != !w_amax))
+  const bool w_scaled = w_amax || (hfrag && w_inv);
+  if (!V || !Wup || !U || n < 0 || h <= 0 || w <= 0 || Cu <= 0 || Cv <= 0 || (colsum_acc && u_nchw) || (!x_amax != !w_scaled))
     return MVK_EINVAL;
   const bool wants_rs = x_amax || y_amax;
   if (fmt & ~(MVK_FMT_IN_BF3 | MVK_FMT_TILED)) return MVK_EINVAL;
@@ -980,7 +984,7 @@
     float* dpart = colsum_acc ? defer_scratch(colsum_acc, 256 * (long long)Cu, mvk_stream(stream)) : nullptr;
     float* cpart = dpart ? dpart : ws;
     const int rc = imgconv_up(V, Wup, wfrag, bias, U, n, h, w, Cu, Cv, act, u_act_src, u_act, colsum_acc ? cpart : nullptr,
-                              &rows, x_amax, w_amax, y_amax, mvk_stream(stream));
+                              &rows, x_amax, w_amax, y_amax, mvk_stream(stream), hfrag, w_inv);
     if (rc == MVK_OK && dpart) return defer_push_plain(colsum_acc, dpart, Cu, rows, Cu, mvk_stream(stream));
     if (rc == MVK_OK && colsum_acc) return colsum_finish(ws, rows, Cu, colsum_acc, mvk_stream(stream));
     if (rc != 1) return rc;
@@ -1037,6 +1041,24 @@
                          w_amax, y_amax, stream);
 }
 
+int mvk_conv4s2_down_sf(const float* U, const float* Wdown, const float* bias, float* V, int n, int h, int w, int Cu, int Cv,
+                        int act, const float* v_act_src, int v_act, float* colsum_acc, const float* x_amax, const void* hfrag,
+                        const float* w_inv, float* y_amax, float* ws, int64_t ws_floats, void* stream) {
+  if (n == 0) return MVK_OK;
+  if (!mvk_conv4s2_scaled_ok(n, h, w, Cu, Cv) || !x_amax || !hfrag || !w_inv || !mvk_aligned16(hfrag)) return MVK_EINVAL;
+  return conv4s2_down_impl(U, Wdown, bias, V, n, h, w, Cu, Cv, act, 0, nullptr, MVK_ACT_NONE, v_act_src, v_act, colsum_acc, ws,
+                           ws_floats, 0, nullptr, x_amax, nullptr, y_amax, stream, hfrag, w_inv);
+}
+
+int mvk_conv4s2_up_sf(const float* V, const float* Wup, const float* bias, float* U, int n, int h, int w, int Cu, int Cv, int act,
+                      const float* u_act_src, int u_act, float* colsum_acc, const float* x_amax, const void* hfrag,
+                      const float* w_inv, float* y_amax, float* ws, int64_t ws_floats, void* stream) {
+  if (n == 0) return MVK_OK;
+  if (!mvk_conv4s2_scaled_ok(n, h, w, Cu, Cv) || !x_amax || !hfrag || !w_inv || !mvk_aligned16(hfrag)) return MVK_EINVAL;
+  return conv4s2_up_impl(V, Wup, bias, U, n, h, w, Cu, Cv, act, 0, u_act_src, u_act, colsum_acc, ws, ws_floats, 0, nullptr, x_amax,
+                         nullptr, y_amax, stream, hfrag, w_inv);
+}
+
 static int conv3x3_any(const float* X, const float* Wp, const float* bias, float* Y, int n, int H, int W, int Cin, int Cout,
                        int act, const float* y_act_src, int y_src_act, float* colsum_acc, const float* res, float res_alpha,
                        float* ws, int64_t ws_floats, void* stream, int x_act = MVK_ACT_NONE, float pre_scale = 1.f,
diff --git a/multivae_amd/csrc/imgconv.hip b/multivae_amd/csrc/imgconv.hip
--- a/multivae_amd/csrc/imgconv.hip
+++ b/multivae_amd/csrc/imgconv.hip
@@ -30,6 +30,8 @@
   const float* x_amax;
   const float* w_amax;
   float* y_amax;
+  const void* hfrag;
+  const float* w_inv;
 };
 
 template <int KIND, int HS, int CIN, int COUT, int NP = 3>
@@ -80,8 +82,7 @@
   using T = ICfg<KIND, HS, CIN, COUT, NP>;
   static_assert(NP == 3 || PIPE, "the scaled-fp16 form exists for the two-tile-latency loop only");
   using frag = std::conditional_t<NP == 3, bf16x8, f16x8>;
-  const float sx = NP == 2 ? f16_scale_of(*g.x_amax) : 1.f, sw = NP == 2 ? f16_scale_of(*g.w_amax) : 1.f;
-  const float inv_s = NP == 2 ? f16_inv_scale(sx) * f16_inv_scale(sw) : 1.f;
+  const float sx = NP == 2 ? f16_scale_of(*g.x_amax) : 1.f, sw = NP == 2 && !g.hfrag ? f16_scale_of(*g.w_amax) : 1.f;
   extern __shared__ __attribute__((aligned(16))) char lds[];
   mvk_prof_begin(g.prof);
 #ifdef MVK_ICPROF
@@ -114,6 +115,7 @@
   }
   const int py = cls >> 1, px = cls & 1;
   const int ncol = ct * 32 + col;
+  const float inv_s = NP == 2 ? f16_inv_scale(sx) * (g.hfrag ? g.w_inv[ncol] : f16_inv_scale(sw)) : 1.f;
 
   frag Bw[T::NTAPS][T::CHUNKS][NP];
   if (NP == 3 && g.wfrag) {
@@ -124,6 +126,14 @@
       for (int c = 0; c < T::CHUNKS; ++c)
 #pragma unroll
         for (int pc = 0; pc < 3; ++pc) Bw[q][c][pc < NP ? pc : 0] = __builtin_bit_cast(frag, f[((q * T::CHUNKS + c) * 3 + pc) * 64]);
+  } else if (NP == 2 && g.hfrag) {
+    const u32x4* f = reinterpret_cast<const u32x4*>(g.hfrag) + (long long)(wgtype * 4 + wave) * 16 * 2 * 64 + lane;
+#pragma unroll
+    for (int q = 0; q < T::NTAPS; ++q)
+#pragma unroll
+      for (int c = 0; c < T::CHUNKS; ++c)
+#pragma unroll
+        for (int pc = 0; pc < 2; ++pc) Bw[q][c][pc] = __builtin_bit_cast(frag, f[((q * T::CHUNKS + c) * 2 + pc) * 64]);
   } else
 #pragma unroll
   for (int q = 0; q < T::NTAPS; ++q) {
@@ -154,6 +164,9 @@
         frag t = Bw[q][c][pc];
         asm volatile("" : "=a"(Bw[q][c][pc]) : "0"(t));
       }
+#ifdef MVK_ICPROF
+  if (PIPE) ic_pre = IC_CLK() - ic_t0;
+#endif
 
   char* const xbase = lds + 2 * T::BUF;
   float* const csred = reinterpret_cast<float*>(lds + 2 * T::BUF + 2 * T::XBUF);
@@ -687,7 +700,7 @@
 template <int KIND, int HS, int CIN, int COUT>
 static int imgconv_launch(const ImgConvArgs& a, int* part_rows, hipStream_t s) {
   using T = ICfg<KIND, HS, CIN, COUT>;
-  if (a.x_amax && a.w_amax) return imgconv_launch_f16<KIND, HS, CIN, COUT>(a, part_rows, s);
+  if (a.x_amax && (a.w_amax || (a.hfrag && a.w_inv))) return imgconv_launch_f16<KIND, HS, CIN, COUT>(a, part_rows, s);
   static bool attr_done = false;
   static const bool pipe = !(mvk_tune("MVK_IMGCONV_PIPE") && atoi(mvk_tune("MVK_IMGCONV_PIPE")) == 0);
   auto kern = a.act_src ? (pipe ? imgconv_kernel<KIND, HS, CIN, COUT, true, true> : imgconv_kernel<KIND, HS, CIN, COUT, true, false>)
@@ -1018,9 +1031,9 @@
 
 int imgconv_up(const float* V, const float* Wup, const void* wfrag, const float* bias, float* U, int n, int h, int w, int Cu,
                int Cv, int act, const float* u_act_src, int u_act, float* colsum_part, int* part_rows, const float* x_amax,
-               const float* w_amax, float* y_amax, hipStream_t s) {
+               const float* w_amax, float* y_amax, hipStream_t s, const void* hfrag, const float* w_inv) {
   if (h != w) return 1;
-  ImgConvArgs a{V, Wup, wfrag, bias, U, u_act_src, colsum_part, n, act, u_act, nullptr, x_amax, w_amax, y_amax};
+  ImgConvArgs a{V, Wup, wfrag, bias, U, u_act_src, colsum_part, n, act, u_act, nullptr, x_amax, w_amax, y_amax, hfrag, w_inv};
   if (h == 8 && Cv == 64 && Cu == 32) return imgconv_launch<IC_UP, 8, 64, 32>(a, part_rows, s);
   if (h == 4 && Cv == 128 && Cu == 64 && n % 2 == 0) return imgconv_launch<IC_UP, 4, 128, 64>(a, part_rows, s);
   return 1;
@@ -1028,9 +1041,9 @@
 
 int imgconv_down(const float* U, const float* Wdown, const void* wfrag, const float* bias, float* V, int n, int h, int w,
                  int Cu, int Cv, int act, const float* v_act_src, int v_act, float* colsum_part, int* part_rows,
-                 const float* x_amax, const float* w_amax, float* y_amax, hipStream_t s) {
+                 const float* x_amax, const float* w_amax, float* y_amax, hipStream_t s, const void* hfrag, const float* w_inv) {
   if (h != w) return 1;
-  ImgConvArgs a{U, Wdown, wfrag, bias, V, v_act_src, colsum_part, n, act, v_act, nullptr, x_amax, w_amax, y_amax};
+  ImgConvArgs a{U, Wdown, wfrag, bias, V, v_act_src, colsum_part, n, act, v_act, nullptr, x_amax, w_amax, y_amax, hfrag, w_inv};
   if (h == 8 && Cu == 32 && Cv == 64) return imgconv_launch<IC_DOWN, 8, 32, 64>(a, part_rows, s);
   if (h == 4 && Cu == 64 && Cv == 128 && n % 2 == 0) return imgconv_launch<IC_DOWN, 4, 64, 128>(a, part_rows, s);
   return 1;
diff --git a/multivae_amd/csrc/misc.hip b/multivae_amd/csrc/misc.hip
--- a/multivae_amd/csrc/misc.hip
+++ b/multivae_amd/csrc/misc.hip
@@ -22,7 +22,19 @@
 
 struct PackJobs {
   mvk_pack_desc j[MVK_PACK_MAX];
+  void* Hdown[MVK_PACK_MAX];
+  void* Hup[MVK_PACK_MAX];
+  float* inv_down[MVK_PACK_MAX];
+  float* inv_up[MVK_PACK_MAX];
 };
+
+template <int MASK>
+__device__ __forceinline__ float pack_lane_max(float v) {
+#pragma unroll
+  for (int off = 1; off < 64; off <<= 1)
+    if (MASK & off) v = fmaxf(v, __shfl_xor(v, off, 64));
+  return v;
+}
 __device__ __forceinline__ void pack_amax(const mvk_pack_desc& d, int total, float* red) {
   constexpr int NB = 32;
   if (!d.amax || blockIdx.x >= NB) return;
@@ -39,7 +51,7 @@
   mvk::amax_publish(mm, d.amax, red);
 }
 
-__global__ __launch_bounds__(256) void pack_multi_kernel(const PackJobs jobs) {
+__global__ __launch_bounds__(256) __attribute__((amdgpu_waves_per_eu(8, 8))) void pack_multi_kernel(const PackJobs jobs) {
   __shared__ float amax_red[4];
   const mvk_pack_desc& d = jobs.j[blockIdx.y];
   if (d.kind == 2) {
@@ -63,9 +75,14 @@
     typedef float pf4 __attribute__((ext_vector_type(4)));
     typedef unsigned pu4 __attribute__((ext_vector_type(4)));
     float wmax = 0.f;
+    void* const hdown = jobs.Hdown[blockIdx.y];
+    void* const hup = jobs.Hup[blockIdx.y];
+    const bool hfr = hdown != nullptr;
+    __shared__ unsigned cmax[16];
     for (int tile = blockIdx.x; tile < ntiles; tile += gridDim.x) {
       const int cv0 = (tile / tcu) * 8, cu0 = (tile % tcu) * 8;
       __syncthreads();
+      if (hfr && t < 16) cmax[t] = 0u;
 #pragma unroll
       for (int r = 0; r < 4; ++r) {
         const int e = t + 256 * r, cvl = e >> 7, rem = e & 127;
@@ -74,6 +91,34 @@
         wmax = fmaxf(wmax, fabsf(v));
       }
       __syncthreads();
+      if (hfr) {
+        auto amax4 = [](const pf4& v) { return fmaxf(fmaxf(fabsf(v[0]), fabsf(v[1])), fmaxf(fabsf(v[2]), fabsf(v[3]))); };
+        const pf4* const rows = reinterpret_cast<const pf4*>(d.Wref + (long long)cv0 * d.Cu * 16);
+#pragma unroll 1
+        for (int r0 = 0; r0 < d.Cu / 8; r0 += 4) {
+          pf4 v[4];
+#pragma unroll
+          for (int r = 0; r < 4; ++r) v[r] = rows[t + 256 * (r0 + r)];
+#pragma unroll
+          for (int r = 0; r < 4; ++r) {
+            const float m = pack_lane_max<63>(amax4(v[r]));
+            if ((t & 63) == 0) atomicMax(&cmax[(t + 256 * (r0 + r)) / (d.Cu * 4)], __float_as_uint(m));
+          }
+        }
+        const pf4* const cols = reinterpret_cast<const pf4*>(d.Wref + (long long)cu0 * 16) + (t & 31);
+        float mu = 0.f;
+#pragma unroll 1
+        for (int r0 = 0; r0 < d.Cv / 8; r0 += 4) {
+          pf4 v[4];
+#pragma unroll
+          for (int r = 0; r < 4; ++r) v[r] = cols[(long long)((t >> 5) + 8 * (r0 + r)) * d.Cu * 4];
+#pragma unroll
+          for (int r = 0; r < 4; ++r) mu = fmaxf(mu, amax4(v[r]));
+        }
+        mu = pack_lane_max<1 | 2 | 32>(mu);
+        if ((t & (1 | 2 | 32)) == 0) atomicMax(&cmax[8 + ((t & 31) >> 2)], __float_as_uint(mu));
+        __syncthreads();
+      }
       const int pair = t >> 1, half = t & 1, tap = pair >> 3, l8 = pair & 7;
       const int kh = tap >> 2, kw = tap & 3, ph = 1 - (kh & 1), a = kh >> 1, pw = 1 - (kw & 1), b = kw >> 1;
       if (d.Wdown) {
@@ -84,44 +129,78 @@
         const pf4 v = {T[l8][4 * half][tap], T[l8][4 * half + 1][tap], T[l8][4 * half + 2][tap], T[l8][4 * half + 3][tap]};
         *reinterpret_cast<pf4*>(d.Wup + ((long long)(ph * 2 + pw) * 4 * d.Cv + (a * 2 + b) * d.Cv + cv0 + l8) * d.Cu + cu0 + 4 * half) = v;
       }
-      if (t < 128 && d.Fdown) {
+      if (t < 128 && (d.Fdown || hfr)) {
         const int tp = t >> 3, cvl = t & 7, cv = cv0 + cvl;
         const int chunks = d.Cu / 16, ntaps = 16 / chunks, ksplit = 16 / ntaps, nct = d.Cv / 32;
         const int ks = tp / ntaps, q = tp % ntaps, ct = cv / 32;
         const int role = nct * ksplit <= 4 ? ks * nct + ct : ct * 4 + ks;
         const int kk = q * chunks + cu0 / 16, lane = ((cu0 % 16) / 8) * 32 + cv % 32;
-        pu4 pc[3];
-#pragma unroll
-        for (int j = 0; j < 4; ++j) {
-          unsigned p0, p1, p2;
-          mvk::bf3_split(T[cvl][2 * j][tp], T[cvl][2 * j + 1][tp], p0, p1, p2);
-          pc[0][j] = p0;
-          pc[1][j] = p1;
-          pc[2][j] = p2;
+        if (d.Fdown) {
+          pu4 pc[3];
+#pragma unroll
+          for (int j = 0; j < 4; ++j) {
+            unsigned p0, p1, p2;
+            mvk::bf3_split(T[cvl][2 * j][tp], T[cvl][2 * j + 1][tp], p0, p1, p2);
+            pc[0][j] = p0;
+            pc[1][j] = p1;
+            pc[2][j] = p2;
+          }
+          pu4* f = static_cast<pu4*>(d.Fdown);
+#pragma unroll
+          for (int p = 0; p < 3; ++p) f[(((long long)role * 16 + kk) * 3 + p) * 64 + lane] = pc[p];
         }
-        pu4* f = static_cast<pu4*>(d.Fdown);
-#pragma unroll
-        for (int p = 0; p < 3; ++p) f[(((long long)role * 16 + kk) * 3 + p) * 64 + lane] = pc[p];
+        if (hfr) {
+          const float s = mvk::f16_scale_of(__uint_as_float(cmax[cvl]));
+          pu4 hi, lo;
+#pragma unroll
+          for (int j = 0; j < 4; ++j) {
+            unsigned h, l;
+            mvk::f16_split(T[cvl][2 * j][tp] * s, T[cvl][2 * j + 1][tp] * s, h, l);
+            hi[j] = h;
+            lo[j] = l;
+          }
+          pu4* f = static_cast<pu4*>(hdown);
+          f[(((long long)role * 16 + kk) * 2 + 0) * 64 + lane] = hi;
+          f[(((long long)role * 16 + kk) * 2 + 1) * 64 + lane] = lo;
+          if (cu0 == 0 && tp == 0) jobs.inv_down[blockIdx.y][cv] = mvk::f16_inv_scale(s);
+        }
       }
-      if (t >= 128 && d.Fup) {
+      if (t >= 128 && (d.Fup || hfr)) {
         const int i = t - 128, tp = i >> 3, cul = i & 7, cu = cu0 + cul;
         const int kh2 = tp >> 2, kw2 = tp & 3, ph2 = 1 - (kh2 & 1), a2 = kh2 >> 1, pw2 = 1 - (kw2 & 1), b2 = kw2 >> 1;
         const int chunks = d.Cv / 16, ntaps = 16 / chunks, ksplit = 4 / ntaps, nct = d.Cu / 32;
         const int t4 = a2 * 2 + b2, ks = t4 / ntaps, q = t4 % ntaps, ct = cu / 32;
         const int role = (ph2 * 2 + pw2) * (ksplit * nct) + ks * nct + ct;
         const int kk = q * chunks + cv0 / 16, lane = ((cv0 % 16) / 8) * 32 + cu % 32;
-        pu4 pc[3];
-#pragma unroll
-        for (int j = 0; j < 4; ++j) {
-          unsigned p0, p1, p2;
-          mvk::bf3_split(T[2 * j][cul][tp], T[2 * j + 1][cul][tp], p0, p1, p2);
-          pc[0][j] = p0;
-          pc[1][j] = p1;
-          pc[2][j] = p2;
+        if (d.Fup) {
+          pu4 pc[3];
+#pragma unroll
+          for (int j = 0; j < 4; ++j) {
+            unsigned p0, p1, p2;
+            mvk::bf3_split(T[2 * j][cul][tp], T[2 * j + 1][cul][tp], p0, p1, p2);
+            pc[0][j] = p0;
+            pc[1][j] = p1;
+            pc[2][j] = p2;
+          }
+          pu4* f = static_cast<pu4*>(d.Fup);
+#pragma unroll
+          for (int p = 0; p < 3; ++p) f[(((long long)role * 16 + kk) * 3 + p) * 64 + lane] = pc[p];
         }
-        pu4* f = static_cast<pu4*>(d.Fup);
-#pragma unroll
-        for (int p = 0; p < 3; ++p) f[(((long long)role * 16 + kk) * 3 + p) * 64 + lane] = pc[p];
+        if (hfr) {
+          const float s = mvk::f16_scale_of(__uint_as_float(cmax[8 + cul]));
+          pu4 hi, lo;
+#pragma unroll
+          for (int j = 0; j < 4; ++j) {
+            unsigned h, l;
+            mvk::f16_split(T[2 * j][cul][tp] * s, T[2 * j + 1][cul][tp] * s, h, l);
+            hi[j] = h;
+            lo[j] = l;
+          }
+          pu4* f = static_cast<pu4*>(hup);
+          f[(((long long)role * 16 + kk) * 2 + 0) * 64 + lane] = hi;
+          f[(((long long)role * 16 + kk) * 2 + 1) * 64 + lane] = lo;
+          if (cv0 == 0 && tp == 0) jobs.inv_up[blockIdx.y][cu] = mvk::f16_inv_scale(s);
+        }
       }
     }
     if (d.amax && blockIdx.x < ntiles) mvk::amax_publish(wmax, d.amax, amax_red);
@@ -592,15 +671,32 @@
 }
 
 int mvk_pack_weights(const mvk_pack_desc* jobs, int n, void* stream) {
+  return mvk_pack_weights_h(jobs, n, nullptr, nullptr, nullptr, nullptr, stream);
+}
+
+int mvk_pack_weights_h(const mvk_pack_desc* jobs, int n, void* const* Hdown, void* const* Hup, float* const* inv_down,
+                       float* const* inv_up, void* stream) {
   if (!jobs || n <= 0 || n > MVK_PACK_MAX) return MVK_EINVAL;
+  if (Hdown && (!Hup || !inv_down || !inv_up)) return MVK_EINVAL;
   PackJobs pj{};
   int maxtot = 0;
   for (int i = 0; i < n; ++i) {
     const mvk_pack_desc& d = jobs[i];
-    if (!d.Wref || d.Cv <= 0 || d.Cu <= 0 || d.kind < 0 || d.kind > 2 || (!d.Wdown && !d.Wup && !d.Fdown && !d.Fup) ||
+    const bool h = Hdown && (Hdown[i] || Hup[i] || inv_down[i] || inv_up[i]);
+    if (!d.Wref || d.Cv <= 0 || d.Cu <= 0 || d.kind < 0 || d.kind > 2 || (!d.Wdown && !d.Wup && !d.Fdown && !d.Fup && !h) ||
         (d.kind == 1 && !d.Wup))
       return MVK_EINVAL;
     if ((d.Fdown || d.Fup) && (d.kind != 0 || mvk_imgconv_frag_bytes(d.Cu, d.Cv) == 0)) return MVK_EINVAL;
+    if (h) {
+      if (!Hdown[i] || !Hup[i] || !inv_down[i] || !inv_up[i] || d.kind != 0 || mvk_imgconv_frag_bytes(d.Cu, d.Cv) == 0 ||
+          (d.ld_down > 0 && d.ld_down % 4) || d.col_off % 4 || !mvk_aligned16(d.Wref) || (d.Wdown && !mvk_aligned16(d.Wdown)) ||
+          (d.Wup && !mvk_aligned16(d.Wup)) || !mvk_aligned16(Hdown[i]) || !mvk_aligned16(Hup[i]))
+        return MVK_EINVAL;
+      pj.Hdown[i] = Hdown[i];
+      pj.Hup[i] = Hup[i];
+      pj.inv_down[i] = inv_down[i];
+      pj.inv_up[i] = inv_up[i];
+    }
     pj.j[i] = d;
     if (pj.j[i].ld_down <= 0) pj.j[i].ld_down = d.Cv;
     const int tot = d.Cv * d.Cu * 16;
diff --git a/multivae_amd/kernels.py b/multivae_amd/kernels.py
--- a/multivae_amd/kernels.py
+++ b/multivae_amd/kernels.py
@@ -176,6 +176,19 @@
     return getattr(w, "mvk_frag", None)
 
 
+def whfrag(w):
+    return getattr(w, "mvk_hfrag", None)
+
+
+def _hfrag(like, Cu, Cv):
+    nb = _lib.load().mvk_imgconv_frag_bytes(Cu, Cv) * 2 // 3
+    if not nb:
+        return None
+    buf = torch.empty(2 * nb + 4 * (Cv + Cu), dtype=torch.uint8, device=like.device)
+    inv = buf[2 * nb:].view(torch.float32)
+    return buf[:nb], buf[nb:2 * nb], inv[:Cv], inv[Cv:]
+
+
 PACK_MAX = 16
 _PACK_SCOPE = None
 
@@ -202,8 +215,15 @@
         return False
 
 
+HFRAG = "h"
+
+
+def hfrag_flag(rows):
+    return (HFRAG,) if (IMG_F16 and rows >= IMG_F16_MIN_ROWS) else ()
+
+
 def _job_key(job):
-    return (job[0].data_ptr(), tuple(job[0].shape)) + tuple(job[1:])
+    return (job[0].data_ptr(), tuple(job[0].shape)) + tuple(x for x in job[1:] if x != HFRAG)
 
 
 def pack_weights(jobs):
@@ -247,6 +267,7 @@
 
 def _pack_launch(jobs, am=None):
     descs = (PackDesc * len(jobs))()
+    hptrs = [(C.c_void_p * len(jobs))() for _ in range(4)]
     outs = []
     if am is None and ((C3_F16 and any(job[1] == "c3" for job in jobs))
                        or (IMG_F16 and any(job[1] not in ("c3", "unflatten") for job in jobs))):
@@ -289,8 +310,16 @@
                 for t in (wd, wu):
                     if t is not None:
                         t.mvk_amax = am[i:i + 1]
+            hf = _hfrag(wref, Cu, Cv) if (IMG_F16 and HFRAG in job[3:]) else None
+            if hf is not None:
+                for a, t in zip(hptrs, hf):
+                    a[i] = t.data_ptr()
+                if wd is not None:
+                    wd.mvk_hfrag = (hf[0], hf[2])
+                if wu is not None:
+                    wu.mvk_hfrag = (hf[1], hf[3])
             outs.append((wd, wu))
-    call("mvk_pack_weights", descs, len(jobs), stream_ptr())
+    call("mvk_pack_weights_h", descs, len(jobs), *hptrs, stream_ptr())
     return outs
 
 
@@ -299,13 +328,17 @@
 
 
 def conv_down(U, wdown, bias, n, h, w, Cu, Cv, act=NONE, u_nchw=False, u_act_src=None, u_act=NONE,
-              v_act_src=None, v_act=NONE, out_bias=None, in_bf3=False, frag=None, amax=None, out=None):
+              v_act_src=None, v_act=NONE, out_bias=None, in_bf3=False, frag=None, amax=None, out=None, hfrag=None):
     V = out if out is not None else torch.empty((n, h, w, Cv), dtype=torch.float32, device=U.device)
     ws = _ws(V)
     tb, rb = _bias_target(out_bias)
     if amax is not None:
         if u_nchw or u_act_src is not None or in_bf3:
             raise _lib.MvkError("conv_down: the amax form takes NHWC fp32 input without a fused input activation")
+        if hfrag is not None and amax[0] is not None:
+            call("mvk_conv4s2_down_sf", ptr(U), ptr(wdown), ptr(bias), ptr(V), n, h, w, Cu, Cv, act, ptr(v_act_src), v_act, ptr(tb),
+                 ptr(amax[0]), ptr(hfrag[0]), ptr(hfrag[1]), ptr(amax[2]), ptr(ws), ws.numel(), stream_ptr())
+            return V if out_bias is None else (V, rb)
         call("mvk_conv4s2_down_s", ptr(U), ptr(wdown), ptr(bias), ptr(V), n, h, w, Cu, Cv, act, ptr(v_act_src), v_act, ptr(tb),
              ptr(amax[0]), ptr(amax[1]), ptr(amax[2]), ptr(ws), ws.numel(), ptr(frag if frag is not None else wfrag(wdown)),
              stream_ptr())
@@ -317,7 +350,7 @@
 
 
 def conv_up(V, wup, bias, n, h, w, Cu, Cv, act=NONE, u_nchw=False, u_act_src=None, u_act=NONE, out_bias=None,
-            in_bf3=False, frag=None, amax=None, out=None):
+            in_bf3=False, frag=None, amax=None, out=None, hfrag=None):
     U = out if out is not None else torch.empty((n, Cu, 2 * h, 2 * w) if u_nchw else (n, 2 * h, 2 * w, Cu), dtype=torch.float32,
                                                 device=V.device)
     ws = _ws(U)
@@ -325,6 +358,10 @@
     if amax is not None:
         if u_nchw or in_bf3:
             raise _lib.MvkError("conv_up: the amax form writes NHWC and reads fp32")
+        if hfrag is not None and amax[0] is not None:
+            call("mvk_conv4s2_up_sf", ptr(V), ptr(wup), ptr(bias), ptr(U), n, h, w, Cu, Cv, act, ptr(u_act_src), u_act, ptr(tb),
+                 ptr(amax[0]), ptr(hfrag[0]), ptr(hfrag[1]), ptr(amax[2]), ptr(ws), ws.numel(), stream_ptr())
+            return U if out_bias is None else (U, rb)
         call("mvk_conv4s2_up_s", ptr(V), ptr(wup), ptr(bias), ptr(U), n, h, w, Cu, Cv, act, ptr(u_act_src), u_act, ptr(tb),
              ptr(amax[0]), ptr(amax[1]), ptr(amax[2]), ptr(ws), ws.numel(), ptr(frag if frag is not None else wfrag(wup)),
              stream_ptr())
@@ -1033,7 +1070,7 @@
         n = z2.shape[0]
         C1, C2, C3, C4 = w0.shape[1], w1.shape[1], w2.shape[1], w3.shape[1]
         wp0, (wd1, wu1), (wd2, wu2), (wd3, _) = pack_weights(
-            [(w0, "unflatten"), (w1, True, True), (w2, True, True), (w3, True, False)])
+            [(w0, "unflatten"), (w1, True, True) + hfrag_flag(n), (w2, True, True) + hfrag_flag(n), (w3, True, False)])
         f16 = (IMG_F16 and n >= IMG_F16_MIN_ROWS and conv4s2_scaled_ok(n, 4, 4, C2, C1) and conv4s2_scaled_ok(n, 8, 8, C3, C2)
                and all(getattr(t, "mvk_amax", None) is not None for t in (wu1, wu2, wd1, wd2)))
         ctx.f16 = f16
@@ -1065,9 +1102,9 @@
             else:
                 gemm(z2, wp0, n, 16 * C1, L, bias=b0, bias_mod=C1, act=RELU, out=g1)
                 amax_of(g1, a1)
-            g2 = conv_up(g1, wu1, b1, n, 4, 4, C2, C1, RELU, amax=(a1, wu1.mvk_amax, a2),
+            g2 = conv_up(g1, wu1, b1, n, 4, 4, C2, C1, RELU, amax=(a1, wu1.mvk_amax, a2), hfrag=whfrag(wu1),
                          out=None if rot is None else rot.buf(rkey + ("g2",), (n, 8, 8, C2)))
-            g3 = conv_up(g2, wu2, b2, n, 8, 8, C3, C2, RELU, amax=(a2, wu2.mvk_amax, a3))
+            g3 = conv_up(g2, wu2, b2, n, 8, 8, C3, C2, RELU, amax=(a2, wu2.mvk_amax, a3), hfrag=whfrag(wu2))
             ctx.wamax = (wd1.mvk_amax, wd2.mvk_amax)
             ctx.gamax = (a1, a2)
         else:
@@ -1098,6 +1135,7 @@
                  stream_ptr())
         ctx.small = small
         ctx.frags = (wfrag(wd1), wfrag(wd2))
+        ctx.hfrags = (whfrag(wd1), whfrag(wd2))
         ctx.save_for_backward(z2, g1, g2, g3, out, wp0, wd1, wd2, wd3, w0, b0, w1, b1, w2, b2, w3, b3)
         _tap("svhn_decoder", w0, g1.view(n, 4, 4, C1), g2, g3)
         ctx.dims = (n, L, C1, C2, C3, C4)
@@ -1180,12 +1218,12 @@
         if not ctx.small and not ctx.fused:
             db2 = colsum(dg3.view(-1, C3), b2)
         dg2, db1 = conv_down(dg3, wd2, None, n, 8, 8, C3, C2, NONE, v_act_src=g2, v_act=RELU, out_bias=b1,
-                             frag=ctx.frags[1], amax=am2, out=None if rot is None else rot.buf(rkey + ("dg2",), (n, 8, 8, C2)))
+                             frag=ctx.frags[1], amax=am2, hfrag=ctx.hfrags[1], out=None if rot is None else rot.buf(rkey + ("dg2",), (n, 8, 8, C2)))
         if not late.on:
             dw1 = conv_wgrad(dg2, g1, w1, n, 4, 4, C2, C1, amax=wam1)
         rany = rot if rot is not None else rot0
         dg1, db0 = conv_down(dg2, wd1, None, n, 4, 4, C2, C1, NONE, v_act_src=g1, v_act=RELU, out_bias=b0, frag=ctx.frags[0],
-                             amax=am1, out=None if rany is None else rany.buf(("svhn_dec", w0.data_ptr(), n, "dg1"), (n, 4, 4, C1)))
+                             amax=am1, hfrag=ctx.hfrags[0], out=None if rany is None else rany.buf(("svhn_dec", w0.data_ptr(), n, "dg1"), (n, 4, 4, C1)))
         dg1f = dg1.view(n, 16 * C1)
         tw0, dw0 = _grad_target(w0)
         dz = None
diff --git a/multivae_amd/models/nn/svhn.py b/multivae_amd/models/nn/svhn.py
--- a/multivae_amd/models/nn/svhn.py
+++ b/multivae_amd/models/nn/svhn.py
@@ -44,6 +44,7 @@
         self.latent_dim = args.latent_dim
         self.fBase = 32
         self.nb_channels = args.input_dim[0]
+        self._rows = 0
         self.dec = nn.Sequential(
             nn.ConvTranspose2d(self.latent_dim, self.fBase * 4, 4, 1, 0, bias=True), nn.ReLU(True),
             nn.ConvTranspose2d(self.fBase * 4, self.fBase * 2, 4, 2, 1, bias=True), nn.ReLU(True),
@@ -53,7 +54,8 @@
 
     def pack_jobs(self):
         d = self.dec
-        return [(d[0].weight, "unflatten"), (d[2].weight, True, True), (d[4].weight, True, True), (d[6].weight, True, False)]
+        h = kernels.hfrag_flag(self._rows)
+        return [(d[0].weight, "unflatten"), (d[2].weight, True, True) + h, (d[4].weight, True, True) + h, (d[6].weight, True, False)]
 
     def late_leaf_params(self):
         d = self.dec
@@ -61,6 +63,7 @@
 
     def forward(self, z: torch.Tensor):
         d = self.dec
+        self._rows = z.numel() // max(z.shape[-1], 1)
         out = kernels.SVHNDecoderFn.apply(z, d[0].weight, d[0].bias, d[2].weight, d[2].bias, d[4].weight, d[4].bias,
                                           d[6].weight, d[6].bias)
         return ModelOutput(reconstruction=out)
@@ -79,6 +82,7 @@
         x = x.float().contiguous()
         if x.data_ptr() % 16:
             x = x.clone()
+        self._rows = n
         return kernels.SVHNDecoderFn.apply(z, d[0].weight, d[0].bias, d[2].weight, d[2].bias, d[4].weight, d[4].bias,
                                            d[6].weight, d[6].bias, x, float(scale),
                                            1.0 if row_weight is None else float(row_weight))
```

New measurement: 543,300 samples/s (median of 6 runs). Within noise of the previous version (+0.8%).
